# CompVis/stable-diffusion

Measured on AMD Instinct MI355X. Metric: 512x512 images/sec, SD-v1-4 50-step PLMS CFG=7.5, higher is better.
Workload: dtype f16

## Files before the change

### include/sdmi.h

```cpp
#ifndef SDMI_H_
#define SDMI_H_

#include <stdint.h>

#ifdef __cplusplus
extern "C" {
#endif

#define SDMI_ABI_VERSION 17

typedef struct sdmi_unet sdmi_unet;

typedef struct sdmi_unet_cfg {
  int32_t in_channels;
  int32_t out_channels;
  int32_t model_channels;
  int32_t num_res_blocks;
  int32_t n_levels;
  int32_t channel_mult[8];
  int32_t n_attention_resolutions;
  int32_t attention_resolutions[8];
  int32_t num_heads;
  int32_t transformer_depth;
  int32_t context_dim;
// ... 2 lines not shown
const char* sdmi_last_error(void);
int sdmi_abi_version(void);
int sdmi_has_experiments(void);

int sdmi_unet_create(const sdmi_unet_cfg* cfg, sdmi_unet** out);
#define SDMI_PRECISION_MIXED 0
#define SDMI_PRECISION_FULL 1
int sdmi_unet_create_with_precision(const sdmi_unet_cfg* cfg, int precision, sdmi_unet** out);
int sdmi_unet_precision(const sdmi_unet* h);
typedef struct sdmi_unet_ext {
  int32_t attention_block;
  int32_t resblock_updown;
} sdmi_unet_ext;
int sdmi_unet_create_ext(const sdmi_unet_cfg* cfg, const sdmi_unet_ext* ext, int precision, sdmi_unet** out);
#define SDMI_UNET_SCALE_SHIFT_NORM 1u
#define SDMI_UNET_NUM_HEAD_CHANNELS_SHIFT 16
#define SDMI_UNET_NUM_HEAD_CHANNELS_MASK 0x0fff0000u
#define SDMI_UNET_NUM_HEAD_CHANNELS(n) (((unsigned)(n) << SDMI_UNET_NUM_HEAD_CHANNELS_SHIFT) & SDMI_UNET_NUM_HEAD_CHANNELS_MASK)
int sdmi_unet_create_flags(const sdmi_unet_cfg* cfg, const sdmi_unet_ext* ext, unsigned flags, int precision, sdmi_unet** out);
int sdmi_unet_destroy(sdmi_unet* h);
int sdmi_unet_num_weights(const sdmi_unet* h);
int sdmi_unet_weight_info(const sdmi_unet* h, int idx, char* key_buf, int key_buf_len, int64_t* shape4, int* ndim);
int sdmi_unet_set_weight(sdmi_unet* h, const char* key, const float* ptr, const int64_t* shape, int ndim, void* stream);
int sdmi_unet_finalize(sdmi_unet* h);

int64_t sdmi_unet_packed_bytes(sdmi_unet* h);
int sdmi_unet_export_packed(sdmi_unet* h, void* host_buf, int64_t bytes, void* stream);
int sdmi_unet_import_packed(sdmi_unet* h, const void* host_buf, int64_t bytes, void* stream);

int64_t sdmi_unet_workspace_bytes(sdmi_unet* h, int B, int H, int W, int Lctx);

int sdmi_unet_cache_context(sdmi_unet* h, const float* ctx, int B, int Lctx, void* workspace, int64_t workspace_bytes,
                            void* stream);
int sdmi_unet_reserve_context(sdmi_unet* h, int B, int Lctx);

int sdmi_unet_cache_timesteps(sdmi_unet* h, const int64_t* t_host, int n, void* stream);
int sdmi_unet_hint_timestep(sdmi_unet* h, int64_t t);
int sdmi_unet_tape_stats(sdmi_unet* h, int64_t* replayed, int64_t* recorded);

int sdmi_unet_forward(sdmi_unet* h, const float* x, const int64_t* t_i64, const float* t_f32, const float* ctx,
                      float* eps_out, int B, int H, int W, int Lctx, void* workspace, int64_t workspace_bytes,
                      void* stream);

int sdmi_sampler_step(const float* eps_model, int cfg, float scale, const float* x, int mode, const float* old0,
                      const float* old1, const float* old2, float a_t, float a_prev, float sigma, float sqrt_1m_at,
                      const float* noise, float* e_t_out, float* x_prev, float* pred_x0, int64_t n, void* stream);


int sdmi_dpm_solver_step(const float* eps_model, int cfg, float scale, const float* x, const float* m_prev, float alpha_s,
                         float sigma_s, float cx, float a, float inv_r0, int order, float* m_out, float* x_next, int64_t n,
                         void* stream);

typedef struct sdmi_vae sdmi_vae;
typedef struct sdmi_vae_cfg {
  int32_t ch;
  int32_t out_ch;
  int32_t n_levels;
  int32_t ch_mult[8];
  int32_t num_res_blocks;
  int32_t in_channels;
  int32_t z_channels;
  int32_t embed_dim;
} sdmi_vae_cfg;
int sdmi_vae_create(const sdmi_vae_cfg* cfg, int parts, sdmi_vae** out);
typedef struct sdmi_vae_ext {
  int32_t double_z;
  int32_t mid_attn;
  int32_t n_embed;
} sdmi_vae_ext;
int sdmi_vae_create_ext(const sdmi_vae_cfg* cfg, const sdmi_vae_ext* ext, int parts, sdmi_vae** out);
int sdmi_vae_create_precision(const sdmi_vae_cfg* cfg, const sdmi_vae_ext* ext, int parts, int precision, sdmi_vae** out);
int sdmi_vae_precision(const sdmi_vae* h);
int sdmi_vae_decode_vq(sdmi_vae* h, const float* z, float z_scale, int quantize, float* img, int B, int H, int W, void* workspace,
                       int64_t workspace_bytes, void* stream);
int sdmi_vae_destroy(sdmi_vae* h);
int sdmi_vae_num_weights(const sdmi_vae* h);
int sdmi_vae_weight_info(const sdmi_vae* h, int idx, char* key_buf, int key_buf_len, int64_t* shape4, int* ndim);
int sdmi_vae_set_weight(sdmi_vae* h, const char* key, const float* ptr, const int64_t* shape, int ndim, void* stream);
int sdmi_vae_finalize(sdmi_vae* h);
int64_t sdmi_vae_decode_workspace_bytes(sdmi_vae* h, int B, int H, int W);
int sdmi_vae_decode(sdmi_vae* h, const float* z, float z_scale, float* img, int B, int H, int W, void* workspace,
                    int64_t workspace_bytes, void* stream);
int64_t sdmi_vae_encode_workspace_bytes(sdmi_vae* h, int B, int H, int W);
int sdmi_vae_encode(sdmi_vae* h, const float* img, float* moments, int B, int H, int W, void* workspace,
                    int64_t workspace_bytes, void* stream);


typedef struct sdmi_clip sdmi_clip;
typedef struct sdmi_clip_cfg {
  int32_t vocab_size;
  int32_t hidden_size;
  int32_t intermediate_size;
  int32_t num_layers;
  int32_t num_heads;
  int32_t max_positions;
} sdmi_clip_cfg;
int sdmi_clip_create(const sdmi_clip_cfg* cfg, sdmi_clip** out);
int sdmi_clip_destroy(sdmi_clip* h);
int sdmi_clip_num_weights(const sdmi_clip* h);
int sdmi_clip_weight_info(const sdmi_clip* h, int idx, char* key_buf, int key_buf_len, int64_t* shape4, int* ndim);
int sdmi_clip_set_weight(sdmi_clip* h, const char* key, const float* ptr, const int64_t* shape, int ndim, void* stream);
int sdmi_clip_finalize(sdmi_clip* h);
int64_t sdmi_clip_workspace_bytes(sdmi_clip* h, int B, int L);
int sdmi_clip_forward(sdmi_clip* h, const int64_t* ids, float* out, int B, int L, void* workspace, int64_t workspace_bytes,
                      void* stream);

typedef struct sdmi_bert sdmi_bert;
typedef struct sdmi_bert_cfg {
  int32_t vocab_size;
  int32_t dim;
  int32_t depth;
  int32_t heads;
  int32_t dim_head;
  int32_t ff_inner;
  int32_t max_seq_len;
} sdmi_bert_cfg;
int sdmi_bert_create(const sdmi_bert_cfg* cfg, sdmi_bert** out);
int sdmi_bert_destroy(sdmi_bert* h);
int sdmi_bert_num_weights(const sdmi_bert* h);
int sdmi_bert_weight_info(const sdmi_bert* h, int idx, char* key_buf, int key_buf_len, int64_t* shape4, int* ndim);
int sdmi_bert_set_weight(sdmi_bert* h, const char* key, const float* ptr, const int64_t* shape, int ndim, void* stream);
int sdmi_bert_finalize(sdmi_bert* h);
int64_t sdmi_bert_workspace_bytes(sdmi_bert* h, int B, int L);
int sdmi_bert_forward(sdmi_bert* h, const int64_t* ids, float* out, int B, int L, void* workspace, int64_t workspace_bytes,
                      void* stream);

typedef struct sdmi_igemm_desc {
  const void* a0; const void* a1; const void* a2;
  int32_t c0, c1, c2, lda0, lda1, lda2;
  int32_t B, Hin, Win, Hout, Wout, ksize, stride, up;
  const void* w;
  int32_t N;
  int32_t mode;
  const float* bias; const float* rowvec; int32_t ld_rowvec;
  const float* residual; int32_t ldr;
  float* out_f32; void* out_f16; int32_t ldo;
  void* seg_dst[3]; int32_t seg_kind[3];
  int32_t heads, dh, ntok, ntok_pad, segC;
  int32_t splitk;
  float* splitk_ws; int64_t splitk_ws_floats;
  int32_t tile;
  int32_t dma;
  int32_t asym_pad;
  int32_t gn_n; void* gn_acc[2]; int32_t gn_cpg[2]; int32_t gn_cbase[2];
  int32_t* splitk_cnt; int32_t splitk_cnt_ints;
  int32_t split16;
  const float* f16_scale; float* lnp_out;
  const float* lnf_part; int32_t lnf_npart; float lnf_eps; const float* lnf_cs; const float* lnf_d;
  const float* pgn_gamma; const float* pgn_beta; float pgn_eps; int32_t pgn_silu;
  void* pgn_out; int32_t pgn_keep_f32; int32_t* pgn_applied;
  void* out_lo;
} sdmi_igemm_desc;
int sdmi_k_igemm(const sdmi_igemm_desc* d, void* stream);
int sdmi_k_ff_tail(const sdmi_igemm_desc* proj_out, const void* ln_f16, const float* lnp, float ln_eps, const float* csd,
                   const void* wgg_f16, const void* wff2_f16, const float* bff2, const float* t, void* stream);
int sdmi_k_st_tail(const sdmi_igemm_desc* proj_out, const void* a_f16, const void* wo_f16, const float* bo, float* t, const float* ln_gamma,
                   float ln_eps, const float* csd, const void* wgg_f16, const void* wff2_f16, const float* bff2, void* stream);
int sdmi_k_gn_conv3(const sdmi_igemm_desc* conv, const float* x0, const float* x1, int c0, int c1, float* gn_ws, int64_t gn_ws_floats,
                    const float* gn_gamma, const float* gn_beta, float gn_eps, void* stream);
int sdmi_k_st_head(const float* x, float* gn_ws, int64_t gn_ws_floats, const float* gn_gamma, const float* gn_beta, float gn_eps,
                   const void* w_in3, const float* b_in, float* t, const float* ln_gamma, float ln_eps, const void* wqkv_f16,
                   const float* lnf_cs, const float* lnf_d, void* q, void* k, void* vt, int B, int ntok, int ntok_pad, int heads, int dh,
                   int C, void* stream);
int sdmi_k_st_mid(const void* a_f16, const void* wo_f16, const float* bo, float* t, const float* ln_gamma, float ln_eps, const void* wq_f16,
                  const float* lnf_cs, const float* lnf_d, void* q, int B, int ntok, int heads, int dh, int C, void* stream);
int sdmi_k_st_mid_ctx(const void* a_f16, const void* wo_f16, const float* bo, float* t, const float* ln_gamma, float ln_eps, const void* wq_f16,
                      const float* lnf_cs, const float* lnf_d, const void* ctx_k, const void* ctx_vt, int nkv, int nkv_pad, float scale, void* ao_out,
                      int B, int ntok, int heads, int dh, int C, void* stream);
int sdmi_k_ln_fold_prep(const void* w_f16, int N, int K, int ldw, const float* gamma, const float* beta, const float* bias,
                        float* cs, float* d, void* stream);
int sdmi_k_attention(const void* q, const void* k, const void* vt, void* out, int BH, int heads, int nq, int nkv,
                     int nkv_pad, int d, float scale, void* stream);
int sdmi_k_attention_split16(const void* q, const void* q_lo, const void* k, const void* k_lo, const void* vt, const void* vt_lo, void* out,
                             void* out_lo, int BH, int heads, int nq, int nkv, int nkv_pad, int d, float scale, void* stream);
int sdmi_k_attention_causal(const void* q, const void* k, const void* vt, void* out, int BH, int heads, int n, int n_pad,
                            int d, float scale, void* stream);
int sdmi_k_groupnorm(const float* x0, const float* x1, int c0, int c1, int B, int HW, const float* gamma,
                     const float* beta, float eps, int silu, void* out_f16, float* out_f32, void* raw_f16, void* out_lo,
                     void* raw_lo, float* partial_ws, int64_t partial_floats, void* stream);
int64_t sdmi_k_groupnorm_ws_floats(int B, int HW);
int sdmi_k_groupnorm_film(const float* x0, const float* x1, int c0, int c1, int B, int HW, const float* gamma, const float* beta, float eps,
                          int silu, const float* film, int film_ld, void* out_f16, float* out_f32, void* raw_f16, void* out_lo, void* raw_lo,
                          float* partial_ws, int64_t partial_floats, void* stream);
int sdmi_k_layernorm(const float* x, const float* gamma, const float* beta, void* out_f16, int M, int C, float eps,
                     void* stream);
int sdmi_k_cast_f16(const float* x, void* out_f16, void* out_lo, int64_t n, void* stream);
int sdmi_k_split_heads(const float* src, int ld, int col0, void* dst, void* dst_lo, int kind, int B, int ntok, int ntok_pad, int heads, int dh,
                       void* stream);
int sdmi_k_geglu_split(const float* src, int M, int F, void* out, void* out_lo, void* stream);
int sdmi_k_layernorm_split(const float* x, const float* gamma, const float* beta, void* out, void* out_lo, int M, int C, float eps, void* stream);
int sdmi_k_timestep_embedding(const int64_t* t_i64, const float* t_f32, float* out, int B, int dim, void* stream);
int sdmi_k_small_linear(const float* in, int ld_in, const float* w, const float* bias, float* out, int ld_out, int B,
                        int N, int K, int silu_in, void* stream);
int sdmi_k_conv_in(const float* x_nchw, const float* w_oihw, const float* bias, float* out_nhwc, int B, int Cin, int H,
                   int W, int Cout, void* stream);
int sdmi_k_conv_out(const float* h_nhwc, const float* w_ohwi, const float* bias, float* out_nchw, int B, int H, int W,
                    int Cin, int Cout, void* stream);
int sdmi_k_pack_conv_weight(const float* w_oihw, void* dst_f16, int O, int I, int KH, int KW, void* stream);
int sdmi_k_pack_conv_weight_src(const float* w_oihw, void* dst_f16, int O, int I, int KH, int KW, int c0, int c1, int c2, void* stream);
int sdmi_k_pack_conv_out(const float* w_oihw, float* dst_ohwi, int O, int I, void* stream);
int sdmi_k_pack_split3(const float* w, void* dst_f16, int N, int K, void* stream);
int sdmi_k_pack_conv_split3(const float* w_oihw, void* dst_f16, int O, int I, int KH, int KW, void* stream);
int sdmi_k_pointwise_nchw(const float* x, const float* w, const float* bias, float* out, int B, int Cin, int Cout, int HW,
                          float in_scale, void* stream);
int sdmi_k_softmax_rows(const float* S, void* P_f16, int rows, int cols, float scale, void* stream);
int sdmi_k_vq_quantize(const float* z, float z_scale, const float* codebook, float* norms_ws, int n_embed, int D, float* zq, int32_t* idx,
                       int B, int HW, void* stream);
int sdmi_k_resample2(const float* x, float* out_f32, void* out_f16, void* out_lo, int B, int H, int W, int C, int dir, void* stream);
int sdmi_k_patch_unfold(const float* x, const float* c, float* out, int B, int Cx, int Cc, int H, int W, int kh, int kw, int sy, int sx,
                        int l0, int nl, void* stream);
int sdmi_k_patch_fold(const float* o, const float* w, float* out, int B, int C, int H, int W, int kh, int kw, int sy, int sx, int uf, int df,
                      int norm_only, void* stream);
int sdmi_k_gelu_erf(const float* x, void* out_f16, int64_t n, void* stream);
int sdmi_k_pack_geglu(const float* w, const float* bias, void* wdst_f16, float* bdst, int N, int K, void* stream);
int sdmi_image_to_uint8(const float* img_nchw, void* out_nhwc_u8, int B, int C, int H, int W, void* stream);
int sdmi_range_check(int enable);
int sdmi_range_report(char* json_buf, int json_buf_len);
int sdmi_tune_begin(void);
int sdmi_tune_round(int r);
int sdmi_tune_end(const char* path, int* n_keys);
int sdmi_tune_dump(char* buf, int buflen);
int sdmi_profile_begin(void);
int sdmi_profile_end(char* json_buf, int json_buf_len);
int sdmi_k_prefetch_lines(const void* ptr, int64_t bytes, void* stream);
const void* sdmi_zero_page(void);

#ifdef __cplusplus
}
#endif
#endif
```

### stable-diffusion_amd/_lib.py

```python
import ctypes as C
import os

_HERE = os.path.dirname(os.path.abspath(__file__))
LIB_PATH = os.environ.get('SDMI_LIB_PATH') or os.path.join(_HERE, 'libsdmi.so')

c_f32p = C.c_void_p
c_ptr = C.c_void_p


class UNetCfg(C.Structure):
    _fields_ = [('in_channels', C.c_int32), ('out_channels', C.c_int32), ('model_channels', C.c_int32),
                ('num_res_blocks', C.c_int32), ('n_levels', C.c_int32), ('channel_mult', C.c_int32 * 8),
                ('n_attention_resolutions', C.c_int32), ('attention_resolutions', C.c_int32 * 8),
                ('num_heads', C.c_int32), ('transformer_depth', C.c_int32), ('context_dim', C.c_int32)]


class VaeCfg(C.Structure):
    _fields_ = [('ch', C.c_int32), ('out_ch', C.c_int32), ('n_levels', C.c_int32), ('ch_mult', C.c_int32 * 8),
                ('num_res_blocks', C.c_int32), ('in_channels', C.c_int32), ('z_channels', C.c_int32),
                ('embed_dim', C.c_int32)]


class UNetExt(C.Structure):
    _fields_ = [('attention_block', C.c_int32), ('resblock_updown', C.c_int32)]


class VaeExt(C.Structure):
    _fields_ = [('double_z', C.c_int32), ('mid_attn', C.c_int32), ('n_embed', C.c_int32)]


class ClipCfg(C.Structure):
    _fields_ = [('vocab_size', C.c_int32), ('hidden_size', C.c_int32), ('intermediate_size', C.c_int32),
                ('num_layers', C.c_int32), ('num_heads', C.c_int32), ('max_positions', C.c_int32)]


class BertCfg(C.Structure):
    _fields_ = [('vocab_size', C.c_int32), ('dim', C.c_int32), ('depth', C.c_int32), ('heads', C.c_int32),
                ('dim_head', C.c_int32), ('ff_inner', C.c_int32), ('max_seq_len', C.c_int32)]


class IGemmDesc(C.Structure):
    _fields_ = [('a0', c_ptr), ('a1', c_ptr), ('a2', c_ptr),
                ('c0', C.c_int32), ('c1', C.c_int32), ('c2', C.c_int32),
                ('lda0', C.c_int32), ('lda1', C.c_int32), ('lda2', C.c_int32),
                ('B', C.c_int32), ('Hin', C.c_int32), ('Win', C.c_int32), ('Hout', C.c_int32), ('Wout', C.c_int32),
                ('ksize', C.c_int32), ('stride', C.c_int32), ('up', C.c_int32),
                ('w', c_ptr), ('N', C.c_int32), ('mode', C.c_int32),
                ('bias', c_ptr), ('rowvec', c_ptr), ('ld_rowvec', C.c_int32),
                ('residual', c_ptr), ('ldr', C.c_int32),
                ('out_f32', c_ptr), ('out_f16', c_ptr), ('ldo', C.c_int32),
                ('seg_dst', c_ptr * 3), ('seg_kind', C.c_int32 * 3),
                ('heads', C.c_int32), ('dh', C.c_int32), ('ntok', C.c_int32), ('ntok_pad', C.c_int32),
                ('segC', C.c_int32), ('splitk', C.c_int32), ('splitk_ws', c_ptr), ('splitk_ws_floats', C.c_int64),
                ('tile', C.c_int32), ('dma', C.c_int32), ('asym_pad', C.c_int32),
                ('gn_n', C.c_int32), ('gn_acc', c_ptr * 2), ('gn_cpg', C.c_int32 * 2), ('gn_cbase', C.c_int32 * 2),
                ('splitk_cnt', c_ptr), ('splitk_cnt_ints', C.c_int32), ('split16', C.c_int32),
                ('f16_scale', c_ptr), ('lnp_out', c_ptr), ('lnf_part', c_ptr), ('lnf_npart', C.c_int32),
                ('lnf_eps', C.c_float), ('lnf_cs', c_ptr), ('lnf_d', c_ptr),
                ('pgn_gamma', c_ptr), ('pgn_beta', c_ptr), ('pgn_eps', C.c_float), ('pgn_silu', C.c_int32),
                ('pgn_out', c_ptr), ('pgn_keep_f32', C.c_int32), ('pgn_applied', C.POINTER(C.c_int32)),
                ('out_lo', c_ptr)]


_SIGS = {
    'sdmi_last_error': (C.c_char_p, []),
    'sdmi_abi_version': (C.c_int, []),
    'sdmi_unet_create': (C.c_int, [C.POINTER(UNetCfg), C.POINTER(c_ptr)]),
    'sdmi_unet_create_with_precision': (C.c_int, [C.POINTER(UNetCfg), C.c_int, C.POINTER(c_ptr)]),
    'sdmi_unet_precision': (C.c_int, [c_ptr]),
    'sdmi_unet_create_ext': (C.c_int, [C.POINTER(UNetCfg), C.POINTER(UNetExt), C.c_int, C.POINTER(c_ptr)]),
    'sdmi_unet_create_flags': (C.c_int, [C.POINTER(UNetCfg), C.POINTER(UNetExt), C.c_uint, C.c_int, C.POINTER(c_ptr)]),
    'sdmi_unet_destroy': (C.c_int, [c_ptr]),
    'sdmi_unet_num_weights': (C.c_int, [c_ptr]),
    'sdmi_unet_weight_info': (C.c_int, [c_ptr, C.c_int, C.c_char_p, C.c_int, C.POINTER(C.c_int64), C.POINTER(C.c_int)]),
    'sdmi_unet_set_weight': (C.c_int, [c_ptr, C.c_char_p, c_ptr, C.POINTER(C.c_int64), C.c_int, c_ptr]),
    'sdmi_unet_finalize': (C.c_int, [c_ptr]),
    'sdmi_unet_packed_bytes': (C.c_int64, [c_ptr]),
    'sdmi_unet_export_packed': (C.c_int, [c_ptr, c_ptr, C.c_int64, c_ptr]),
    'sdmi_unet_import_packed': (C.c_int, [c_ptr, c_ptr, C.c_int64, c_ptr]),
    'sdmi_unet_workspace_bytes': (C.c_int64, [c_ptr, C.c_int, C.c_int, C.c_int, C.c_int]),
    'sdmi_unet_cache_context': (C.c_int, [c_ptr, c_ptr, C.c_int, C.c_int, c_ptr, C.c_int64, c_ptr]),
    'sdmi_unet_reserve_context': (C.c_int, [c_ptr, C.c_int, C.c_int]),
    'sdmi_unet_cache_timesteps': (C.c_int, [c_ptr, C.POINTER(C.c_int64), C.c_int, c_ptr]),
    'sdmi_unet_hint_timestep': (C.c_int, [c_ptr, C.c_int64]),
    'sdmi_unet_tape_stats': (C.c_int, [c_ptr, C.POINTER(C.c_int64), C.POINTER(C.c_int64)]),
    'sdmi_unet_forward': (C.c_int, [c_ptr, c_ptr, c_ptr, c_ptr, c_ptr, c_ptr, C.c_int, C.c_int, C.c_int, C.c_int,
                                    c_ptr, C.c_int64, c_ptr]),
    'sdmi_sampler_step': (C.c_int, [c_ptr, C.c_int, C.c_float, c_ptr, C.c_int, c_ptr, c_ptr, c_ptr, C.c_float,
                                    C.c_float, C.c_float, C.c_float, c_ptr, c_ptr, c_ptr, c_ptr, C.c_int64, c_ptr]),
    'sdmi_dpm_solver_step': (C.c_int, [c_ptr, C.c_int, C.c_float, c_ptr, c_ptr, C.c_float, C.c_float, C.c_float, C.c_float,
                                       C.c_float, C.c_int, c_ptr, c_ptr, C.c_int64, c_ptr]),
    'sdmi_vae_create': (C.c_int, [C.POINTER(VaeCfg), C.c_int, C.POINTER(c_ptr)]),
    'sdmi_vae_destroy': (C.c_int, [c_ptr]),
    'sdmi_vae_create_ext': (C.c_int, [C.POINTER(VaeCfg), C.POINTER(VaeExt), C.c_int, C.POINTER(c_ptr)]),
    'sdmi_vae_create_precision': (C.c_int, [C.POINTER(VaeCfg), C.POINTER(VaeExt), C.c_int, C.c_int, C.POINTER(c_ptr)]),
    'sdmi_vae_precision': (C.c_int, [c_ptr]),
    'sdmi_vae_decode_vq': (C.c_int, [c_ptr, c_ptr, C.c_float, C.c_int, c_ptr, C.c_int, C.c_int, C.c_int, c_ptr, C.c_int64, c_ptr]),
    'sdmi_k_vq_quantize': (C.c_int, [c_ptr, C.c_float, c_ptr, c_ptr, C.c_int, C.c_int, c_ptr, c_ptr, C.c_int, C.c_int, c_ptr]),
    'sdmi_k_patch_unfold': (C.c_int, [c_ptr, c_ptr, c_ptr] + [C.c_int] * 11 + [c_ptr]),
    'sdmi_k_patch_fold': (C.c_int, [c_ptr, c_ptr, c_ptr] + [C.c_int] * 11 + [c_ptr]),
    'sdmi_k_resample2': (C.c_int, [c_ptr, c_ptr, c_ptr, c_ptr, C.c_int, C.c_int, C.c_int, C.c_int, C.c_int, c_ptr]),
    'sdmi_vae_num_weights': (C.c_int, [c_ptr]),
    'sdmi_vae_weight_info': (C.c_int, [c_ptr, C.c_int, C.c_char_p, C.c_int, C.POINTER(C.c_int64), C.POINTER(C.c_int)]),
    'sdmi_vae_set_weight': (C.c_int, [c_ptr, C.c_char_p, c_ptr, C.POINTER(C.c_int64), C.c_int, c_ptr]),
    'sdmi_vae_finalize': (C.c_int, [c_ptr]),
    'sdmi_vae_decode_workspace_bytes': (C.c_int64, [c_ptr, C.c_int, C.c_int, C.c_int]),
    'sdmi_vae_decode': (C.c_int, [c_ptr, c_ptr, C.c_float, c_ptr, C.c_int, C.c_int, C.c_int, c_ptr, C.c_int64, c_ptr]),
    'sdmi_vae_encode_workspace_bytes': (C.c_int64, [c_ptr, C.c_int, C.c_int, C.c_int]),
    'sdmi_vae_encode': (C.c_int, [c_ptr, c_ptr, c_ptr, C.c_int, C.c_int, C.c_int, c_ptr, C.c_int64, c_ptr]),
    'sdmi_clip_create': (C.c_int, [C.POINTER(ClipCfg), C.POINTER(c_ptr)]),
    'sdmi_clip_destroy': (C.c_int, [c_ptr]),
    'sdmi_clip_num_weights': (C.c_int, [c_ptr]),
    'sdmi_clip_weight_info': (C.c_int, [c_ptr, C.c_int, C.c_char_p, C.c_int, C.POINTER(C.c_int64), C.POINTER(C.c_int)]),
    'sdmi_clip_set_weight': (C.c_int, [c_ptr, C.c_char_p, c_ptr, C.POINTER(C.c_int64), C.c_int, c_ptr]),
    'sdmi_clip_finalize': (C.c_int, [c_ptr]),
    'sdmi_clip_workspace_bytes': (C.c_int64, [c_ptr, C.c_int, C.c_int]),
    'sdmi_clip_forward': (C.c_int, [c_ptr, c_ptr, c_ptr, C.c_int, C.c_int, c_ptr, C.c_int64, c_ptr]),
    'sdmi_bert_create': (C.c_int, [C.POINTER(BertCfg), C.POINTER(c_ptr)]),
    'sdmi_bert_destroy': (C.c_int, [c_ptr]),
    'sdmi_bert_num_weights': (C.c_int, [c_ptr]),
    'sdmi_bert_weight_info': (C.c_int, [c_ptr, C.c_int, C.c_char_p, C.c_int, C.POINTER(C.c_int64), C.POINTER(C.c_int)]),
    'sdmi_bert_set_weight': (C.c_int, [c_ptr, C.c_char_p, c_ptr, C.POINTER(C.c_int64), C.c_int, c_ptr]),
    'sdmi_bert_finalize': (C.c_int, [c_ptr]),
    'sdmi_bert_workspace_bytes': (C.c_int64, [c_ptr, C.c_int, C.c_int]),
    'sdmi_bert_forward': (C.c_int, [c_ptr, c_ptr, c_ptr, C.c_int, C.c_int, c_ptr, C.c_int64, c_ptr]),
    'sdmi_has_experiments': (C.c_int, []),
    'sdmi_k_igemm': (C.c_int, [C.POINTER(IGemmDesc), c_ptr]),
    'sdmi_k_ff_tail': (C.c_int, [C.POINTER(IGemmDesc), c_ptr, c_ptr, C.c_float, c_ptr, c_ptr, c_ptr, c_ptr, c_ptr, c_ptr]),
    'sdmi_k_gn_conv3': (C.c_int, [C.POINTER(IGemmDesc), c_ptr, c_ptr, C.c_int, C.c_int, c_ptr, C.c_int64, c_ptr, c_ptr, C.c_float, c_ptr]),
    'sdmi_k_st_mid_ctx': (C.c_int, [c_ptr, c_ptr, c_ptr, c_ptr, c_ptr, C.c_float, c_ptr, c_ptr, c_ptr, c_ptr, c_ptr, C.c_int, C.c_int, C.c_float, c_ptr,
                                    C.c_int, C.c_int, C.c_int, C.c_int, C.c_int, c_ptr]),
    'sdmi_k_st_tail': (C.c_int, [C.POINTER(IGemmDesc), c_ptr, c_ptr, c_ptr, c_ptr, c_ptr, C.c_float, c_ptr, c_ptr, c_ptr, c_ptr, c_ptr]),
    'sdmi_k_st_mid': (C.c_int, [c_ptr, c_ptr, c_ptr, c_ptr, c_ptr, C.c_float, c_ptr, c_ptr, c_ptr, c_ptr, C.c_int, C.c_int, C.c_int, C.c_int,
                                C.c_int, c_ptr]),
    'sdmi_k_st_head': (C.c_int, [c_ptr, c_ptr, C.c_int64, c_ptr, c_ptr, C.c_float, c_ptr, c_ptr, c_ptr, c_ptr, C.c_float, c_ptr, c_ptr, c_ptr,
                                 c_ptr, c_ptr, c_ptr, C.c_int, C.c_int, C.c_int, C.c_int, C.c_int, C.c_int, c_ptr]),
    'sdmi_k_attention_split16': (C.c_int, [c_ptr, c_ptr, c_ptr, c_ptr, c_ptr, c_ptr, c_ptr, c_ptr, C.c_int, C.c_int, C.c_int, C.c_int,
                                           C.c_int, C.c_int, C.c_float, c_ptr]),
    'sdmi_k_attention_causal': (C.c_int, [c_ptr, c_ptr, c_ptr, c_ptr, C.c_int, C.c_int, C.c_int, C.c_int, C.c_int, C.c_float,
                                          c_ptr]),
    'sdmi_k_pointwise_nchw': (C.c_int, [c_ptr, c_ptr, c_ptr, c_ptr, C.c_int, C.c_int, C.c_int, C.c_int, C.c_float, c_ptr]),
    'sdmi_k_softmax_rows': (C.c_int, [c_ptr, c_ptr, C.c_int, C.c_int, C.c_float, c_ptr]),
    'sdmi_k_gelu_erf': (C.c_int, [c_ptr, c_ptr, C.c_int64, c_ptr]),
    'sdmi_k_attention': (C.c_int, [c_ptr, c_ptr, c_ptr, c_ptr, C.c_int, C.c_int, C.c_int, C.c_int, C.c_int, C.c_int,
                                   C.c_float, c_ptr]),
    'sdmi_k_groupnorm': (C.c_int, [c_ptr, c_ptr, C.c_int, C.c_int, C.c_int, C.c_int, c_ptr, c_ptr, C.c_float, C.c_int,
                                   c_ptr, c_ptr, c_ptr, c_ptr, c_ptr, c_ptr, C.c_int64, c_ptr]),
    'sdmi_k_groupnorm_ws_floats': (C.c_int64, [C.c_int, C.c_int]),
    'sdmi_k_groupnorm_film': (C.c_int, [c_ptr, c_ptr, C.c_int, C.c_int, C.c_int, C.c_int, c_ptr, c_ptr, C.c_float, C.c_int, c_ptr, C.c_int,
                                        c_ptr, c_ptr, c_ptr, c_ptr, c_ptr, c_ptr, C.c_int64, c_ptr]),
    'sdmi_k_layernorm': (C.c_int, [c_ptr, c_ptr, c_ptr, c_ptr, C.c_int, C.c_int, C.c_float, c_ptr]),
    'sdmi_k_cast_f16': (C.c_int, [c_ptr, c_ptr, c_ptr, C.c_int64, c_ptr]),
    'sdmi_k_split_heads': (C.c_int, [c_ptr, C.c_int, C.c_int, c_ptr, c_ptr, C.c_int, C.c_int, C.c_int, C.c_int, C.c_int, C.c_int,
                                     c_ptr]),
    'sdmi_k_geglu_split': (C.c_int, [c_ptr, C.c_int, C.c_int, c_ptr, c_ptr, c_ptr]),
    'sdmi_k_layernorm_split': (C.c_int, [c_ptr, c_ptr, c_ptr, c_ptr, c_ptr, C.c_int, C.c_int, C.c_float, c_ptr]),
    'sdmi_k_timestep_embedding': (C.c_int, [c_ptr, c_ptr, c_ptr, C.c_int, C.c_int, c_ptr]),
    'sdmi_k_small_linear': (C.c_int, [c_ptr, C.c_int, c_ptr, c_ptr, c_ptr, C.c_int, C.c_int, C.c_int, C.c_int,
                                      C.c_int, c_ptr]),
    'sdmi_k_conv_in': (C.c_int, [c_ptr, c_ptr, c_ptr, c_ptr, C.c_int, C.c_int, C.c_int, C.c_int, C.c_int, c_ptr]),
    'sdmi_k_conv_out': (C.c_int, [c_ptr, c_ptr, c_ptr, c_ptr, C.c_int, C.c_int, C.c_int, C.c_int, C.c_int, c_ptr]),
    'sdmi_k_pack_conv_weight': (C.c_int, [c_ptr, c_ptr, C.c_int, C.c_int, C.c_int, C.c_int, c_ptr]),
    'sdmi_k_pack_conv_weight_src': (C.c_int, [c_ptr, c_ptr, C.c_int, C.c_int, C.c_int, C.c_int, C.c_int, C.c_int, C.c_int, c_ptr]),
    'sdmi_k_pack_conv_out': (C.c_int, [c_ptr, c_ptr, C.c_int, C.c_int, c_ptr]),
    'sdmi_k_pack_split3': (C.c_int, [c_ptr, c_ptr, C.c_int, C.c_int, c_ptr]),
    'sdmi_k_pack_conv_split3': (C.c_int, [c_ptr, c_ptr, C.c_int, C.c_int, C.c_int, C.c_int, c_ptr]),
    'sdmi_k_pack_geglu': (C.c_int, [c_ptr, c_ptr, c_ptr, c_ptr, C.c_int, C.c_int, c_ptr]),
    'sdmi_k_ln_fold_prep': (C.c_int, [c_ptr, C.c_int, C.c_int, C.c_int, c_ptr, c_ptr, c_ptr, c_ptr, c_ptr, c_ptr]),
    'sdmi_image_to_uint8': (C.c_int, [c_ptr, c_ptr, C.c_int, C.c_int, C.c_int, C.c_int, c_ptr]),
    'sdmi_range_check': (C.c_int, [C.c_int]),
    'sdmi_range_report': (C.c_int, [C.c_char_p, C.c_int]),
    'sdmi_tune_begin': (C.c_int, []),
    'sdmi_tune_round': (C.c_int, [C.c_int]),
    'sdmi_tune_end': (C.c_int, [C.c_char_p, C.POINTER(C.c_int)]),
    'sdmi_tune_dump': (C.c_int, [C.c_char_p, C.c_int]),
    'sdmi_profile_begin': (C.c_int, []),
    'sdmi_profile_end': (C.c_int, [C.c_char_p, C.c_int]),
    'sdmi_k_prefetch_lines': (C.c_int, [c_ptr, C.c_int64, c_ptr]),
    'sdmi_zero_page': (c_ptr, []),
}

_lib = None


class SdmiError(RuntimeError):
    pass


def load():
    global _lib
    if _lib is None:
        if not os.path.exists(LIB_PATH):
            raise SdmiError(f'{LIB_PATH} not found: build it with `python stable-diffusion_amd/build.py` '
                            '(the MI355X path has no fallback implementation)')
        lib = C.CDLL(LIB_PATH)
        for name, (res, args) in _SIGS.items():
            fn = getattr(lib, name)
            fn.restype = res
            fn.argtypes = args
        if lib.sdmi_abi_version() != 17:
            raise SdmiError('libsdmi ABI version mismatch')
        _lib = lib
    return _lib


def exported_symbols():
    return sorted(_SIGS)


def check(rc):
    if rc != 0:
        raise SdmiError(load().sdmi_last_error().decode('utf-8', 'replace'))


def ptr(t):
    return None if t is None else t.data_ptr()


def stream_ptr():
    import torch
    return torch.cuda.current_stream().cuda_stream
```

### stable-diffusion_amd/csrc/api.cpp

```cpp
#include <string.h>

#include <new>

#include "prof.h"
#include "split16.h"
#include "unet.h"
#include "vae.h"
#include "clip.h"

namespace sdmi {
static thread_local std::string g_err;
void set_error(const std::string& msg) { g_err = msg; }
int fail(const std::string& msg) { g_err = msg; return -1; }
}

struct sdmi_unet { sdmi::UNet impl; };
struct sdmi_vae { sdmi::Vae impl; };
struct sdmi_clip { sdmi::ClipText impl; };
struct sdmi_bert { sdmi::BertText impl; };

using namespace sdmi;

static void* g_zero_page[16] = {nullptr};
static int zero_page(const f16** out) {
// ... 188 lines not shown
                       int64_t workspace_bytes, void* stream) {
  SDMI_CHECK(h && z && img, "null argument");
  return h->impl.decode(z, z_scale, img, B, H, W, workspace, workspace_bytes, (hipStream_t)stream, false, nullptr, quantize != 0);
}
int64_t sdmi_vae_encode_workspace_bytes(sdmi_vae* h, int B, int H, int W) {
  if (!h) { fail("null handle"); return 0; }
  int64_t need = 0;
  if (h->impl.encode(nullptr, nullptr, B, H, W, nullptr, 0, nullptr, true, &need)) return 0;
  return need;
}
int sdmi_vae_encode(sdmi_vae* h, const float* img, float* moments, int B, int H, int W, void* workspace,
                    int64_t workspace_bytes, void* stream) {
  SDMI_CHECK(h && img && moments, "null argument");
  return h->impl.encode(img, moments, B, H, W, workspace, workspace_bytes, (hipStream_t)stream, false, nullptr);
}
int sdmi_k_pointwise_nchw(const float* x, const float* w, const float* bias, float* out, int B, int Cin, int Cout, int HW,
                          float in_scale, void* stream) {
  return launch_pointwise_nchw(x, w, bias, out, B, Cin, Cout, HW, in_scale, (hipStream_t)stream);
}
int sdmi_k_softmax_rows(const float* S, void* P_f16, int rows, int cols, float scale, void* stream) {
  return launch_softmax_rows(S, (f16*)P_f16, rows, cols, cols, cols, scale, (hipStream_t)stream);
}


int sdmi_clip_create(const sdmi_clip_cfg* cfg, sdmi_clip** out) {
  SDMI_CHECK(cfg && out, "null argument");
  sdmi_clip* h = new (std::nothrow) sdmi_clip();
  SDMI_CHECK(h != nullptr, "out of host memory");
  if (h->impl.build(*cfg)) { delete h; return -1; }
  *out = h;
  return 0;
}
int sdmi_clip_destroy(sdmi_clip* h) { delete h; return 0; }
int sdmi_clip_num_weights(const sdmi_clip* h) { return h ? (int)h->impl.slots().size() : fail("null handle"); }
static int text_weight_info(const TextEncBase& t, int idx, char* key_buf, int key_buf_len, int64_t* shape4, int* ndim) {
  SDMI_CHECK(key_buf && shape4 && ndim, "null argument");
  SDMI_CHECK(idx >= 0 && idx < (int)t.slots().size(), "weight index out of range");
  const CWeightSlot& s = t.slots()[idx];
  SDMI_CHECK((int)s.key.size() + 1 <= key_buf_len, "key buffer too small");
  memcpy(key_buf, s.key.c_str(), s.key.size() + 1);
  *ndim = (int)s.shape.size();
  for (int i = 0; i < 4; ++i) shape4[i] = i < *ndim ? s.shape[i] : 1;
  return 0;
}
int sdmi_clip_weight_info(const sdmi_clip* h, int idx, char* key_buf, int key_buf_len, int64_t* shape4, int* ndim) {
  SDMI_CHECK(h && key_buf && shape4 && ndim, "null argument");
  return text_weight_info(h->impl, idx, key_buf, key_buf_len, shape4, ndim);
}
int sdmi_clip_set_weight(sdmi_clip* h, const char* key, const float* ptr, const int64_t* shape, int ndim, void* stream) {
  SDMI_CHECK(h && key && ptr && shape, "null argument");
  return h->impl.set_weight(key, ptr, shape, ndim, (hipStream_t)stream);
}
int sdmi_clip_finalize(sdmi_clip* h) { SDMI_CHECK(h, "null handle"); return h->impl.finalize(); }
int64_t sdmi_clip_workspace_bytes(sdmi_clip* h, int B, int L) {
  if (!h) { fail("null handle"); return 0; }
  int64_t need = 0;
  if (h->impl.forward(nullptr, nullptr, B, L, nullptr, 0, nullptr, true, &need)) return 0;
  return need;
}
int sdmi_clip_forward(sdmi_clip* h, const int64_t* ids, float* out, int B, int L, void* workspace, int64_t workspace_bytes,
                      void* stream) {
  SDMI_CHECK(h && ids && out, "null argument");
  return h->impl.forward(ids, out, B, L, workspace, workspace_bytes, (hipStream_t)stream, false, nullptr);
}

int sdmi_bert_create(const sdmi_bert_cfg* cfg, sdmi_bert** out) {
  SDMI_CHECK(cfg && out, "null argument");
  sdmi_bert* h = new (std::nothrow) sdmi_bert();
  SDMI_CHECK(h != nullptr, "out of host memory");
  if (h->impl.build(*cfg)) { delete h; return -1; }
  *out = h;
  return 0;
}
int sdmi_bert_destroy(sdmi_bert* h) { delete h; return 0; }
int sdmi_bert_num_weights(const sdmi_bert* h) { return h ? (int)h->impl.slots().size() : fail("null handle"); }
int sdmi_bert_weight_info(const sdmi_bert* h, int idx, char* key_buf, int key_buf_len, int64_t* shape4, int* ndim) {
  SDMI_CHECK(h && key_buf && shape4 && ndim, "null argument");
  return text_weight_info(h->impl, idx, key_buf, key_buf_len, shape4, ndim);
}
int sdmi_bert_set_weight(sdmi_bert* h, const char* key, const float* ptr, const int64_t* shape, int ndim, void* stream) {
  SDMI_CHECK(h && key && ptr && shape, "null argument");
  return h->impl.set_weight(key, ptr, shape, ndim, (hipStream_t)stream);
}
int sdmi_bert_finalize(sdmi_bert* h) { SDMI_CHECK(h, "null handle"); return h->impl.finalize(); }
int64_t sdmi_bert_workspace_bytes(sdmi_bert* h, int B, int L) {
  if (!h) { fail("null handle"); return 0; }
  int64_t need = 0;
  if (h->impl.forward(nullptr, nullptr, B, L, nullptr, 0, nullptr, true, &need)) return 0;
  return need;
}
int sdmi_bert_forward(sdmi_bert* h, const int64_t* ids, float* out, int B, int L, void* workspace, int64_t workspace_bytes,
                      void* stream) {
  SDMI_CHECK(h && ids && out, "null argument");
  return h->impl.forward(ids, out, B, L, workspace, workspace_bytes, (hipStream_t)stream, false, nullptr);
}
int sdmi_k_vq_quantize(const float* z, float z_scale, const float* codebook, float* norms_ws, int n_embed, int D, float* zq, int32_t* idx,
                       int B, int HW, void* stream) {
  if (launch_vq_norms(codebook, norms_ws, n_embed, D, (hipStream_t)stream)) return -1;
  return launch_vq_quantize(z, z_scale, codebook, norms_ws, n_embed, D, zq, (int*)idx, B, HW, (hipStream_t)stream);
}
int sdmi_k_resample2(const float* x, float* out_f32, void* out_f16, void* out_lo, int B, int H, int W, int C, int dir, void* stream) {
  return launch_resample2(x, out_f32, (f16*)out_f16, (f16*)out_lo, B, H, W, C, dir, (hipStream_t)stream);
}
int sdmi_k_patch_unfold(const float* x, const float* c, float* out, int B, int Cx, int Cc, int H, int W, int kh, int kw, int sy, int sx,
                        int l0, int nl, void* stream) {
  return launch_patch_unfold(x, c, out, B, Cx, Cc, H, W, kh, kw, sy, sx, l0, nl, (hipStream_t)stream);
}
int sdmi_k_patch_fold(const float* o, const float* w, float* out, int B, int C, int H, int W, int kh, int kw, int sy, int sx, int uf, int df,
                      int norm_only, void* stream) {
  return launch_patch_fold(o, w, out, B, C, H, W, kh, kw, sy, sx, uf, df, norm_only, (hipStream_t)stream);
}
int sdmi_k_gelu_erf(const float* x, void* out_f16, int64_t n, void* stream) {
  return launch_gelu_erf(x, (f16*)out_f16, n, (hipStream_t)stream);
}
int sdmi_k_attention_causal(const void* q, const void* k, const void* vt, void* out, int BH, int heads, int n, int n_pad,
                            int d, float scale, void* stream) {
  AttnParams a = AttnParams();
  a.q = (const f16*)q; a.k = (const f16*)k; a.vt = (const f16*)vt; a.out = (f16*)out;
  a.BH = BH; a.heads = heads; a.nq = n; a.nkv = n; a.nkv_pad = n_pad; a.d = d; a.scale = scale; a.causal = 1;
  return launch_attention(a, (hipStream_t)stream);
}

static int igemm_params_of(const sdmi_igemm_desc* d, IGemmParams& p) {
  p.a0 = (const f16*)d->a0; p.a1 = (const f16*)d->a1; p.a2 = (const f16*)d->a2;
  p.c0 = d->c0; p.c1 = d->c1; p.c2 = d->c2; p.lda0 = d->lda0; p.lda1 = d->lda1; p.lda2 = d->lda2;
  p.B = d->B; p.Hin = d->Hin; p.Win = d->Win; p.Hout = d->Hout; p.Wout = d->Wout;
  p.ksize = d->ksize; p.stride = d->stride; p.up = d->up; p.pad = d->asym_pad ? 0 : 1;
  p.w = (const f16*)d->w; p.M = d->B * d->Hout * d->Wout; p.N = d->N; p.K = d->ksize * d->ksize * (d->c0 + d->c1 + d->c2);
  p.mode = d->mode; p.bias = d->bias; p.rowvec = d->rowvec; p.ld_rowvec = d->ld_rowvec;
  p.residual = d->residual; p.ldr = d->ldr; p.out_f32 = d->out_f32; p.out_f16 = (f16*)d->out_f16; p.ldo = d->ldo;
  for (int i = 0; i < 3; ++i) { p.seg_dst[i] = (f16*)d->seg_dst[i]; p.seg_kind[i] = d->seg_kind[i]; }
  p.heads = d->heads; p.dh = d->dh; p.ntok = d->ntok; p.ntok_pad = d->ntok_pad; p.segC = d->segC;
  p.splitk = d->splitk; p.splitk_ws = d->splitk_ws; p.splitk_ws_floats = d->splitk_ws_floats;
  p.splitk_cnt = d->splitk_cnt; p.splitk_cnt_ints = d->splitk_cnt_ints;
  p.gn_n = d->gn_n;
  for (int i = 0; i < 2; ++i) { p.gn_acc[i] = (long long*)d->gn_acc[i]; p.gn_cpg[i] = d->gn_cpg[i]; p.gn_cbase[i] = d->gn_cbase[i]; }
  if (d->split16) {
    p.split16 = 1; p.c1 = 0; p.K = d->c0; p.ldw = 3 * d->c0;
  }
  p.f16_scale = d->f16_scale; p.lnp_out = d->lnp_out;
  p.lnf_part = d->lnf_part; p.lnf_npart = d->lnf_npart; p.lnf_eps = d->lnf_eps; p.lnf_cs = d->lnf_cs; p.lnf_d = d->lnf_d;
  p.pgn_gamma = d->pgn_gamma; p.pgn_beta = d->pgn_beta; p.pgn_eps = d->pgn_eps; p.pgn_silu = d->pgn_silu;
  p.pgn_out = (f16*)d->pgn_out; p.pgn_keep_f32 = d->pgn_keep_f32; p.pgn_applied = d->pgn_applied;
  p.out_lo = (f16*)d->out_lo;
  return zero_page(&p.zero_page);
}
int sdmi_k_igemm(const sdmi_igemm_desc* d, void* stream) {
  SDMI_CHECK(d, "null descriptor");
  IGemmParams p = IGemmParams();
  if (igemm_params_of(d, p)) return -1;
  IGemmTune t; t.tile = d->tile; t.dma = d->dma;
  return launch_igemm(p, t, (hipStream_t)stream);
}
int sdmi_k_ff_tail(const sdmi_igemm_desc* proj_out, const void* ln_f16, const float* lnp, float ln_eps, const float* csd,
                   const void* wgg_f16, const void* wff2_f16, const float* bff2, const float* t, void* stream) {
  SDMI_CHECK(proj_out, "null descriptor");
  FfTailParams q = FfTailParams();
  if (igemm_params_of(proj_out, q.epi)) return -1;
  SDMI_CHECK(proj_out->split16 && proj_out->ksize == 1, "ff_tail: the proj_out descriptor is a split-fp16 1x1 (w = sdmi_k_pack_split3)");
  q.ln = (const f16*)ln_f16; q.lnp = lnp; q.ln_eps = ln_eps; q.csd = csd; q.wgg = (const f16*)wgg_f16; q.wff2 = (const f16*)wff2_f16;
  q.bff2 = bff2; q.t = t; q.wpo = (const f16*)proj_out->w;
  return launch_ff_tail(q, (hipStream_t)stream);
}
int sdmi_k_st_tail(const sdmi_igemm_desc* proj_out, const void* a_f16, const void* wo_f16, const float* bo, float* t, const float* ln_gamma,
                   float ln_eps, const float* csd, const void* wgg_f16, const void* wff2_f16, const float* bff2, void* stream) {
  SDMI_CHECK(proj_out && a_f16, "null argument");
  FfTailParams q = FfTailParams();
  if (igemm_params_of(proj_out, q.epi)) return -1;
  SDMI_CHECK(proj_out->split16 && proj_out->ksize == 1, "st_tail: the proj_out descriptor is a split-fp16 1x1 (w = sdmi_k_pack_split3)");
  q.a16 = (const f16*)a_f16; q.wo = (const f16*)wo_f16; q.bo = bo; q.ln_gamma = ln_gamma; q.ln_eps = ln_eps; q.csd = csd;
  q.wgg = (const f16*)wgg_f16; q.wff2 = (const f16*)wff2_f16; q.bff2 = bff2; q.t = t; q.wpo = (const f16*)proj_out->w;
  return launch_ff_tail(q, (hipStream_t)stream);
}
int sdmi_k_gn_conv3(const sdmi_igemm_desc* conv, const float* x0, const float* x1, int c0, int c1, float* gn_ws, int64_t gn_ws_floats,
                    const float* gn_gamma, const float* gn_beta, float gn_eps, void* stream) {
  SDMI_CHECK(conv && x0 && gn_ws && gn_gamma && gn_beta, "gn_conv3: null argument");
  GnConvParams q = GnConvParams();
  if (igemm_params_of(conv, q.epi)) return -1;
  const int B = q.epi.B;
  SDMI_CHECK(gn_ws_floats >= gn_acc_words(B) * 2, "groupnorm workspace too small");
  SDMI_HIP_OK(hipMemsetAsync(gn_ws, 0, gn_acc_words(B) * sizeof(long long), (hipStream_t)stream));
  GroupNormParams g = GroupNormParams();
  g.x0 = x0; g.c0 = c0; g.x1 = x1; g.c1 = c1; g.B = B; g.HW = q.epi.Hout * q.epi.Wout; g.gamma = gn_gamma; g.beta = gn_beta; g.eps = gn_eps;
  g.stats_only = 1; g.acc = (long long*)gn_ws;
  if (launch_groupnorm(g, (hipStream_t)stream)) return -1;
  q.x0 = x0; q.x1 = x1; q.c0 = c0; q.c1 = c1; q.gn_acc = (const long long*)gn_ws; q.gn_gamma = gn_gamma; q.gn_beta = gn_beta; q.gn_eps = gn_eps;
  q.w = (const f16*)conv->w;
  return launch_gn_conv3(q, (hipStream_t)stream);
}
int sdmi_k_st_head(const float* x, float* gn_ws, int64_t gn_ws_floats, const float* gn_gamma, const float* gn_beta, float gn_eps,
                   const void* w_in3, const float* b_in, float* t, const float* ln_gamma, float ln_eps, const void* wqkv_f16,
                   const float* lnf_cs, const float* lnf_d, void* q, void* k, void* vt, int B, int ntok, int ntok_pad, int heads, int dh,
                   int C, void* stream) {
  SDMI_CHECK(x && gn_ws && gn_gamma && gn_beta, "st_head: null argument");
  SDMI_CHECK(gn_ws_floats >= gn_acc_words(B) * 2, "groupnorm workspace too small");
  SDMI_HIP_OK(hipMemsetAsync(gn_ws, 0, gn_acc_words(B) * sizeof(long long), (hipStream_t)stream));
  GroupNormParams g = GroupNormParams();
  g.x0 = x; g.c0 = C; g.B = B; g.HW = ntok; g.gamma = gn_gamma; g.beta = gn_beta; g.eps = gn_eps; g.stats_only = 1; g.acc = (long long*)gn_ws;
  if (launch_groupnorm(g, (hipStream_t)stream)) return -1;
  StHeadParams p = StHeadParams();
  p.x = x; p.gn_acc = (const long long*)gn_ws; p.gn_gamma = gn_gamma; p.gn_beta = gn_beta; p.gn_eps = gn_eps;
  p.w_in = (const f16*)w_in3; p.b_in = b_in; p.t = t; p.ln_gamma = ln_gamma; p.ln_eps = ln_eps; p.wqkv = (const f16*)wqkv_f16;
  p.lnf_cs = lnf_cs; p.lnf_d = lnf_d; p.q = (f16*)q; p.k = (f16*)k; p.vt = (f16*)vt;
  p.M = B * ntok; p.B = B; p.ntok = ntok; p.ntok_pad = ntok_pad; p.heads = heads; p.dh = dh; p.C = C;
  return launch_st_head(p, (hipStream_t)stream);
}
int sdmi_k_st_mid(const void* a_f16, const void* wo_f16, const float* bo, float* t, const float* ln_gamma, float ln_eps, const void* wq_f16,
                  const float* lnf_cs, const float* lnf_d, void* q, int B, int ntok, int heads, int dh, int C, void* stream) {
  StHeadParams p = StHeadParams();
  p.a16 = (const f16*)a_f16; p.w_in = (const f16*)wo_f16; p.b_in = bo; p.t = t; p.ln_gamma = ln_gamma; p.ln_eps = ln_eps;
  p.wqkv = (const f16*)wq_f16; p.lnf_cs = lnf_cs; p.lnf_d = lnf_d; p.q = (f16*)q;
  p.M = B * ntok; p.B = B; p.ntok = ntok; p.ntok_pad = ntok; p.heads = heads; p.dh = dh; p.C = C;
  return launch_st_mid(p, (hipStream_t)stream);
}
int sdmi_k_st_mid_ctx(const void* a_f16, const void* wo_f16, const float* bo, float* t, const float* ln_gamma, float ln_eps, const void* wq_f16,
                      const float* lnf_cs, const float* lnf_d, const void* ctx_k, const void* ctx_vt, int nkv, int nkv_pad, float scale, void* ao_out,
                      int B, int ntok, int heads, int dh, int C, void* stream) {
  StHeadParams p = StHeadParams();
  p.a16 = (const f16*)a_f16; p.w_in = (const f16*)wo_f16; p.b_in = bo; p.t = t; p.ln_gamma = ln_gamma; p.ln_eps = ln_eps;
  p.wqkv = (const f16*)wq_f16; p.lnf_cs = lnf_cs; p.lnf_d = lnf_d;
  p.ctx_k = (const f16*)ctx_k; p.ctx_vt = (const f16*)ctx_vt; p.ctx_nkv = nkv; p.ctx_nkv_pad = nkv_pad; p.ctx_scale = scale; p.ao_out = (f16*)ao_out;
  SDMI_CHECK(ctx_k && ctx_vt && ao_out, "st_mid_ctx: null argument");
  p.M = B * ntok; p.B = B; p.ntok = ntok; p.ntok_pad = ntok; p.heads = heads; p.dh = dh; p.C = C;
  return launch_st_mid(p, (hipStream_t)stream);
}
int sdmi_k_ln_fold_prep(const void* w_f16, int N, int K, int ldw, const float* gamma, const float* beta, const float* bias,
                        float* cs, float* d, void* stream) {
  return launch_ln_fold_prep((const f16*)w_f16, N, K, ldw, gamma, beta, bias, cs, d, (hipStream_t)stream);
}
int sdmi_k_attention(const void* q, const void* k, const void* vt, void* out, int BH, int heads, int nq, int nkv,
                     int nkv_pad, int d, float scale, void* stream) {
  AttnParams a = AttnParams();
  a.q = (const f16*)q; a.k = (const f16*)k; a.vt = (const f16*)vt; a.out = (f16*)out;
  a.BH = BH; a.heads = heads; a.nq = nq; a.nkv = nkv; a.nkv_pad = nkv_pad; a.d = d; a.scale = scale;
  if (const char* e = getenv("SDMI_ATTN_NW")) a.nw = atoi(e);
  return launch_attention(a, (hipStream_t)stream);
}
int sdmi_k_attention_split16(const void* q, const void* q_lo, const void* k, const void* k_lo, const void* vt, const void* vt_lo, void* out,
                             void* out_lo, int BH, int heads, int nq, int nkv, int nkv_pad, int d, float scale, void* stream) {
  AttnSplitParams a = AttnSplitParams();
  a.q = (const f16*)q; a.q_lo = (const f16*)q_lo; a.k = (const f16*)k; a.k_lo = (const f16*)k_lo; a.vt = (const f16*)vt;
  a.vt_lo = (const f16*)vt_lo; a.out = (f16*)out; a.out_lo = (f16*)out_lo;
  a.BH = BH; a.heads = heads; a.nq = nq; a.nkv = nkv; a.nkv_pad = nkv_pad; a.d = d; a.scale = scale;
  return launch_attention_split16(a, (hipStream_t)stream);
}
int64_t sdmi_k_groupnorm_ws_floats(int B, int HW) { (void)HW; return gn_acc_words(B) * 2; }
int sdmi_k_groupnorm(const float* x0, const float* x1, int c0, int c1, int B, int HW, const float* gamma,
                     const float* beta, float eps, int silu, void* out_f16, float* out_f32, void* raw_f16, void* out_lo,
                     void* raw_lo, float* partial_ws, int64_t partial_floats, void* stream) {
  SDMI_CHECK(partial_floats >= gn_acc_words(B) * 2, "groupnorm workspace too small");
  SDMI_HIP_OK(hipMemsetAsync(partial_ws, 0, gn_acc_words(B) * sizeof(long long), (hipStream_t)stream));
  GroupNormParams g = GroupNormParams();
  g.x0 = x0; g.x1 = x1; g.c0 = c0; g.c1 = c1; g.B = B; g.HW = HW; g.gamma = gamma; g.beta = beta; g.eps = eps;
  g.silu = silu; g.out_f16 = (f16*)out_f16; g.out_f32 = out_f32; g.raw_f16 = (f16*)raw_f16; g.out_lo = (f16*)out_lo; g.raw_lo = (f16*)raw_lo;
  g.acc = (long long*)partial_ws;
  return launch_groupnorm(g, (hipStream_t)stream);
}
int sdmi_k_groupnorm_film(const float* x0, const float* x1, int c0, int c1, int B, int HW, const float* gamma, const float* beta, float eps,
                          int silu, const float* film, int film_ld, void* out_f16, float* out_f32, void* raw_f16, void* out_lo, void* raw_lo,
                          float* partial_ws, int64_t partial_floats, void* stream) {
  SDMI_CHECK(partial_floats >= gn_acc_words(B) * 2, "groupnorm workspace too small");
  SDMI_HIP_OK(hipMemsetAsync(partial_ws, 0, gn_acc_words(B) * sizeof(long long), (hipStream_t)stream));
  GroupNormParams g = GroupNormParams();
  g.x0 = x0; g.x1 = x1; g.c0 = c0; g.c1 = c1; g.B = B; g.HW = HW; g.gamma = gamma; g.beta = beta; g.eps = eps;
  g.silu = silu; g.out_f16 = (f16*)out_f16; g.out_f32 = out_f32; g.raw_f16 = (f16*)raw_f16; g.out_lo = (f16*)out_lo; g.raw_lo = (f16*)raw_lo;
  g.film = film; g.film_ld = film_ld;
  g.acc = (long long*)partial_ws;
  return launch_groupnorm(g, (hipStream_t)stream);
}
int sdmi_k_layernorm(const float* x, const float* gamma, const float* beta, void* out_f16, int M, int C, float eps,
                     void* stream) {
  return launch_layernorm(x, gamma, beta, (f16*)out_f16, M, C, eps, (hipStream_t)stream);
}
int sdmi_k_cast_f16(const float* x, void* out_f16, void* out_lo, int64_t n, void* stream) {
  return launch_cast_f16(x, (f16*)out_f16, (f16*)out_lo, n, (hipStream_t)stream);
}
int sdmi_k_split_heads(const float* src, int ld, int col0, void* dst, void* dst_lo, int kind, int B, int ntok, int ntok_pad, int heads, int dh,
                       void* stream) {
  return launch_split_heads(src, ld, col0, (f16*)dst, (f16*)dst_lo, kind, B, ntok, ntok_pad, heads, dh, (hipStream_t)stream);
}
int sdmi_k_geglu_split(const float* src, int M, int F, void* out, void* out_lo, void* stream) {
  return launch_geglu_split(src, M, F, (f16*)out, (f16*)out_lo, (hipStream_t)stream);
}
int sdmi_k_layernorm_split(const float* x, const float* gamma, const float* beta, void* out, void* out_lo, int M, int C, float eps, void* stream) {
  return launch_layernorm_split(x, gamma, beta, (f16*)out, (f16*)out_lo, M, C, eps, (hipStream_t)stream);
}
int sdmi_k_timestep_embedding(const int64_t* t_i64, const float* t_f32, float* out, int B, int dim, void* stream) {
  return launch_timestep_embedding(t_i64, t_f32, out, B, dim, (hipStream_t)stream);
}
int sdmi_k_small_linear(const float* in, int ld_in, const float* w, const float* bias, float* out, int ld_out, int B,
                        int N, int K, int silu_in, void* stream) {
  return launch_small_linear(in, ld_in, w, bias, out, ld_out, B, N, K, silu_in, (hipStream_t)stream);
}
int sdmi_k_conv_in(const float* x, const float* w, const float* bias, float* out, int B, int Cin, int H, int W, int Cout,
                   void* stream) {
  return launch_conv_in(x, w, bias, out, B, Cin, H, W, Cout, (hipStream_t)stream);
}
int sdmi_k_conv_out(const float* h, const float* w, const float* bias, float* out, int B, int H, int W, int Cin, int Cout,
                    void* stream) {
  return launch_conv_out(h, w, bias, out, B, H, W, Cin, Cout, (hipStream_t)stream);
}
int sdmi_k_pack_conv_weight(const float* w, void* dst, int O, int I, int KH, int KW, void* stream) {
  return launch_pack_conv_weight(w, (f16*)dst, O, I, KH, KW, (hipStream_t)stream);
}
int sdmi_k_pack_conv_weight_src(const float* w, void* dst, int O, int I, int KH, int KW, int c0, int c1, int c2, void* stream) {
  return launch_pack_conv_weight_src(w, (f16*)dst, O, I, KH, KW, c0, c1, c2, (hipStream_t)stream);
// ... 57 lines not shown
```

### stable-diffusion_amd/csrc/common.h

```cpp
#pragma once
#include <hip/hip_runtime.h>
#include <stdint.h>
#include <algorithm>
#include <string>

#include "tape.h"

typedef _Float16 f16;
typedef _Float16 f16x2 __attribute__((ext_vector_type(2)));
typedef _Float16 f16x4 __attribute__((ext_vector_type(4)));
typedef _Float16 f16x8 __attribute__((ext_vector_type(8)));
typedef float f32x4 __attribute__((ext_vector_type(4)));
typedef float f32x16 __attribute__((ext_vector_type(16)));

#ifdef __HIPCC__
__device__ __forceinline__ float gn_apply_elem(float v, float mean, float rstd, float gamma, float beta, int silu) {
  float t = __builtin_fmaf((v - mean) * rstd, gamma, beta);
  if (silu) t = t * __builtin_amdgcn_rcpf(1.0f + __expf(-t));
  return t;
}
__device__ __forceinline__ float gn_apply_film_elem(float v, float mean, float rstd, float gamma, float beta, float scale, float shift,
                                                    int silu) {
  float t = __builtin_fmaf((v - mean) * rstd, gamma, beta);
  t = __builtin_fmaf(t, 1.0f + scale, shift);
  if (silu) t = t * __builtin_amdgcn_rcpf(1.0f + __expf(-t));
  return t;
}
__device__ __forceinline__ void gn_acc_add(unsigned long long* dst, float v) {
  const double d = (double)v;
  const double hi = rint(d);
  atomicAdd(dst, (unsigned long long)(long long)hi);
  atomicAdd(dst + 1, (unsigned long long)__double2ll_rn((d - hi) * 1099511627776.0));
}
__device__ __forceinline__ double gn_acc_value(long long hi, long long lo) {
  return (double)hi + (double)lo * (1.0 / 1099511627776.0);
}
__device__ __forceinline__ void gn_fixed_split(float v, long long* hi, long long* lo) {
  const double d = (double)v;
  const double h = rint(d);
  *hi = (long long)h;
  *lo = __double2ll_rn((d - h) * 1099511627776.0);
}
__device__ __forceinline__ void gn_mean_rstd(long long s, long long sl, long long ss, long long ssl, double n, float eps,
                                             float* mean, float* rstd) {
  const double m = gn_acc_value(s, sl) / n;
  double var = gn_acc_value(ss, ssl) / n - m * m;
  if (var < 0.0) var = 0.0;
  *mean = (float)m;
  *rstd = (float)(1.0 / sqrt(var + (double)eps));
}
#endif

namespace sdmi {

void set_error(const std::string& msg);
int fail(const std::string& msg);

#define SDMI_HIP_OK(expr)                                                                    \
  do {                                                                                       \
    hipError_t _e = (expr);                                                                  \
    if (_e != hipSuccess)                                                                    \
      return ::sdmi::fail(std::string(#expr) + ": " + hipGetErrorString(_e));                \
  } while (0)

#define SDMI_CHECK(cond, msg)                                                                \
  do {                                                                                       \
    if (!(cond)) return ::sdmi::fail(std::string("check failed: ") + #cond + " -- " + (msg)); \
  } while (0)

static inline int cdiv(int a, int b) { return (a + b - 1) / b; }
static inline int64_t round_up(int64_t a, int64_t b) { return (a + b - 1) / b * b; }

enum EpiMode { EPI_PLAIN = 0, EPI_GEGLU = 1, EPI_HEADS = 2 };

#ifdef SDMI_NT_STORES
#define SDMI_ST(T, ptr, val) __builtin_nontemporal_store((T)(val), (T*)(ptr))
#else
#define SDMI_ST(T, ptr, val) (*(T*)(ptr) = (T)(val))
#endif
#ifndef SDMI_W_AUX
#define SDMI_W_AUX 0
#endif
#ifndef SDMI_WT_STORES
#define SDMI_WT_STORES 1
#endif
#if defined(__HIPCC__) && SDMI_WT_STORES >= 1
typedef unsigned sdmi_u32x4 __attribute__((ext_vector_type(4)));
typedef unsigned sdmi_u32x2 __attribute__((ext_vector_type(2)));
__device__ __forceinline__ void sdmi_st_wt16(const void* base, size_t byte_off, f32x4 v) {
  if (__builtin_expect(byte_off < (size_t)0x80000000u - 16, 1)) {
    const __amdgpu_buffer_rsrc_t r = __builtin_amdgcn_make_buffer_rsrc((void*)base, 0, (int)0x80000000, 0x00020000);
    __builtin_amdgcn_raw_buffer_store_b128(__builtin_bit_cast(sdmi_u32x4, v), r, (int)byte_off, 0, 16);
  } else {
    *(f32x4*)((char*)base + byte_off) = v;
  }
}
__device__ __forceinline__ void sdmi_st_wt8(const void* base, size_t byte_off, f16x4 v) {
  if (__builtin_expect(byte_off < (size_t)0x80000000u - 16, 1)) {
    const __amdgpu_buffer_rsrc_t r = __builtin_amdgcn_make_buffer_rsrc((void*)base, 0, (int)0x80000000, 0x00020000);
    __builtin_amdgcn_raw_buffer_store_b64(__builtin_bit_cast(sdmi_u32x2, v), r, (int)byte_off, 0, 16);
  } else {
    *(f16x4*)((char*)base + byte_off) = v;
  }
}
#define SDMI_ST_F32X4(base, off, val) sdmi_st_wt16((base), (size_t)(off) * 4, (val))
#if SDMI_WT_STORES >= 2
#define SDMI_ST_F16X4(base, off, val) sdmi_st_wt8((base), (size_t)(off) * 2, (val))
#else
#define SDMI_ST_F16X4(base, off, val) SDMI_ST(f16x4, (base) + (off), (val))
#endif
#else
#define SDMI_ST_F32X4(base, off, val) SDMI_ST(f32x4, (base) + (off), (val))
#define SDMI_ST_F16X4(base, off, val) SDMI_ST(f16x4, (base) + (off), (val))
#endif

struct IGemmParams {
  const f16* a0 = nullptr; const f16* a1 = nullptr; const f16* a2 = nullptr;
  int c0 = 0, c1 = 0, c2 = 0;
  int lda0 = 0, lda1 = 0, lda2 = 0;
  int B = 1, Hin = 1, Win = 1;
  int Hout = 1, Wout = 1;
  int ksize = 1, stride = 1, up = 0;
  int pad = 1;
  const f16* w = nullptr;
  int M = 0, N = 0, K = 0;
  int k_alg = 0;
  int split16 = 0;
  int ldw = 0;
  int mode = EPI_PLAIN;
  const float* bias = nullptr;
  const float* rowvec = nullptr; int ld_rowvec = 0;
  const float* residual = nullptr; int ldr = 0;
  float* out_f32 = nullptr; f16* out_f16 = nullptr; int ldo = 0;
  f16* out_lo = nullptr;
  const float* ln_gamma = nullptr; const float* ln_beta = nullptr; f16* ln_out = nullptr; float ln_eps = 1e-5f;
  const float* f16_scale = nullptr;
  float* lnp_out = nullptr;
  const float* lnf_part = nullptr; int lnf_npart = 0; float lnf_eps = 1e-5f;
  const float* lnf_cs = nullptr; const float* lnf_d = nullptr;
  f16* seg_dst[3] = {nullptr, nullptr, nullptr};
  int seg_kind[3] = {0, 0, 0};
  int heads = 0, dh = 0, ntok = 0, ntok_pad = 0, segC = 0;
  int splitk = 1;
  float* splitk_ws = nullptr; int64_t splitk_ws_floats = 0;
  int* splitk_cnt = nullptr; int splitk_cnt_ints = 0;
  int nkt = 0;
#ifdef SDMI_IGEMM_TIMING
  long long* dbg_times = nullptr;
  int dbg_abl = 0;
#endif
  int splitk_fused = 0;
  int slab_tiled = 0, slab_bm = 0, slab_bn = 0, slab_wm = 0, slab_wn = 0;
  int slab_sh_qpt = 0, slab_sh_nt = 0, slab_sh_tn = 0, slab_sh_wn = 0;
  int epi_vec = 0;
  int tile_n_fastest = 0;
  const f16* zero_page = nullptr;
  int gn_n = 0;
  long long* gn_acc[2] = {nullptr, nullptr};
  int gn_cpg[2] = {0, 0}, gn_cbase[2] = {0, 0};
  unsigned long long gn_magic[2] = {0, 0};
  const float* pgn_gamma = nullptr; const float* pgn_beta = nullptr; float pgn_eps = 1e-5f; int pgn_silu = 1;
  f16* pgn_out = nullptr;
  int pgn_keep_f32 = 0;
  int* pgn_applied = nullptr;
  unsigned long long magic_hw = 0, magic_w = 0, magic_w2 = 0;
  int log2w = 0;
  const float* xf0 = nullptr; const float* xf1 = nullptr;
  const long long* gn_in_acc = nullptr;
  const float* gn_in_gamma = nullptr; const float* gn_in_beta = nullptr; float gn_in_eps = 1e-5f; int gn_in_silu = 1;
  f16* raw_hi = nullptr; f16* raw_lo = nullptr;
  f16* gn_scratch = nullptr;
  unsigned long long magic_cpg_in = 0;
  int halo_thi = 0, halo_ipt = 1, log2_tpi = 30;
  unsigned long long magic_hpi = 0;
};

constexpr int SDMI_NUM_TILES = 22;
struct IGemmTune {
  int tile = -1;
  int dma = -1;
};

int launch_igemm(const IGemmParams& p, const IGemmTune& tune, hipStream_t stream);
bool range_check_enabled();
uint64_t tune_generation();
bool tune_collecting();
int range_check_set(int enable);
int range_scan(const char* what, const f16* p, int64_t n, hipStream_t stream);
int range_report(std::string* json);

int tune_begin();
int tune_round(int r);
int tune_end(const char* path, int* n_keys);
int tune_dump(std::string* out);
int launch_splitk_reduce(const IGemmParams& p, int nsplit, hipStream_t stream);

struct FfTailParams {
  const f16* ln = nullptr;
  const float* lnp = nullptr;
  float ln_eps = 1e-5f;
  const float* csd = nullptr;
  const f16* wgg = nullptr;
  const f16* wff2 = nullptr;
  const float* bff2 = nullptr;
  const float* t = nullptr;
  const f16* wpo = nullptr;
  const f16* a16 = nullptr;
  const f16* wo = nullptr;
  const float* bo = nullptr;
  const float* ln_gamma = nullptr;
#ifdef SDMI_RC_TIMING
  long long* dbg = nullptr;
#endif
  IGemmParams epi;
};
bool ff_tail_supported(int C, int M, int rows_per_sample);
int launch_ff_tail(const FfTailParams& p, hipStream_t stream);

struct StHeadParams {
  const f16* a16 = nullptr;
  const float* x = nullptr;
  const long long* gn_acc = nullptr;
  const float* gn_gamma = nullptr; const float* gn_beta = nullptr; float gn_eps = 1e-6f;
  const f16* w_in = nullptr;
  const float* b_in = nullptr;
  float* t = nullptr;
  const float* ln_gamma = nullptr;
  float ln_eps = 1e-5f;
  const f16* wqkv = nullptr;
  const float* lnf_cs = nullptr; const float* lnf_d = nullptr;
  f16* q = nullptr; f16* k = nullptr;
  f16* vt = nullptr;
  int M = 0, B = 0, ntok = 0, ntok_pad = 0, heads = 0, dh = 0, C = 0;
  const f16* ctx_k = nullptr; const f16* ctx_vt = nullptr; int ctx_nkv = 0, ctx_nkv_pad = 0; float ctx_scale = 0.f; f16* ao_out = nullptr;
#ifdef SDMI_RC_TIMING
  long long* dbg = nullptr;
#endif
};
bool st_head_supported(int C, int M, int ntok, int ntok_pad, int heads, int dh);
int launch_st_head(const StHeadParams& p, hipStream_t stream);
int launch_st_mid(const StHeadParams& p, hipStream_t stream);

struct GnConvParams {
  const float* x0 = nullptr; const float* x1 = nullptr; int c0 = 0, c1 = 0;
  const long long* gn_acc = nullptr;
  const float* gn_gamma = nullptr; const float* gn_beta = nullptr; float gn_eps = 1e-5f;
  const f16* w = nullptr;
#ifdef SDMI_RC_TIMING
  long long* dbg = nullptr;
#endif
  IGemmParams epi;
};
bool gn_conv3_supported(int B, int H, int W, int c0, int c1, int Cout);
int launch_gn_conv3(const GnConvParams& p, hipStream_t stream);

struct AttnParams {
  const f16* q = nullptr;
  const f16* k = nullptr;
  const f16* vt = nullptr;
  f16* out = nullptr;
  int BH = 0, heads = 0, nq = 0, nkv = 0, nkv_pad = 0, d = 0;
  float scale = 1.f;
  int nw = 0;
  int causal = 0;
  int prio = 0;
  int pingpong = 0;
};
int launch_attention(const AttnParams& p, hipStream_t stream);
int launch_attention_wide(const AttnParams& p, hipStream_t stream);

struct GroupNormParams {
  const float* x0 = nullptr; const float* x1 = nullptr; int c0 = 0, c1 = 0;
  int B = 0, HW = 0;
  const float* gamma = nullptr; const float* beta = nullptr; float eps = 1e-5f;
  int silu = 0;
  int stats_only = 0;
  int skip_stats = 0;
  f16* out_f16 = nullptr;
  float* out_f32 = nullptr;
  f16* raw_f16 = nullptr;
  f16* out_lo = nullptr;
  f16* raw_lo = nullptr;
  const float* film = nullptr; int film_ld = 0;
  long long* acc = nullptr;
};
constexpr int GN_SLOTS = 8;
constexpr int GN_MAX_CALLS = 96;
constexpr int GN_WORDS = 4;
constexpr int GN_STRIDE = 16;
static inline int64_t gn_acc_words(int B) { return (int64_t)B * 32 * GN_SLOTS * GN_STRIDE; }
int launch_groupnorm(const GroupNormParams& p, hipStream_t stream);

int launch_layernorm(const float* x, const float* gamma, const float* beta, f16* out, int M, int C, float eps,
                     hipStream_t stream, float* out_f32 = nullptr);
int launch_cast_f16(const float* x, f16* out, f16* out_lo, int64_t n, hipStream_t stream);

int launch_timestep_embedding(const int64_t* t_i64, const float* t_f32, float* out, int B, int dim, hipStream_t s);
int launch_small_linear(const float* in, int ld_in, const float* w, const float* bias, float* out, int ld_out,
                        int B, int N, int K, int silu_in, hipStream_t s);
int launch_ctx1_broadcast(const f16* vt, int ld_v, f16* ao, int B, int ntok, int C, hipStream_t s);
int launch_conv_in(const float* x_nchw, const float* w, const float* bias, float* out_nhwc, int B, int Cin, int H,
                   int W, int Cout, hipStream_t s, int gn_n = 0, long long* const* gn_acc = nullptr, const int* gn_cpg = nullptr,
                   const int* gn_cbase = nullptr);
int launch_conv_out(const float* h_nhwc, const float* w_khwc, const float* bias, float* out_nchw, int B, int H, int W,
                    int Cin, int Cout, hipStream_t s);

struct DpmStepParams {
  const float* eps_model = nullptr;
  int cfg = 0; float scale = 1.f;
  const float* x = nullptr;
  const float* m_prev = nullptr;
  float alpha_s = 1.f, sigma_s = 0.f;
  float cx = 1.f, a = 0.f, inv_r0 = 0.f;
  int order = 1;
  float* m_out = nullptr;
  float* x_next = nullptr;
  int64_t n = 0;
};
int launch_dpm_step(const DpmStepParams& p, hipStream_t s);

int launch_embed_tokens(const int64_t* ids, const float* tok_emb, const float* pos_emb, float* out, int M, int L, int C,
                        int vocab, hipStream_t s);
int launch_quick_gelu(const float* x, f16* out, int64_t n, hipStream_t s);
int launch_gelu_erf(const float* x, f16* out, int64_t n, hipStream_t s);

int launch_pointwise_nchw(const float* x_nchw, const float* w, const float* bias, float* out_nchw, int B, int Cin, int Cout,
                          int HW, float in_scale, hipStream_t s);
int launch_softmax_rows(const float* S, f16* P, int rows, int cols, int lds, int ldp, float scale, hipStream_t s);

int launch_resample2(const float* x, float* o32, f16* hi, f16* lo, int B, int H, int W, int C, int dir, hipStream_t s);
int launch_vq_norms(const float* e, float* se, int n_embed, int D, hipStream_t s);
int launch_vq_quantize(const float* z, float z_scale, const float* e, const float* se, int n_embed, int D, float* zq, int* idx, int B,
                       int HW, hipStream_t s);

int launch_patch_unfold(const float* x, const float* c, float* out, int B, int Cx, int Cc, int H, int W, int kh, int kw, int sy, int sx,
                        int l0, int nl, hipStream_t s);
// ... 32 lines not shown
```

### stable-diffusion_amd/csrc/conv3halo.hip

```cpp
#include "igemm_dev.h"

namespace sdmi {
namespace {

template <int BM, int BN, int WARPS_M, int WARPS_N, int NS>
__global__ void __launch_bounds__(WARPS_M* WARPS_N * 64) conv3halo_kernel(const IGemmParams p, const int tiles_m,
                                                                           const int tiles_n, const int chunks_per_split) {
#if defined(__HIP_DEVICE_COMPILE__)
  constexpr int NT = WARPS_M * WARPS_N * 64;
  constexpr int RPP = NT / 8;
  constexpr int PB = BN / RPP;
  constexpr int WTM = BM / WARPS_M, WTN = BN / WARPS_N;
  constexpr int TM = WTM / 32, TN = WTN / 32;
  constexpr int HPMAX = (BM / 64 + 2) * 66;
  constexpr int AHP = (HPMAX + RPP - 1) / RPP;
  constexpr int HALO_BYTES = AHP * RPP * 128;
  constexpr int BSTAGE = BN * 128;
  constexpr int LDS_BYTES = 2 * HALO_BYTES + NS * BSTAGE;
  constexpr int LASTA = 10 - NS;
  constexpr int PA = (AHP + LASTA) / (LASTA + 1);
  constexpr int KS = BK / 16;
  constexpr int G = (TM * TN >= 4) ? 1 : 2;
  constexpr int U = KS / G;
  constexpr int MPU = G * TM * TN;
  static_assert(PB >= 1 && TM >= 1 && TN >= 1 && RPP % 16 == 0 && NS >= 2 && NS <= 9, "tile/wave shape");
  static_assert(LDS_BYTES <= 160 * 1024, "LDS budget");

  __shared__ __attribute__((aligned(16))) unsigned char smem[LDS_BYTES];

  const int nblk = gridDim.x;
  const int bid = blockIdx.x;
  const int q8 = nblk >> 3, r8 = nblk & 7, xcd = bid & 7;
  const int wgid = (xcd < r8 ? xcd * (q8 + 1) : r8 * (q8 + 1) + (xcd - r8) * q8) + (bid >> 3);
  const int tiles_mn = tiles_m * tiles_n;
  const int split = wgid / tiles_mn;
  const int tmn = wgid - split * tiles_mn;
  int tile_m, tile_n;
  if (p.tile_n_fastest) { tile_m = tmn / tiles_n; tile_n = tmn - tile_m * tiles_n; }
  else { tile_n = tmn / tiles_m; tile_m = tmn - tile_n * tiles_m; }
  const int m0 = tile_m * BM, n0 = tile_n * BN;
  const int nch = (p.c0 + p.c1 + p.c2) / BK;
  const int c_begin = split * chunks_per_split;
  const int c_end = min(nch, c_begin + chunks_per_split);
  if (c_begin >= c_end) return;

  const int tid = threadIdx.x;
  SDMI_STAMP(dbg_t0);
  const int lane = tid & 63;
  const int wave = tid >> 6;
  const int cpos = tid & 7, lrow = tid >> 3;
  const int gch = cpos ^ ((lrow >> 1) & 7);
  const int wave_u = __builtin_amdgcn_readfirstlane(wave);
  const int wm = wave / WARPS_N, wn = wave - wm * WARPS_N;
  const int l31 = lane & 31, lg = lane >> 5;
  const int rsw = (l31 >> 1) & 7;

  const int W = p.Wout, H = p.Hout, HW = H * W, W2 = W + 2, ld = p.lda0;
  const int bimg = m0 / HW;
  const int THI = p.halo_thi;
  const int HPI = (THI + 2) * W2;
  const int y0 = p.halo_ipt > 1 ? 0 : (m0 - bimg * HW) >> p.log2w;
  const int HP = p.halo_ipt * HPI;
  constexpr int OOB = (int)0x80000000;

  int hvoff[AHP];
#pragma unroll
  for (int q = 0; q < AHP; ++q) {
    const int hp = q * RPP + lrow;
    const int ip = fast_div(hp, p.magic_hpi), hr = hp - ip * HPI;
    const int hy = fast_div(hr, p.magic_w2), hx = hr - hy * W2;
    const int y = y0 + hy - 1, x = hx - 1;
    const bool valid = hp < HP && y >= 0 && y < H && x >= 0 && x < W;
    hvoff[q] = valid ? ((((bimg + ip) * H + y) * W + x) * ld + gch * 8) * 2 : OOB;
  }
  int b_off[PB];
#pragma unroll
  for (int i = 0; i < PB; ++i) {
    const int n = min(n0 + i * RPP + lrow, p.N - 1);
    b_off[i] = (n * p.K + gch * 8) * 2;
  }
  int hr0[TM];
#pragma unroll
  for (int i = 0; i < TM; ++i) {
    const int ml = wm * WTM + i * 32 + l31;
    const int ip = ml >> p.log2_tpi, mr = ml & ((1 << p.log2_tpi) - 1);
    hr0[i] = ip * HPI + (mr >> p.log2w) * W2 + (mr & (W - 1));
  }
  const int b_lds = 2 * HALO_BYTES + (wn * WTN + l31) * 128;

  const char* const srcA0 = (const char*)p.a0; const char* const srcA1 = (const char*)p.a1;
  const char* const srcA2 = (const char*)p.a2;
  const __amdgpu_buffer_rsrc_t rsrc_w = __builtin_amdgcn_make_buffer_rsrc((void*)p.w, 0, OOB, 0x00020000);
  const int pc0 = p.c0, pc01 = p.c0 + p.c1;
  struct ChunkSrc { __amdgpu_buffer_rsrc_t rsrc; int soff; };
  auto chunk_src = [&](int c) {
    const int cin0 = c * BK;
    const char* src; int coff;
    if (cin0 < pc0) { src = srcA0; coff = cin0; }
    else if (cin0 < pc01) { src = srcA1; coff = cin0 - pc0; }
    else { src = srcA2; coff = cin0 - pc01; }
    ChunkSrc r; r.rsrc = __builtin_amdgcn_make_buffer_rsrc((void*)src, 0, OOB, 0x00020000); r.soff = coff * 2;
    return r;
  };
  auto issue_halo = [&](const ChunkSrc& cs, int hbuf, int q) {
    auto dst = (__attribute__((address_space(3))) void*)(smem + hbuf * HALO_BYTES + (q * RPP + wave_u * 8) * 128);
    __builtin_amdgcn_raw_ptr_buffer_load_lds(cs.rsrc, dst, 16, hvoff[q], cs.soff, 0, 0);
  };
  auto issue_b = [&](int kt, int stage, int q) {
    auto dst = (__attribute__((address_space(3))) void*)(smem + 2 * HALO_BYTES + stage * BSTAGE + (q * RPP + wave_u * 8) * 128);
    __builtin_amdgcn_raw_ptr_buffer_load_lds(rsrc_w, dst, 16, b_off[q], kt * (BK * 2), 0, SDMI_W_AUX);
  };

  f32x16 acc[TM][TN];
#pragma unroll
  for (int i = 0; i < TM; ++i)
#pragma unroll
    for (int j = 0; j < TN; ++j)
#pragma unroll
      for (int r = 0; r < 16; ++r) acc[i][j][r] = 0.f;

  auto a_base = [&](int i, int ky, int kx, int hbuf) -> int {
    const int rowt = hr0[i] + ky * W2 + kx;
    return hbuf * HALO_BYTES + ((rowt << 7) | ((lg ^ ((rowt >> 1) & 7)) << 4));
  };
  auto read_frags = [&](const int (&ab)[TM], int bstage, int ks, f16x8 (&a)[TM], f16x8 (&b)[TN]) {
#pragma unroll
    for (int i = 0; i < TM; ++i) a[i] = *(const f16x8*)(smem + (ab[i] ^ (ks << 5)));
    const unsigned char* st = smem + bstage * BSTAGE + b_lds + (((ks * 2 + lg) ^ rsw) << 4);
#pragma unroll
    for (int j = 0; j < TN; ++j) b[j] = *(const f16x8*)(st + j * 32 * 128);
  };
  auto mfma_step = [&](const f16x8 (&a)[TM], const f16x8 (&b)[TN]) {
#pragma unroll
    for (int i = 0; i < TM; ++i)
#pragma unroll
      for (int j = 0; j < TN; ++j) acc[i][j] = __builtin_amdgcn_mfma_f32_32x32x16_f16(a[i], b[j], acc[i][j], 0, 0, 0);
  };

  auto a_lo = [](int t) { return t <= LASTA ? (t * PA < AHP ? t * PA : AHP) : AHP; };
  auto a_hi = [](int t) { return t <= LASTA ? ((t + 1) * PA < AHP ? (t + 1) * PA : AHP) : AHP; };
  auto in_flight_ok = [&](int t) {
    int n = 0;
    for (int d = 0; d < NS - 2; ++d) { const int tt = (t - d + 18) % 9; n += a_hi(tt) - a_lo(tt) + PB; }
    return n;
  };

  const int kt_first = c_begin * 9, kt_last = c_end * 9 - 1;
  {
    const ChunkSrc cs = chunk_src(c_begin);
#pragma unroll
    for (int q = 0; q < AHP; ++q) issue_halo(cs, 0, q);
#pragma unroll
    for (int s2 = 0; s2 < NS - 1; ++s2) {
      const int vt = 9 - (NS - 1) + s2;
#pragma unroll
      for (int e = a_lo(vt); e < a_hi(vt); ++e) issue_halo(cs, 0, 0);
#pragma unroll
      for (int q = 0; q < PB; ++q) issue_b(min(kt_first + s2, kt_last), s2, q);
    }
  }
  wait_vmcnt_n(in_flight_ok(8));
  asm volatile("s_waitcnt lgkmcnt(0)\n\ts_barrier" ::: "memory");
  SDMI_STAMP(dbg_t1);
  f16x8 fa[2][G][TM], fb[2][G][TN];
  int ab[TM];
#pragma unroll
  for (int i = 0; i < TM; ++i) ab[i] = a_base(i, 0, 0, 0);
#pragma unroll
  for (int g = 0; g < G; ++g) read_frags(ab, 0, g, fa[0][g], fb[0][g]);

  int cur = 0, nxt = NS - 1, hb = 0;
  for (int c = c_begin; c < c_end; ++c) {
    const ChunkSrc csn = chunk_src(min(c + 1, c_end - 1));
#pragma unroll
    for (int tap = 0; tap < 9; ++tap) {
      const int kt = c * 9 + tap;
      const int tap1 = tap == 8 ? 0 : tap + 1;
      const int hb1 = tap == 8 ? (hb ^ 1) : hb;
      const int cur1 = (cur + 1 == NS) ? 0 : cur + 1;
      int ab1[TM];
#pragma unroll
      for (int i = 0; i < TM; ++i) ab1[i] = a_base(i, tap1 / 3, tap1 % 3, hb1);
      const int alo = a_lo(tap);
      const int na = a_hi(tap) - alo;
      const int npieces = na + PB;
      const int ppu = (npieces + U - 2) / (U - 1);
      const int bt = min(kt + NS - 1, kt_last);
#pragma unroll
      for (int u = 0; u < U; ++u) {
        if (u + 1 < U) {
#pragma unroll
          for (int g = 0; g < G; ++g) read_frags(ab, cur, (u + 1) * G + g, fa[(u + 1) & 1][g], fb[(u + 1) & 1][g]);
#pragma unroll
          for (int e = u * ppu; e < (u + 1) * ppu && e < npieces; ++e) {
            if (e < na) issue_halo(csn, hb ^ 1, alo + e);
            else issue_b(bt, nxt, e - na);
          }
        } else {
          wait_vmcnt_n(in_flight_ok(tap));
          asm volatile("s_waitcnt lgkmcnt(0)\n\ts_barrier" ::: "memory");
#pragma unroll
          for (int g = 0; g < G; ++g) read_frags(ab1, cur1, g, fa[0][g], fb[0][g]);
        }
#pragma unroll
        for (int g = 0; g < G; ++g) mfma_step(fa[u & 1][g], fb[u & 1][g]);
        __builtin_amdgcn_sched_group_barrier(0x100, G * (TM + TN), 0);
#pragma unroll
        for (int e = 0; e < MPU; ++e) {
          __builtin_amdgcn_sched_group_barrier(0x008, 1, 0);
          if (u + 1 < U && e < ppu && u * ppu + e < npieces) __builtin_amdgcn_sched_group_barrier(0x010, 1, 0);
        }
      }
#pragma unroll
      for (int i = 0; i < TM; ++i) ab[i] = ab1[i];
      cur = cur1;
      nxt = (nxt + 1 == NS) ? 0 : nxt + 1;
      hb = hb1;
    }
  }
  wait_vmcnt<0>();
  SDMI_STAMP(dbg_t2);
  igemm_epilogue<BM, BN, WARPS_M, WARPS_N, LDS_BYTES>(p, acc, m0, n0, split, tile_m, tile_n, smem);
#ifdef SDMI_IGEMM_TIMING
  if (p.dbg_times && tid == 0) {
    long long* d = p.dbg_times + 6 * (size_t)blockIdx.x;
    d[0] = dbg_t0; d[1] = dbg_t1; d[2] = dbg_t2; d[4] = (long long)__builtin_readcyclecounter();
  }
#endif
#endif
}

}

bool halo_supported(const IGemmParams& p, int bm) {
  const int W = p.Wout, HW = p.Hout * p.Wout;
  if (p.c0 % BK || p.c1 % BK || p.c2 % BK) return false;
  if (!(p.ksize == 3 && p.stride == 1 && p.pad == 1 && !p.up && p.Hin == p.Hout && p.Win == p.Wout && W >= 8 && W <= 64 &&
        (W & (W - 1)) == 0 && bm % W == 0))
    return false;
  const int cap = (((bm / 64 + 2) * 66 + bm / 4 - 1) / (bm / 4)) * (bm / 4);
  if (bm <= HW) return HW % bm == 0 && (bm / W + 2) * (W + 2) <= cap;
  return bm % HW == 0 && p.M % bm == 0 && (bm / HW) * (p.Hout + 2) * (W + 2) <= cap;
}

template <int BM, int BN, int WARPS_M, int WARPS_N, int NS>
int launch_halo_cfg(const IGemmParams& p, int splitk, hipStream_t stream) {
  SDMI_CHECK(halo_supported(p, BM), "halo-staged conv tile requested for an unsupported shape");
  const int tiles_m = cdiv(p.M, BM), tiles_n = cdiv(p.N, BN);
  const int nch = (p.c0 + p.c1 + p.c2) / BK;
  const int chunks_per_split = cdiv(nch, splitk);
  const int nsplit = cdiv(nch, chunks_per_split);
  IGemmParams q = p;
  q.splitk = nsplit;
  q.tile_n_fastest = tile_order_n_fastest(p);
  q.splitk_fused = 0;
  slab_layout(q, BM, BN, WARPS_M, WARPS_N, nsplit);
  q.epi_vec = epi_vec_ok(p);
  SDMI_CHECK(splitk_ws_need(p, BM, BN, nsplit) <= p.splitk_ws_floats, "split-K workspace too small");
  SDMI_CHECK((int64_t)p.M < (int64_t)65536 * p.Hout * p.Wout, "fast_div_hw: at most 65535 samples per launch");
  q.magic_hw = div_magic_hw(p.Hout * p.Wout);
  q.magic_w = div_magic(p.Wout);
  q.magic_w2 = div_magic(p.Wout + 2);
  q.log2w = 0;
  while ((1 << q.log2w) < p.Wout) ++q.log2w;
  {
    const int HW = p.Hout * p.Wout;
    q.halo_ipt = BM <= HW ? 1 : BM / HW;
    q.halo_thi = BM <= HW ? BM / p.Wout : p.Hout;
    q.magic_hpi = div_magic((q.halo_thi + 2) * (p.Wout + 2));
    const int tpi = q.halo_thi * p.Wout;
    q.log2_tpi = 0;
    while ((1 << q.log2_tpi) < tpi) ++q.log2_tpi;
    if (q.halo_ipt == 1) q.log2_tpi = 30;
  }
  for (int t = 0; t < p.gn_n; ++t) q.gn_magic[t] = div_magic(p.gn_cpg[t]);
  dim3 grid(tiles_m * tiles_n * nsplit), block(WARPS_M * WARPS_N * 64);
  static const int by_shape = env_int("SDMI_PROF_SHAPES", 0);
  std::string pname = std::string("conv3halo_") + std::to_string(BM) + "x" + std::to_string(BN) + "w" +
                      std::to_string(WARPS_M * WARPS_N) + "s" + std::to_string(NS);
  if (by_shape && prof_enabled())
    pname += "_M" + std::to_string(p.M) + "_N" + std::to_string(p.N) + "_K" + std::to_string(p.K) + "_s" + std::to_string(nsplit);
  const double src_pix = (double)p.B * p.Hin * p.Win;
  ProfScope ps(pname.c_str(), 2.0 * p.M * (double)p.N * p.K,
               src_pix * (p.c0 + p.c1) * 2.0 + (double)p.N * p.K * 2.0 + (double)p.M * p.N * ((p.out_f32 ? 4.0 : 0.0) + (p.out_f16 ? 2.0 : 0.0)) +
                   (p.residual ? (double)p.M * p.N * 4.0 : 0.0),
               stream);
  SDMI_LAUNCH((conv3halo_kernel<BM, BN, WARPS_M, WARPS_N, NS>), grid, block, 0, stream, q, tiles_m, tiles_n, chunks_per_split);
  SDMI_HIP_OK(hipGetLastError());
  ps.end();
  if (nsplit > 1) return launch_splitk_reduce(q, nsplit, stream);
  if (q.ln_out) return launch_layernorm(q.out_f32, q.ln_gamma, q.ln_beta, q.ln_out, q.M, q.N, q.ln_eps, stream);
  return 0;
}

int launch_halo_tile(int tile, const IGemmParams& p, int splitk, hipStream_t stream) {
  switch (tile) {
    case 14: return launch_halo_cfg<256, 64, 4, 2, 5>(p, splitk, stream);
    case 15: return launch_halo_cfg<256, 128, 4, 2, 3>(p, splitk, stream);
    case 16: return launch_halo_cfg<128, 64, 2, 2, 8>(p, splitk, stream);
    case 17: return launch_halo_cfg<128, 128, 2, 2, 5>(p, splitk, stream);
    default: return fail("not a halo-staged conv tile id");
  }
}

}
```

### stable-diffusion_amd/csrc/igemm.hip

```cpp
#include <dlfcn.h>

#include <map>
#include <mutex>
#include <tuple>
#include <vector>

#include "igemm_dev.h"

namespace sdmi {
namespace {

__global__ void __launch_bounds__(256) splitk_reduce_kernel(IGemmParams p, int nsplit, int rows_per_block) {
  __shared__ unsigned long long s_gn[2][32][GN_WORDS];
  const int tx = threadIdx.x & 7, ty = threadIdx.x >> 3;
  const int n = (blockIdx.x * 8 + tx) * 4;
  const int row0 = blockIdx.y * rows_per_block;
  const int HW = p.Hout * p.Wout;
  const bool gn = p.gn_n > 0;
  const bool ncol = n < p.N;
  if (gn) {
    for (int i = threadIdx.x; i < 2 * 32 * GN_WORDS; i += 256) (&s_gn[0][0][0])[i] = 0ull;
    __syncthreads();
  }
  const size_t slab_sz = (size_t)p.M * p.N;
// ... 309 lines not shown
    const bool coop = env_int("SDMI_REDUCE_GN_XCD", SDMI_REDUCE_GN_XCD_DEFAULT) && p.pgn_out && p.pgn_gamma && p.pgn_beta && p.mode == EPI_PLAIN && p.gn_n == 1 &&
                      p.gn_cbase[0] == 0 && p.gn_cpg[0] == p.N / 32 && p.N % 128 == 0 && p.N / 32 >= 16 && p.M == p.B * p.Hout * p.Wout &&
                      (p.Hout * p.Wout) % 32 == 0 && !p.out_f16 && !p.out_lo && !p.ln_out && p.splitk_cnt && p.splitk_cnt_ints >= COOP_BAR_INTS &&
                      quads % 1024 == 0 && quads / 1024 <= 256 && (!p.pgn_keep_f32 || (p.out_f32 && p.ldo % 4 == 0));
    ProfScope pst(coop ? "splitk_reduce_gn" : "splitk_reduce", 0.0, coop ? mn * (4.0 * nsplit + 2.0 + (p.pgn_keep_f32 ? 4.0 : 0.0)) : mn * 4.0 * (nsplit + 1), stream);
    const int rb_env = env_int("SDMI_REDUCE_BLOCK", 256);
    const int rb = (rb_env == 128 || (rb_env == 0 && quads / 256 < 512)) ? 128 : 256;
    if (coop) {
      SDMI_LAUNCH(splitk_reduce_tiled_kernel<true>, dim3((unsigned)(quads / 1024)), dim3(1024), 0, stream, p, nsplit);
      SDMI_HIP_OK(hipGetLastError());
      pst.end();
      if (p.pgn_applied) *p.pgn_applied = 1;
      if (range_check_enabled() && range_scan("GroupNorm fp16 output (split-K reduction)", p.pgn_out, (int64_t)p.M * p.N, stream)) return -1;
      return 0;
    }
    SDMI_LAUNCH(splitk_reduce_tiled_kernel<false>, dim3((unsigned)(quads / rb)), dim3(rb), 0, stream, p, nsplit);
    SDMI_HIP_OK(hipGetLastError());
    pst.end();
    if (p.ln_out) return launch_layernorm(p.out_f32, p.ln_gamma, p.ln_beta, p.ln_out, p.M, p.N, p.ln_eps, stream);
    return 0;
  }
  if (p.mode == EPI_HEADS) {
    const int64_t total_h = (int64_t)p.M * (p.N / 4);
    ProfScope psh("splitk_reduce", 0.0, (double)p.M * p.N * (4.0 * nsplit + 2.0), stream);
    SDMI_LAUNCH(splitk_reduce_heads_kernel, dim3((unsigned)((total_h + 255) / 256)), dim3(256), 0, stream, p, nsplit);
    SDMI_HIP_OK(hipGetLastError());
    return 0;
  }
  const int hw = p.Hout * p.Wout;
  if (p.gn_n > 0) SDMI_CHECK(hw % 32 == 0, "GroupNorm statistics need Hout*Wout % 32 == 0");
  const int rpb = reduce_rows_per_block(p);
  ProfScope ps2("splitk_reduce", 0.0, (double)p.M * p.N * 4.0 * (nsplit + 1), stream);
  SDMI_LAUNCH(splitk_reduce_kernel, dim3((unsigned)cdiv(p.N / 4, 8), (unsigned)cdiv(p.M, rpb)), dim3(256), 0, stream, p, nsplit,
                     rpb);
  SDMI_HIP_OK(hipGetLastError());
  ps2.end();
  if (p.ln_out) return launch_layernorm(p.out_f32, p.ln_gamma, p.ln_beta, p.ln_out, p.M, p.N, p.ln_eps, stream);
  return 0;
}

struct TileCfg { int bm, bn, wm, wn, ns; };
static const TileCfg kTiles[SDMI_NUM_TILES] = {
    {128, 128, 2, 2, 2},
    {128, 64, 2, 2, 2},
    {64, 64, 2, 2, 2},
    {256, 128, 4, 2, 2},
    {128, 64, 2, 2, 3},
    {64, 64, 2, 2, 3},
    {256, 128, 4, 2, 3},
    {128, 128, 2, 2, 3},
    {64, 128, 2, 2, 3},
    {128, 128, 4, 2, 3},
    {64, 64, 2, 2, 4},
    {128, 256, 2, 4, 2},
    {64, 256, 1, 4, 3},
    {256, 64, 4, 1, 3},
    {256, 64, 4, 2, 5},
    {256, 128, 4, 2, 3},
    {128, 64, 2, 2, 8},
    {128, 128, 2, 2, 5},
    {64, 64, 2, 2, 8},
    {64, 128, 2, 2, 6},
    {128, 64, 2, 2, 6},
    {128, 128, 4, 2, 4},
};
static inline bool tile_is_halo(int t) { return t >= 14 && t <= 17; }
static inline bool tile_tn_even(int t) { return (kTiles[t].bn / kTiles[t].wn / 32) % 2 == 0; }

static int launch_tile(int tile, const IGemmParams& p, bool dma, int splitk, hipStream_t stream) {
  if (p.split16) return launch_split16_tile(tile, p, splitk, stream);
  if (igemm_has_half(p)) {
    switch (tile) {
      case 0: case 1: case 2: case 3: case 4: case 5: return launch_generic_tile_h0(tile, p, dma, splitk, stream);
      case 6: case 7: case 8: case 9: case 10: return launch_generic_tile_h1(tile, p, dma, splitk, stream);
      case 11: case 12: case 13: case 18: case 19: case 20: case 21: return launch_generic_tile_h2(tile, p, dma, splitk, stream);
      default: break;
    }
  }
  switch (tile) {
    case 0: case 1: case 2: case 3: case 4: case 5: return launch_generic_tile_g0(tile, p, dma, splitk, stream);
    case 6: case 7: case 8: case 9: case 10: return launch_generic_tile_g1(tile, p, dma, splitk, stream);
    case 11: case 12: case 13: case 18: case 19: case 20: case 21: return launch_generic_tile_g2(tile, p, dma, splitk, stream);
    case 14: case 15: case 16: case 17: return launch_halo_tile(tile, p, splitk, stream);
    default: return fail("unknown igemm tile id");
  }
}

struct TuneKey {
  int M, N, K, ksize, stride, up, mode, splitk_req;
  bool operator<(const TuneKey& o) const {
    return std::tie(M, N, K, ksize, stride, up, mode, splitk_req) <
           std::tie(o.M, o.N, o.K, o.ksize, o.stride, o.up, o.mode, o.splitk_req);
  }
};
struct TuneChoice { int tile, splitk; double us; };
struct TuneRec { TuneKey key; int cand; hipEvent_t e0, e1; };

class Tuner {
 public:
  std::mutex mu;
  std::map<TuneKey, TuneChoice> table;
  bool loaded = false, collecting = false;
  int round = 0;
  std::vector<TuneRec> recs;
  std::map<TuneKey, std::vector<std::pair<TuneChoice, std::vector<float>>>> stats;
  std::vector<hipEvent_t> pool;

  static std::string default_path() {
    if (const char* e = getenv("SDMI_TUNE_FILE")) return e;
    Dl_info info;
    if (dladdr((const void*)&Tuner::default_path, &info) && info.dli_fname) {
      std::string so = info.dli_fname;
      const size_t k = so.find_last_of('/');
      return (k == std::string::npos ? std::string(".") : so.substr(0, k)) + "/tune_gfx950.txt";
    }
    return "tune_gfx950.txt";
  }
  void load_file(const std::string& path) {
    FILE* f = fopen(path.c_str(), "r");
    if (!f) return;
    char line[256];
    while (fgets(line, sizeof line, f)) {
      if (line[0] == '#') continue;
      TuneKey k; TuneChoice c; c.us = 0;
      if (sscanf(line, "%d %d %d %d %d %d %d %d %d %d %lf", &k.M, &k.N, &k.K, &k.ksize, &k.stride, &k.up, &k.mode,
                 &k.splitk_req, &c.tile, &c.splitk, &c.us) >= 10 && c.tile >= 0 && c.tile < SDMI_NUM_TILES && c.splitk >= 1 &&
          c.splitk <= 16)
        table[k] = c;
    }
    fclose(f);
  }
  void ensure_loaded() {
    if (loaded) return;
    loaded = true;
    if (env_int("SDMI_TUNE_DISABLE", 0)) return;
    load_file(default_path());
  }
  hipEvent_t ev() {
    if (!pool.empty()) { hipEvent_t e = pool.back(); pool.pop_back(); return e; }
    hipEvent_t e = nullptr;
    (void)hipEventCreate(&e);
    return e;
  }
};
static Tuner g_tuner;

static std::vector<TuneChoice> tune_candidates(const IGemmParams& p, bool can_split) {
  std::vector<TuneChoice> out;
  const int nkt = igemm_nkt(p);
  static const int splits[] = {1, 2, 3, 4, 5, 6, 8, 10, 12, 16};
  for (int t = 0; t < SDMI_NUM_TILES; ++t) {
    const TileCfg& c = kTiles[t];
    if (tile_is_halo(t) && !halo_supported(p, c.bm)) continue;
    if (p.split16 && !split16_tile_supported(t)) continue;
    if (!p.split16 && ((c.ns == 2 && t != 11 && !tile_is_halo(t)) || t == 12 || t == 13)) continue;
    if (p.mode == EPI_GEGLU && !tile_tn_even(t)) continue;
    if (p.lnp_out && (p.M % c.bm || p.N % c.bn || (p.Hout * p.Wout) % c.bm)) continue;
    const long blocks = (long)cdiv(p.M, c.bm) * cdiv(p.N, c.bn);
    if ((long)c.bm > 2L * p.M && c.bm > 64) continue;
    if ((long)c.bn > 2L * p.N && c.bn > 64) continue;
    for (int sk : splits) {
      if ((sk == 5 || sk == 10) && !tile_is_halo(t)) continue;
      if (sk > 1) {
        if (p.splitk != 0 || !can_split) break;
        if (nkt / sk < 4) break;
        if (tile_is_halo(t) && (nkt / 9) % sk != 0) continue;
        if (blocks * (sk / 2 + 1) > 1536) break;
        if (splitk_ws_need(p, c.bm, c.bn, sk) > p.splitk_ws_floats) break;
      }
      if (blocks * sk < 48 && sk < 16 && nkt / (sk * 2) >= 4 && can_split && p.splitk == 0) continue;
      out.push_back({t, p.splitk > 1 ? p.splitk : sk, 0.0});
      if (p.splitk != 0) break;
    }
  }
  if (out.empty()) out.push_back({5, p.splitk > 0 ? p.splitk : 1, 0.0});
  return out;
}

int tune_begin() {
  std::lock_guard<std::mutex> lk(g_tuner.mu);
  g_tuner.ensure_loaded();
  g_tuner.collecting = true; g_tuner.round = 0;
  g_tuner.recs.clear(); g_tuner.stats.clear();
  return 0;
}
int tune_round(int r) {
  std::lock_guard<std::mutex> lk(g_tuner.mu);
  g_tuner.round = r;
  return 0;
}
static int tune_drain() {
  for (auto& r : g_tuner.recs) {
    float ms = 0.f;
    SDMI_HIP_OK(hipEventSynchronize(r.e1));
    SDMI_HIP_OK(hipEventElapsedTime(&ms, r.e0, r.e1));
    auto& v = g_tuner.stats[r.key];
    if ((int)v.size() > r.cand) v[r.cand].second.push_back(ms * 1e3f);
    g_tuner.pool.push_back(r.e0); g_tuner.pool.push_back(r.e1);
  }
  g_tuner.recs.clear();
  return 0;
}
bool tune_collecting() { return g_tuner.collecting; }
static uint64_t g_tune_generation = 0;
uint64_t tune_generation() { return g_tune_generation; }
int tune_end(const char* path, int* n_keys) {
  std::lock_guard<std::mutex> lk(g_tuner.mu);
  if (!g_tuner.collecting) return fail("sdmi_tune_end without sdmi_tune_begin");
  if (tune_drain()) return -1;
  g_tuner.collecting = false;
  auto score = [](std::vector<float> v) -> double {
    if (v.empty()) return 1e30;
    std::sort(v.begin(), v.end());
    return v.size() % 2 ? v[v.size() / 2] : 0.5 * (v[v.size() / 2 - 1] + v[v.size() / 2]);
  };
  for (auto& kv : g_tuner.stats) {
    double best = 1e30; const TuneChoice* bc = nullptr;
    for (auto& c : kv.second) {
      const double sc = score(c.second);
      if (sc < best) { best = sc; bc = &c.first; }
    }
    if (bc) g_tuner.table[kv.first] = {bc->tile, bc->splitk, best};
  }
  if (n_keys) *n_keys = (int)g_tuner.stats.size();
  ++g_tune_generation;
  const std::string out = (path && *path) ? std::string(path) : Tuner::default_path();
  FILE* f = fopen(out.c_str(), "w");
  if (!f) return fail("cannot write the tuning table to " + out);
  fprintf(f, "# libsdmi igemm tuning table (gfx950), measured in situ by tools/tune.py -- M N K ksize stride up mode splitk_req tile splitk us\n");
  for (auto& kv : g_tuner.table) {
    const TuneKey& k = kv.first;
    fprintf(f, "%d %d %d %d %d %d %d %d %d %d %.2f\n", k.M, k.N, k.K, k.ksize, k.stride, k.up, k.mode, k.splitk_req, kv.second.tile,
            kv.second.splitk, kv.second.us);
  }
  fclose(f);
  return 0;
}
int tune_dump(std::string* out) {
  std::lock_guard<std::mutex> lk(g_tuner.mu);
  char buf[256];
  for (auto& kv : g_tuner.stats) {
    const TuneKey& k = kv.first;
    for (auto& c : kv.second) {
      if (c.second.empty()) continue;
      std::vector<float> v = c.second;
      std::sort(v.begin(), v.end());
      snprintf(buf, sizeof buf, "%d %d %d %d %d %d %d %d | %d %d %.2f %.2f %d\n", k.M, k.N, k.K, k.ksize, k.stride, k.up, k.mode,
               k.splitk_req, c.first.tile, c.first.splitk, (double)v[v.size() / 2], (double)v[0], (int)v.size());
      *out += buf;
    }
  }
  return 0;
}

int launch_igemm(const IGemmParams& p, const IGemmTune& tune, hipStream_t stream) {
  SDMI_CHECK(p.M > 0 && p.N > 0 && p.K > 0, "empty GEMM");
  SDMI_CHECK(p.ksize == 1 || p.ksize == 3, "ksize must be 1 or 3");
  const int Cin = p.c0 + p.c1 + p.c2;
  SDMI_CHECK(p.K == p.ksize * p.ksize * Cin, "K != ksize^2 * (c0 + c1 + c2)");
  SDMI_CHECK(p.c0 % BKH == 0 && p.c1 % BKH == 0 && p.c2 % BKH == 0 && p.c0 > 0, "channel counts of every A source must be multiples of 32");
  SDMI_CHECK((p.c2 == 0 || p.c1 > 0), "third A source without a second");
  SDMI_CHECK(p.lda0 % 8 == 0 && (p.a1 == nullptr || p.lda1 % 8 == 0), "A row pitch must be a multiple of 8 halves");
  SDMI_CHECK(p.zero_page != nullptr, "zero page missing");
  SDMI_CHECK(p.M == p.B * p.Hout * p.Wout, "M != B * Hout * Wout");
  SDMI_CHECK(p.c1 == 0 || p.a1 != nullptr, "second A source missing");
  SDMI_CHECK(p.c2 == 0 || (p.a2 != nullptr && p.lda2 % 8 == 0), "third A source missing");
  SDMI_CHECK((p.c1 == 0 || p.lda1 == p.lda0) && (p.c2 == 0 || p.lda2 == p.lda0), "all A sources must share one row pitch");
  SDMI_CHECK(!p.up || (p.ksize == 3 && p.stride == 1), "upsample folding needs a 3x3 stride-1 conv");
  if (p.mode == EPI_GEGLU) SDMI_CHECK(p.N % 64 == 0 && p.out_f16 != nullptr, "GEGLU needs N % 64 == 0 and an fp16 output");
  if (p.ln_out)
    SDMI_CHECK(p.mode == EPI_PLAIN && p.out_f32 && p.ldo == p.N && p.N % 4 == 0 && p.N <= 2560 && p.ln_gamma && p.ln_beta,
               "LayerNorm post-op needs plain mode, an fp32 output with ldo == N <= 2560, gamma and beta");
  if (p.out_lo) SDMI_CHECK(p.mode == EPI_PLAIN && p.ldo % 4 == 0, "out_lo needs plain mode");
  if (p.lnp_out || p.f16_scale)
    SDMI_CHECK(p.mode == EPI_PLAIN && p.out_f32 && p.out_f16 && !p.out_lo && !p.ln_out && p.N % 64 == 0 && p.M % 64 == 0 &&
                   (p.Hout * p.Wout) % 64 == 0 && p.splitk == 1 && epi_vec_ok(p),
               "LayerNorm row statistics: plain mode, fp32 + fp16 outputs, no split-K, M / N / rows per sample multiples of 64, 16-byte aligned rows");
  if (p.lnf_part)
    SDMI_CHECK(p.ksize == 1 && p.c1 == 0 && p.c2 == 0 && !p.split16 && p.lnf_npart * 32 == p.K && p.lnf_cs && p.lnf_d && !p.bias &&
                   p.splitk == 1 && p.lnf_npart <= 40,
               "LayerNorm-folding GEMM: dense, one source, K = 32 * lnf_npart <= 1280, column sums + offsets, no bias, no split-K");
  if (p.gn_n) {
    SDMI_CHECK(p.mode == EPI_PLAIN && p.gn_n <= 2 && (p.Hout * p.Wout) % 32 == 0, "GroupNorm statistics need plain mode and Hout*Wout % 32 == 0");
    SDMI_CHECK(p.N % 4 == 0, "GroupNorm statistics: N % 4 == 0");
    for (int t = 0; t < p.gn_n; ++t)
      SDMI_CHECK(p.gn_acc[t] && p.gn_cpg[t] >= 2 && (p.gn_cbase[t] + p.N + p.gn_cpg[t] - 1) / p.gn_cpg[t] <= 32, "bad GroupNorm statistics target");
  }
  if (p.mode == EPI_HEADS) SDMI_CHECK(p.segC > 0 && p.dh > 0 && p.N % p.segC == 0 && p.N / p.segC <= 3, "bad head scatter");

  SDMI_CHECK((int64_t)p.B * p.Hin * p.Win * p.lda0 * 2 + (int64_t)(p.Win + 1) * p.lda0 * 2 < ((int64_t)1 << 31) - 65536 &&
                 (int64_t)p.N * p.K * 2 < ((int64_t)1 << 31) - 65536,
             "tensor too large for 31-bit byte offsets (buffer addressing)");
  static const int env_dma = env_int("SDMI_IGEMM_DMA", 1);
  static const int env_tile = env_int("SDMI_IGEMM_TILE", -1);
  const bool dma = (tune.dma >= 0 ? tune.dma : env_dma) != 0;
  int tile = tune.tile >= 0 ? tune.tile : env_tile;
  SDMI_CHECK(tile < SDMI_NUM_TILES, "unknown igemm tile id");
  int splitk = p.splitk;
  const int nkt = igemm_nkt(p);
  static const int env_split = env_int("SDMI_SPLITK", -1);
  const bool can_split_plain = p.mode == EPI_PLAIN && p.splitk_ws && p.N % 4 == 0 && p.ldo % 4 == 0 &&
                               (p.residual == nullptr || p.ldr % 4 == 0);
  const bool can_split_heads = p.mode == EPI_HEADS && p.splitk_ws && p.dh % 4 == 0 && p.segC % 4 == 0;
  const bool can_split = can_split_plain || can_split_heads;
  if (env_split >= 0 && splitk == 0) splitk = env_split;

  hipEvent_t ev0 = nullptr, ev1 = nullptr;
  TuneKey tkey{p.M, p.N, nkt * BK, p.split16 ? 11 : p.ksize, p.stride, p.up, p.mode, splitk};
  int tcand = -1;
  if (tile < 0) {
    std::lock_guard<std::mutex> lk(g_tuner.mu);
    g_tuner.ensure_loaded();
    static const int only_ksize = env_int("SDMI_TUNE_ONLY_KSIZE", -1);
    if (g_tuner.collecting && (only_ksize < 0 || tkey.ksize == only_ksize)) {
      IGemmParams q = p; q.splitk = splitk;
      const std::vector<TuneChoice> cands = tune_candidates(q, can_split);
      auto& st = g_tuner.stats[tkey];
      if (st.empty()) for (auto& c : cands) st.push_back({c, {}});
      tcand = g_tuner.round % (int)cands.size();
      tile = cands[tcand].tile; splitk = cands[tcand].splitk;
      ev0 = g_tuner.ev(); ev1 = g_tuner.ev();
    } else {
      auto it = g_tuner.table.find(tkey);
      if (it != g_tuner.table.end()) {
        const int tt = it->second.tile, sk = it->second.splitk;
        const bool halo = tile_is_halo(tt);
        const bool ws_ok = sk == 1 || (can_split && splitk_ws_need(p, kTiles[tt].bm, kTiles[tt].bn, sk) <= p.splitk_ws_floats);
        const bool split_ok = splitk != 0 ? (sk == splitk && ws_ok)
                                          : (sk == 1 || (ws_ok && nkt / sk >= 4 && (halo || (sk != 5 && sk != 10)) &&
                                                         (!halo || (nkt / 9) % sk == 0)));
        if (split_ok && (p.mode != EPI_GEGLU || tile_tn_even(tt)) && (!halo || halo_supported(p, kTiles[tt].bm)) &&
            (!p.split16 || split16_tile_supported(tt))) {
          tile = tt; splitk = sk;
        }
      }
    }
  }
  if (p.mode == EPI_GEGLU && tile >= 0 && !tile_tn_even(tile)) tile = 0;
  if (p.split16) {
    if (tile >= 0) SDMI_CHECK(split16_tile_supported(tile), "split-fp16 GEMM: tile id without an instantiation");
    else tile = 5;
  }
  if (tile < 0) {
    const double gflop = 2.0 * p.M * (double)p.N * p.K * 1e-9;
    if (p.mode == EPI_GEGLU) tile = 0;
    else if (p.mode == EPI_HEADS) tile = 2;
    else tile = gflop >= 25.0 ? 3 : 5;
  }
  if (p.lnp_out) {
    const int hw = p.Hout * p.Wout;
    if (p.M % kTiles[tile].bm || p.N % kTiles[tile].bn || hw % kTiles[tile].bm || (p.split16 && !split16_tile_supported(tile))) tile = 5;
  }
  if (splitk <= 0) {
    splitk = 1;
    if (can_split) {
      const long blocks = (long)cdiv(p.M, kTiles[tile].bm) * cdiv(p.N, kTiles[tile].bn);
      const long want = (kTiles[tile].wm * kTiles[tile].wn == 8) ? 160 : 512;
      while (blocks * splitk < want && nkt / (splitk * 2) >= 8 && splitk < 16 &&
             splitk_ws_need(p, kTiles[tile].bm, kTiles[tile].bn, splitk * 2) <= p.splitk_ws_floats)
        splitk *= 2;
    }
  }
  if (splitk > 1) {
    SDMI_CHECK(can_split, "split-K needs plain or head-scatter mode, a slab workspace and N / ldo / ldr multiples of 4");
    SDMI_CHECK(splitk_ws_need(p, kTiles[tile].bm, kTiles[tile].bn, splitk) <= p.splitk_ws_floats, "split-K workspace too small");
  }
  if (ev0) SDMI_HIP_OK(hipEventRecord(ev0, stream));
#ifdef SDMI_IGEMM_TIMING
  static const char* dbg_path = getenv("SDMI_IGEMM_TIMING");
  static const int dbg_abl = env_int("SDMI_EPI_ABL", 0);
  static long long* dbg_buf = nullptr;
  constexpr int DBG_WG = 16384;
  IGemmParams pd = p;
  pd.dbg_abl = dbg_abl;
  if (dbg_path) {
    if (!dbg_buf) SDMI_HIP_OK(hipMalloc((void**)&dbg_buf, 6 * DBG_WG * sizeof(long long)));
    SDMI_HIP_OK(hipMemsetAsync(dbg_buf, 0, 6 * DBG_WG * sizeof(long long), stream));
    pd.dbg_times = dbg_buf;
  }
  const int rc = launch_tile(tile, pd, dma, splitk, stream);
  if (dbg_path && pd.dbg_times && rc == 0) {
    SDMI_HIP_OK(hipStreamSynchronize(stream));
    std::vector<long long> h(6 * DBG_WG);
    SDMI_HIP_OK(hipMemcpy(h.data(), dbg_buf, h.size() * sizeof(long long), hipMemcpyDeviceToHost));
    std::vector<long long> pro, loop, epi, sto, start;
    long long tmin = 0, tmax = 0;
    for (int b = 0; b < DBG_WG; ++b) {
      const long long* d = &h[6 * b];
      if (d[4] == 0) continue;
      pro.push_back(d[1] - d[0]); loop.push_back(d[2] - d[1]); epi.push_back(d[4] - d[2]);
      sto.push_back(d[3] ? d[3] - d[2] : d[4] - d[2]);
      if (start.empty() || d[0] < tmin) tmin = d[0];
      if (d[4] > tmax) tmax = d[4];
      start.push_back(d[0]);
    }
    if (!pro.empty()) {
      auto med = [](std::vector<long long>& v) { std::sort(v.begin(), v.end()); return v[v.size() / 2]; };
      auto mx = [](std::vector<long long>& v) { return *std::max_element(v.begin(), v.end()); };
      long long late = 0;
      for (long long t : start) late = std::max(late, t - tmin);
      if (FILE* f = fopen(dbg_path, "a")) {
        const int nkt_split = (p.K / BK + std::max(splitk, 1) - 1) / std::max(splitk, 1);
        fprintf(f, "M%d N%d K%d k%d mode%d tile%d split%d res%d gn%d blocks%zu k-tiles/block %d | shader cycles: span %lld last-start %lld | median prologue %lld loop %lld epilogue %lld (stores %lld) | max loop %lld max epi %lld | loop cycles per k-tile %.1f\n",
                p.M, p.N, p.K, p.ksize, p.mode, tile, splitk, p.residual ? 1 : 0, p.gn_n, pro.size(), nkt_split, tmax - tmin, late, med(pro), med(loop),
                med(epi), med(sto), mx(loop), mx(epi), (double)med(loop) / nkt_split);
        fclose(f);
      }
    }
  }
#else
  const int rc = launch_tile(tile, p, dma, splitk, stream);
#endif
  if (rc == 0 && range_check_enabled()) {
    const char* what = p.mode == EPI_GEGLU ? "igemm GEGLU output" : (p.mode == EPI_HEADS ? "igemm q/k/v^T" : "igemm fp16 output");
    if (p.mode == EPI_HEADS) {
      for (int sg = 0; sg < p.N / p.segC; ++sg)
        if (range_scan(what, p.seg_dst[sg], p.seg_kind[sg] == 0 ? (int64_t)p.M * p.segC : (int64_t)p.B * p.segC * p.ntok_pad, stream)) return -1;
    } else if (p.out_f16) {
      if (range_scan(what, p.out_f16, (int64_t)(p.M - 1) * p.ldo + (p.mode == EPI_GEGLU ? p.N / 2 : p.N), stream)) return -1;
    }
    if (p.ln_out && range_scan("LayerNorm output", p.ln_out, (int64_t)p.M * p.N, stream)) return -1;
  }
  if (ev0) {
    SDMI_HIP_OK(hipEventRecord(ev1, stream));
    std::lock_guard<std::mutex> lk(g_tuner.mu);
    g_tuner.recs.push_back({tkey, tcand, ev0, ev1});
  }
  return rc;
}

}
```

### stable-diffusion_amd/csrc/unet.cpp

```cpp
#include "unet.h"

extern "C" char** environ;
#include "prof.h"
#include "split16.h"

#include <math.h>
#include <stdio.h>
#include <string.h>

#include <algorithm>

namespace sdmi {

static bool in_list(const int* v, int n, int x) {
  for (int i = 0; i < n; ++i)
    if (v[i] == x) return true;
  return false;
}

void UNet::expect(const std::string& key, std::vector<int64_t> shape, WKind kind, void** dst, int row0, int ld,
                  void** dst2) {
  WeightSlot s;
  s.key = key; s.shape = std::move(shape); s.kind = kind; s.dst = dst; s.row0 = row0; s.ld = ld; s.dst2 = dst2;
  slot_index_[key] = (int)slots_.size();
// ... 286 lines not shown
  return 0;
}

size_t UNet::slot_bytes(const WeightSlot& s) const {
  size_t numel = 1;
  for (int64_t d : s.shape) numel *= (size_t)d;
  switch (s.kind) {
    case W_F32: case W_CONV_OUT: case W_GEGLU_B: case W_QKV_LEGACY_B: return numel * sizeof(float);
    case W_QKV_LEGACY: return numel * sizeof(f16) * (s.ld ? 3 : 1);
    case W_F32_ROWS: return (size_t)emb_total_ * s.ld * sizeof(float);
    case W_CONV: case W_GEGLU_W: return numel * sizeof(f16);
    case W_SPLIT3: case W_CONV_SPLIT3: return 3 * numel * sizeof(f16);
    case W_SPLIT3_ROWS: case W_ROWS16: {
      size_t total_rows = (size_t)s.shape[0];
      if (s.key.find(".attn1.to_") != std::string::npos && s.key.find("to_out") == std::string::npos) total_rows *= 3;
      if (s.key.find(".attn2.to_k") != std::string::npos || s.key.find(".attn2.to_v") != std::string::npos) total_rows *= 2;
      return total_rows * s.ld * sizeof(f16) * (s.kind == W_SPLIT3_ROWS ? 3 : 1);
    }
  }
  return 0;
}

int UNet::set_weight(const char* key, const float* ptr, const int64_t* shape, int ndim, hipStream_t stream) {
  auto it = slot_index_.find(key);
  if (it == slot_index_.end()) return fail(std::string("unexpected weight key: ") + key);
  WeightSlot& s = slots_[it->second];
  SDMI_CHECK((int)s.shape.size() == ndim, std::string("rank mismatch for ") + key);
  int64_t numel = 1;
  for (int i = 0; i < ndim; ++i) {
    SDMI_CHECK(shape[i] == s.shape[i], std::string("shape mismatch for ") + key);
    numel *= shape[i];
  }
  DevStage st;
  if (st.acquire(ptr, numel, stream)) return -1;
  const float* dptr = st.dptr;
  int rc = 0;
  switch (s.kind) {
    case W_F32:
      rc = dev_alloc(s.dst, slot_bytes(s));
      if (!rc) SDMI_HIP_OK(hipMemcpyAsync(*s.dst, dptr, numel * sizeof(float), hipMemcpyDeviceToDevice, stream));
      break;
    case W_F32_ROWS: {
      rc = dev_alloc(s.dst, slot_bytes(s));
      if (!rc)
        SDMI_HIP_OK(hipMemcpyAsync((float*)*s.dst + (size_t)s.row0 * s.ld, dptr, numel * sizeof(float),
                                   hipMemcpyDeviceToDevice, stream));
      break;
    }
    case W_CONV:
      rc = dev_alloc(s.dst, slot_bytes(s));
      if (!rc) rc = launch_pack_conv_weight(dptr, (f16*)*s.dst, (int)shape[0], (int)shape[1], (int)shape[2], (int)shape[3], stream);
      break;
    case W_SPLIT3:
      rc = dev_alloc(s.dst, slot_bytes(s));
      if (!rc) rc = launch_pack_split3(dptr, (f16*)*s.dst, (int)shape[0], (int)shape[1], stream);
      break;
    case W_CONV_SPLIT3:
      rc = dev_alloc(s.dst, slot_bytes(s));
      if (!rc) rc = launch_pack_conv_split3(dptr, (f16*)*s.dst, (int)shape[0], (int)shape[1], (int)shape[2], (int)shape[3], stream);
      break;
    case W_SPLIT3_ROWS:
      rc = dev_alloc(s.dst, slot_bytes(s));
      if (!rc) rc = launch_pack_split3(dptr, (f16*)*s.dst + (size_t)s.row0 * 3 * s.ld, (int)shape[0], (int)shape[1], stream);
      break;
    case W_CONV_OUT:
      rc = dev_alloc(s.dst, slot_bytes(s));
      if (!rc) rc = launch_pack_conv_out(dptr, (float*)*s.dst, (int)shape[0], (int)shape[1], stream);
      break;
    case W_ROWS16: {
      const int rows = (int)shape[0];
      rc = dev_alloc(s.dst, slot_bytes(s));
      if (!rc) rc = launch_pack_rows(dptr, (f16*)*s.dst, rows, (int)shape[1], s.row0, s.ld, stream);
      break;
    }
    case W_QKV_LEGACY:
    case W_QKV_LEGACY_B: {
      const int R = (int)shape[0], K = s.kind == W_QKV_LEGACY ? (int)shape[1] : 1, heads = s.row0, C = R / 3, d = C / heads;
      float* perm = nullptr;
      rc = dev_alloc(s.dst, slot_bytes(s));
      if (!rc && s.kind == W_QKV_LEGACY) SDMI_HIP_OK(hipMalloc((void**)&perm, (size_t)R * K * sizeof(float)));
      float* dst = s.kind == W_QKV_LEGACY ? perm : (float*)*s.dst;
      for (int h = 0; !rc && h < heads; ++h)
        for (int j = 0; j < 3; ++j)
          SDMI_HIP_OK(hipMemcpyAsync(dst + ((size_t)j * C + (size_t)h * d) * K, dptr + ((size_t)h * 3 * d + (size_t)j * d) * K,
                                     (size_t)d * K * sizeof(float), hipMemcpyDeviceToDevice, stream));
      if (!rc && s.kind == W_QKV_LEGACY)
        rc = s.ld ? launch_pack_split3(perm, (f16*)*s.dst, R, K, stream) : launch_pack_rows(perm, (f16*)*s.dst, R, K, 0, K, stream);
      if (perm) {
        SDMI_HIP_OK(hipStreamSynchronize(stream));
        (void)hipFree(perm);
      }
      break;
    }
    case W_GEGLU_W: {
      rc = dev_alloc(s.dst, slot_bytes(s));
      if (!rc) rc = launch_pack_geglu(dptr, nullptr, (f16*)*s.dst, nullptr, (int)shape[0], (int)shape[1], stream);
      break;
    }
    case W_GEGLU_B: {
      rc = dev_alloc(s.dst, slot_bytes(s));
      if (!rc) {
        f16* tmp = nullptr;
        SDMI_HIP_OK(hipMalloc((void**)&tmp, numel * sizeof(f16)));
        rc = launch_pack_geglu(dptr, dptr, tmp, (float*)*s.dst, (int)shape[0], 1, stream);
        SDMI_HIP_OK(hipStreamSynchronize(stream));
        (void)hipFree(tmp);
      }
      break;
    }
  }
  if (st.release(stream)) return -1;
  if (rc) return rc;
  s.set = true;
  ++weights_gen_;
  finalized_ = false;
  ctx_valid_ = false;
  drop_timestep_table();
  return 0;
}

int UNet::finalize() {
  for (auto& s : slots_)
    if (!s.set) return fail("weight not set: " + s.key);
  if (!zero_) {
    SDMI_HIP_OK(hipMalloc((void**)&zero_, 4096));
    owned_.push_back(zero_);
    SDMI_HIP_OK(hipMemset(zero_, 0, 4096));
  }
  if (reserve_ctx_cache(8, 77)) return -1;
  {
    SDMI_HIP_OK(hipDeviceSynchronize());
    auto each = [&](Layer& L) -> int {
      if (L.kind != L_ATTN || full()) return 0;
      const int C = L.cin;
      for (auto& T : L.tb) {
        const int n_[3] = {3 * C, C, 8 * C};
        const f16* w_[3] = {T.wqkv, T.wq2, T.wgg};
        const float* b_[3] = {nullptr, nullptr, T.bgg};
        for (int i = 0; i < 3; ++i) {
          if (dev_alloc((void**)&T.lnf[2 * i], (size_t)n_[i] * sizeof(float)) || dev_alloc((void**)&T.lnf[2 * i + 1], (size_t)n_[i] * sizeof(float)))
            return -1;
          if (launch_ln_fold_prep(w_[i], n_[i], C, C, T.ln[2 * i], T.ln[2 * i + 1], b_[i], T.lnf[2 * i], T.lnf[2 * i + 1], nullptr)) return -1;
        }
        if (ff_tail_supported(C, 32, 32)) {
          if (dev_alloc((void**)&T.lnf_csd, (size_t)16 * C * sizeof(float))) return -1;
          for (int h = 0; h < 4; ++h) {
            SDMI_HIP_OK(hipMemcpyAsync(T.lnf_csd + (size_t)h * 4 * C, T.lnf[4] + (size_t)h * 2 * C, (size_t)2 * C * sizeof(float), hipMemcpyDeviceToDevice, nullptr));
            SDMI_HIP_OK(hipMemcpyAsync(T.lnf_csd + (size_t)h * 4 * C + 2 * C, T.lnf[5] + (size_t)h * 2 * C, (size_t)2 * C * sizeof(float), hipMemcpyDeviceToDevice, nullptr));
          }
        }
      }
      return 0;
    };
    for (auto& blk : input_blocks_) for (auto& L : blk) if (each(L)) return -1;
    for (auto& L : middle_) if (each(L)) return -1;
    for (auto& blk : output_blocks_) for (auto& L : blk) if (each(L)) return -1;
    SDMI_HIP_OK(hipDeviceSynchronize());
  }
  ++weights_gen_;
  finalized_ = true;
  return 0;
}

namespace {
struct PackedHeader {
  char magic[8];
  int32_t abi, precise_1x1, n_buffers, reserved;
  sdmi_unet_cfg cfg;
  int64_t total_bytes;
};
constexpr int64_t PK_ALIGN = 256;
constexpr int PK_NHC_SHIFT = 16;
constexpr int32_t PK_NHC_MASK = 0xfff << PK_NHC_SHIFT;
constexpr int32_t PK_FULL = 4;
}

int UNet::packed_layout(std::vector<std::pair<void**, size_t>>* bufs, int64_t* total) const {
  std::vector<void**> seen;
  int64_t off = (int64_t)round_up((int64_t)sizeof(PackedHeader), PK_ALIGN);
  for (const auto& s : slots_) {
    if (std::find(seen.begin(), seen.end(), s.dst) != seen.end()) continue;
    seen.push_back(s.dst);
    const size_t b = slot_bytes(s);
    if (bufs) bufs->push_back({s.dst, b});
    off += (int64_t)round_up((int64_t)b, PK_ALIGN);
  }
  *total = off;
  return 0;
}

int UNet::export_packed(void* host_buf, int64_t bytes, hipStream_t stream) {
  SDMI_CHECK(finalized_, "export needs a finalized handle");
  std::vector<std::pair<void**, size_t>> bufs;
  int64_t total = 0;
  packed_layout(&bufs, &total);
  SDMI_CHECK(host_buf && bytes >= total, "packed buffer too small: need " + std::to_string(total) + " bytes");
  PackedHeader h{};
  memcpy(h.magic, "SDMIPK01", 8);
  h.abi = SDMI_ABI_VERSION; h.precise_1x1 = precise_1x1_ ? 1 : 0; h.n_buffers = (int32_t)bufs.size(); h.cfg = cfg_;
  h.reserved = (precise_kv_ ? 1 : 0) | (precise_last_res_ ? 2 : 0) | (precise_1x1_max_ds_ << 8);
  h.reserved |= (ext_.attention_block << 4) | (ext_.resblock_updown << 5) | ((scale_shift_ ? 1 : 0) << 6);
  h.reserved |= num_head_channels_ << PK_NHC_SHIFT;
  if (full()) h.reserved |= PK_FULL;
  h.total_bytes = total;
  memcpy(host_buf, &h, sizeof(h));
  int64_t off = (int64_t)round_up((int64_t)sizeof(PackedHeader), PK_ALIGN);
  for (auto& b : bufs) {
    SDMI_HIP_OK(hipMemcpyAsync((char*)host_buf + off, *b.first, b.second, hipMemcpyDeviceToHost, stream));
    off += (int64_t)round_up((int64_t)b.second, PK_ALIGN);
  }
  SDMI_HIP_OK(hipStreamSynchronize(stream));
  return 0;
}

int UNet::import_packed(const void* host_buf, int64_t bytes, hipStream_t stream) {
  SDMI_CHECK(host_buf && bytes >= (int64_t)sizeof(PackedHeader), "packed blob truncated");
  PackedHeader h;
  memcpy(&h, host_buf, sizeof(h));
  SDMI_CHECK(memcmp(h.magic, "SDMIPK01", 8) == 0, "not a libsdmi packed-weight blob");
  SDMI_CHECK(h.abi == SDMI_ABI_VERSION, "packed blob was written by a different ABI version: repack it");
  SDMI_CHECK(memcmp(&h.cfg, &cfg_, sizeof(cfg_)) == 0, "packed blob was written for a different UNet configuration");
  SDMI_CHECK(((h.reserved & PK_FULL) != 0) == full(), std::string("packed blob was written by a ") +
             ((h.reserved & PK_FULL) ? "full" : "mixed") + "-precision UNet handle and cannot be imported into a " + (full() ? "full" : "mixed") +
             "-precision one: repack it with a handle of this precision");
  SDMI_CHECK((h.precise_1x1 != 0) == precise_1x1_, "packed blob was written with a different precision allocation (split-fp16 1x1 convs)");
  SDMI_CHECK((h.reserved & (7 << 4)) == ((ext_.attention_block << 4) | (ext_.resblock_updown << 5) | ((scale_shift_ ? 1 : 0) << 6)),
             "packed blob was written for a different UNet family (attention_block / resblock_updown / scale-shift norm)");
  SDMI_CHECK(((h.reserved & PK_NHC_MASK) >> PK_NHC_SHIFT) == num_head_channels_,
             "packed blob was written for num_head_channels " + std::to_string((h.reserved & PK_NHC_MASK) >> PK_NHC_SHIFT) + ", this handle has " +
             std::to_string(num_head_channels_) + ": repack it");
  SDMI_CHECK((h.reserved & ~PK_FULL & ~(7 << 4) & ~PK_NHC_MASK) == ((precise_kv_ ? 1 : 0) | (precise_last_res_ ? 2 : 0) | (precise_1x1_max_ds_ << 8)),
             "packed blob was written with a different precision allocation (context K / V, last ResBlock, 1x1 conv levels)");
  std::vector<std::pair<void**, size_t>> bufs;
  int64_t total = 0;
  packed_layout(&bufs, &total);
  SDMI_CHECK(h.n_buffers == (int32_t)bufs.size() && h.total_bytes == total && bytes >= total, "packed blob truncated or inconsistent");
  int64_t off = (int64_t)round_up((int64_t)sizeof(PackedHeader), PK_ALIGN);
  for (auto& b : bufs) {
    if (dev_alloc(b.first, b.second)) return -1;
    SDMI_HIP_OK(hipMemcpyAsync(*b.first, (const char*)host_buf + off, b.second, hipMemcpyHostToDevice, stream));
    off += (int64_t)round_up((int64_t)b.second, PK_ALIGN);
  }
  SDMI_HIP_OK(hipStreamSynchronize(stream));
  for (auto& s : slots_) s.set = true;
  ctx_valid_ = false;
  drop_timestep_table();
  return finalize();
}

struct Fwd : FwdBase {
  UNet* u; int Lctx;
  bool ln_fold_on = false;
  bool ff_tail_on = false;
  bool st_head_on = false;
  bool st_mid_on = false;
  bool st_tail_on = false;
  bool st_mid_ctx_on = false;
  bool ctx1_on = false;
  bool gn_conv_on = false;
  float* emb_all = nullptr;
  int emb_ld = 0;
  bool emb_caller = false;
  const f16* ctx16 = nullptr;
  const f16* ctx16_lo = nullptr;

  Act res_block(Layer& L, const Act& x0, const Act* x1) {
    const int H = x0.H, W = x0.W, M = B * H * W;
    const int Cin = x0.C + (x1 ? x1->C : 0), Cout = L.cout;
    if (Cin != L.cin) { ok(fail("res block channel mismatch at " + L.prefix)); }
    if (Cin == Cout && x1) ok(fail("identity skip with a concatenated input at " + L.prefix));
    const size_t mark = scratch.off;
    f16* raw = (Cin != Cout) ? S<f16>((size_t)M * Cin) : nullptr;
    const bool p1 = L.p1x1;
    const bool p3 = L.precise3;
    f16* raw_lo = (Cin != Cout && p1) ? S<f16>((size_t)M * Cin) : nullptr;
    auto split3 = [&](IGemmParams& q, const f16* hi, const f16* lo, int C) {
      q.a0 = hi; q.c0 = C; q.lda0 = C; q.a1 = lo; q.c1 = C; q.lda1 = C; q.a2 = hi; q.c2 = C; q.lda2 = C; q.K = 27 * C; q.k_alg = 9 * C;
    };
    float* h = S<float>((size_t)M * Cout);
    Act out = make_act(P<float>((size_t)M * Cout), Cout, H, W, true);
    Act hact = make_act(h, Cout, H, W, true);
    f16* a2 = nullptr;
    int& gn2_applied = u->gn2_applied_;
    gn2_applied = 0;
    const bool ss = u->scale_shift_;
    const float* const film = ss ? emb_all + L.emb_off : nullptr;
    const bool gc1 = gn_conv_on && !ss && !p3 && Cin == Cout && gn_conv3_supported(B, H, W, x0.C, x1 ? x1->C : 0, Cout);
    const bool gc2 = gn_conv_on && !ss && !p3 && gn_conv3_supported(B, H, W, Cout, 0, Cout);
    auto gn_conv = [&](const Act& a0, const Act* a1, const float* gamma, const float* beta, const f16* w, IGemmParams& e) {
      GnConvParams g = GnConvParams();
      g.gn_acc = groupnorm(a0, a1, gamma, beta, 1e-5f, 1, nullptr, nullptr, nullptr, nullptr, nullptr, true);
      g.x0 = a0.p; g.c0 = a0.C; g.x1 = a1 ? a1->p : nullptr; g.c1 = a1 ? a1->C : 0;
      g.gn_gamma = gamma; g.gn_beta = beta; g.gn_eps = 1e-5f; g.w = w; g.epi = e;
      if (!dry && !rc) ok(launch_gn_conv3(g, s));
    };
    if (gc1) {
      IGemmParams p = conv3(nullptr, Cin, H, W, H, W, 1, 0, L.w16[0], Cout);
      p.bias = L.f32[2]; p.rowvec = emb_all + L.emb_off; p.ld_rowvec = emb_ld;
      p.out_f32 = h; p.ldo = Cout;
      attach_gn_targets(p, hact);
      TapeCaller tc(Tape::R_EMB, emb_caller ? p.rowvec : nullptr);
      gn_conv(x0, x1, L.f32[0], L.f32[1], L.w16[0], p);
    } else {
      f16* a = S<f16>((size_t)M * Cin);
      f16* a_lo = p3 ? S<f16>((size_t)M * Cin) : nullptr;
      groupnorm(x0, x1, L.f32[0], L.f32[1], 1e-5f, 1, a, nullptr, raw, a_lo, raw_lo);
      IGemmParams p = conv3(a, Cin, H, W, H, W, 1, 0, L.w16[0], Cout);
      if (p3) split3(p, a, a_lo, Cin);
      p.bias = L.f32[2];
      if (!ss) { p.rowvec = emb_all + L.emb_off; p.ld_rowvec = emb_ld; }
      p.out_f32 = h; p.ldo = Cout;
      attach_gn_targets(p, hact);
      if (!gc2 && !p3 && !ss) {
        a2 = S<f16>((size_t)M * Cout);
        p.pgn_gamma = L.f32[3]; p.pgn_beta = L.f32[4]; p.pgn_eps = 1e-5f; p.pgn_silu = 1; p.pgn_out = a2; p.pgn_applied = &gn2_applied;
      }
      TapeCaller tc(Tape::R_EMB, emb_caller ? p.rowvec : nullptr);
      gemm(p);
    }
    const float* residual = x0.p;
    if (Cin != Cout) {
      IGemmParams p = dense1x1(raw, raw_lo, M, Cin, L.w16[2], Cout, H * W, p1);
      p.bias = L.f32[6]; p.out_f32 = out.p; p.ldo = Cout;
      gemm(p);
      residual = out.p;
    }
    if (gc2) {
      IGemmParams p = conv3(nullptr, Cout, H, W, H, W, 1, 0, L.w16[1], Cout);
      p.bias = L.f32[5]; p.residual = residual; p.ldr = Cout; p.out_f32 = out.p; p.ldo = Cout;
      attach_gn_targets(p, out);
      attach_f16_copy(p, out);
      gn_conv(hact, nullptr, L.f32[3], L.f32[4], L.w16[1], p);
    } else {
      f16* a2_lo = nullptr;
      if (p3) { a2 = S<f16>((size_t)M * Cout); a2_lo = S<f16>((size_t)M * Cout); }
      if (ss && !a2) a2 = S<f16>((size_t)M * Cout);
      {
        TapeCaller tc(Tape::R_EMB, emb_caller ? film : nullptr);
        groupnorm(hact, nullptr, L.f32[3], L.f32[4], 1e-5f, 1, a2, nullptr, nullptr, a2_lo, nullptr, false, gn2_applied != 0, film, emb_ld);
      }
      IGemmParams p = conv3(a2, Cout, H, W, H, W, 1, 0, L.w16[1], Cout);
      if (p3) split3(p, a2, a2_lo, Cout);
      p.bias = L.f32[5]; p.residual = residual; p.ldr = Cout; p.out_f32 = out.p; p.ldo = Cout;
      attach_gn_targets(p, out);
      attach_f16_copy(p, out);
      gemm(p);
    }
    scratch.off = mark;
    return out;
  }

  void context_kv(Layer& L, int d) {
    TBlock& T = L.tb[d];
    const int C = L.cin, Lp = (int)round_up(Lctx, 8);
    const int CD = u->cfg_.context_dim;
    IGemmParams p = dense(ctx16, B * Lctx, CD, T.wkv2, 2 * C, Lctx);
    if (ctx16_lo) {
      p.a1 = ctx16_lo; p.c1 = CD; p.lda1 = CD; p.a2 = ctx16; p.c2 = CD; p.lda2 = CD; p.K = 3 * CD; p.k_alg = CD;
    }
    if (u->full()) {
      const size_t mark = scratch.off;
      float* kv = S<float>((size_t)B * Lctx * 2 * C);
      p.out_f32 = kv; p.ldo = 2 * C;
      gemm(p);
      if (!dry && !rc) ok(launch_split_heads(kv, 2 * C, 0, T.ck, T.ck_lo, 0, B, Lctx, Lp, L.heads, L.dh, s));
      if (!dry && !rc) ok(launch_split_heads(kv, 2 * C, C, T.cvt, T.cvt_lo, 1, B, Lctx, Lp, L.heads, L.dh, s));
      scratch.off = mark;
      return;
    }
    p.mode = EPI_HEADS; p.seg_dst[0] = T.ck; p.seg_dst[1] = T.cvt; p.seg_kind[0] = 0; p.seg_kind[1] = 1;
    p.heads = L.heads; p.dh = L.dh; p.ntok = Lctx; p.ntok_pad = Lp; p.segC = C; p.splitk = 1;
    if (!dry && !rc && Lp != Lctx) {
      hipError_t e = memset_async(T.cvt, 0, (size_t)B * C * Lp * sizeof(f16), s);
      if (e != hipSuccess) ok(fail(std::string("hipMemsetAsync: ") + hipGetErrorString(e)));
    }
    gemm(p);
  }

  Act attn_block_full(Layer& L, const Act& x) {
    const int H = x.H, W = x.W, N = H * W, M = B * N, C = L.cin;
    const int Np = (int)round_up(N, 8), Lp = (int)round_up(Lctx, 8);
    const float scale = 1.0f / sqrtf((float)L.dh);
    const size_t mark = scratch.off;
    f16* a = S<f16>((size_t)M * C); f16* a_lo = S<f16>((size_t)M * C);
    float* t = S<float>((size_t)M * C);
    float* y = S<float>((size_t)M * 8 * C);
    f16* q = S<f16>((size_t)M * C); f16* q_lo = S<f16>((size_t)M * C);
    f16* k = S<f16>((size_t)M * C); f16* k_lo = S<f16>((size_t)M * C);
    f16* vt = S<f16>((size_t)B * C * Np); f16* vt_lo = S<f16>((size_t)B * C * Np);
    f16* gg = S<f16>((size_t)M * 4 * C); f16* gg_lo = S<f16>((size_t)M * 4 * C);
    auto linear = [&](const f16* hi, const f16* lo, int K, const f16* w, int n_out, const float* bias, float* out, bool residual) {
      IGemmParams p = dense1x1(hi, lo, M, K, w, n_out, N, true);
      p.bias = bias; p.out_f32 = out; p.ldo = n_out;
      if (residual) { p.residual = out; p.ldr = n_out; }
      gemm(p);
    };
    auto layernorm = [&](const float* gamma, const float* beta) {
      if (!dry && !rc) ok(launch_layernorm_split(t, gamma, beta, a, a_lo, M, C, 1e-5f, s));
    };
    auto heads = [&](const float* src, int ld, int col0, f16* dst, f16* dst_lo, int kind) {
      if (!dry && !rc) ok(launch_split_heads(src, ld, col0, dst, dst_lo, kind, B, N, Np, L.heads, L.dh, s));
    };
    auto attend = [&](const f16* kk, const f16* kk_lo, const f16* v, const f16* v_lo, int nkv, int nkv_pad) {
      AttnSplitParams p = AttnSplitParams();
      p.q = q; p.q_lo = q_lo; p.k = kk; p.k_lo = kk_lo; p.vt = v; p.vt_lo = v_lo; p.out = a; p.out_lo = a_lo;
      p.BH = B * L.heads; p.heads = L.heads; p.nq = N; p.nkv = nkv; p.nkv_pad = nkv_pad; p.d = L.dh; p.scale = scale;
      if (!dry && !rc) ok(launch_attention_split16(p, s));
    };
    groupnorm(x, nullptr, L.f32[0], L.f32[1], 1e-6f, 0, a, nullptr, nullptr, a_lo, nullptr);
    linear(a, a_lo, C, L.w16[0], C, L.f32[2], t, false);
    for (auto& T : L.tb) {
      layernorm(T.ln[0], T.ln[1]);
      linear(a, a_lo, C, T.wqkv, 3 * C, nullptr, y, false);
      heads(y, 3 * C, 0, q, q_lo, 0); heads(y, 3 * C, C, k, k_lo, 0); heads(y, 3 * C, 2 * C, vt, vt_lo, 1);
      attend(k, k_lo, vt, vt_lo, N, Np);
      linear(a, a_lo, C, T.wo1, C, T.bo1, t, true);
      layernorm(T.ln[2], T.ln[3]);
      if (ctx16) context_kv(L, (int)(&T - L.tb.data()));
      linear(a, a_lo, C, T.wq2, C, nullptr, y, false);
      heads(y, C, 0, q, q_lo, 0);
      attend(T.ck, T.ck_lo, T.cvt, T.cvt_lo, Lctx, Lp);
      linear(a, a_lo, C, T.wo2, C, T.bo2, t, true);
      layernorm(T.ln[4], T.ln[5]);
      linear(a, a_lo, C, T.wgg, 8 * C, T.bgg, y, false);
      if (!dry && !rc) ok(launch_geglu_split(y, M, 4 * C, gg, gg_lo, s));
      linear(gg, gg_lo, 4 * C, T.wff2, C, T.bff2, t, true);
    }
    if (!dry && !rc) ok(launch_cast_f16(t, a, a_lo, (int64_t)M * C, s));
    Act out = make_act(P<float>((size_t)M * C), C, H, W, true);
    {
      IGemmParams p = dense1x1(a, a_lo, M, C, L.w16[1], C, N, true);
      p.bias = L.f32[3]; p.residual = x.p; p.ldr = C; p.out_f32 = out.p; p.ldo = C;
      attach_gn_targets(p, out);
      gemm(p);
    }
    scratch.off = mark;
    return out;
  }

  Act attn_block(Layer& L, const Act& x) {
    if (u->full()) return attn_block_full(L, x);
    const int H = x.H, W = x.W, N = H * W, M = B * N, C = L.cin;
    const int Np = (int)round_up(N, 8), Lp = (int)round_up(Lctx, 8);
    const float scale = 1.0f / sqrtf((float)L.dh);
    const size_t mark = scratch.off;
    f16* xn = S<f16>((size_t)M * C);
    const bool p1 = L.p1x1;
    f16* xn_lo = p1 ? S<f16>((size_t)M * C) : nullptr;
    const bool fold_ln = ln_fold_on && C % 64 == 0 && C <= 1280 && N % 64 == 0 && M % 64 == 0 && M >= u->ln_fold_min_rows_;
    const bool chain_head = st_head_on && fold_ln && p1 && L.tb[0].lnf[0] != nullptr &&
                            st_head_supported(C, M, N, Np, L.heads, L.dh) && dense1x1(nullptr, nullptr, M, C, L.w16[0], C, N, p1).split16;
    long long* gn_stats = nullptr;
    if (chain_head) gn_stats = groupnorm(x, nullptr, L.f32[0], L.f32[1], 1e-6f, 0, nullptr, nullptr, nullptr, nullptr, nullptr, true);
    else groupnorm(x, nullptr, L.f32[0], L.f32[1], 1e-6f, 0, xn, nullptr, nullptr, xn_lo, nullptr);
    float* t = S<float>((size_t)M * C);
    f16* ln = S<f16>((size_t)M * C);
    f16* q = S<f16>((size_t)M * C);
    f16* k = S<f16>((size_t)M * C);
    f16* vt = S<f16>((size_t)B * C * Np);
    f16* ao = S<f16>((size_t)M * C);
    f16* gg = S<f16>((size_t)M * 4 * C);
    float* lnp = fold_ln ? S<float>((size_t)(C / 32) * M * 2) : nullptr;
    auto with_ln = [&](IGemmParams& p, const float* gamma, const float* beta) {
      if (fold_ln) { p.out_f16 = ln; p.f16_scale = gamma; p.lnp_out = lnp; p.splitk = 1; }
      else { p.ln_gamma = gamma; p.ln_beta = beta; p.ln_out = ln; p.ln_eps = 1e-5f; }
    };
    auto fold_in = [&](IGemmParams& p, const float* cs, const float* dn) {
      if (!fold_ln) return;
      p.lnf_part = lnp; p.lnf_npart = C / 32; p.lnf_eps = 1e-5f; p.lnf_cs = cs; p.lnf_d = dn; p.bias = nullptr;
    };
    if (chain_head) {
      TBlock& T = L.tb[0];
      StHeadParams h = StHeadParams();
      h.x = x.p; h.gn_acc = gn_stats; h.gn_gamma = L.f32[0]; h.gn_beta = L.f32[1]; h.gn_eps = 1e-6f;
      h.w_in = L.w16[0]; h.b_in = L.f32[2]; h.t = t; h.ln_gamma = T.ln[0]; h.ln_eps = 1e-5f;
      h.wqkv = T.wqkv; h.lnf_cs = T.lnf[0]; h.lnf_d = T.lnf[1]; h.q = q; h.k = k; h.vt = vt;
      h.M = M; h.B = B; h.ntok = N; h.ntok_pad = Np; h.heads = L.heads; h.dh = L.dh; h.C = C;
      if (!dry && !rc && Np != N) {
        hipError_t e = memset_async(vt, 0, (size_t)B * C * Np * sizeof(f16), s);
        if (e != hipSuccess) ok(fail(std::string("hipMemsetAsync: ") + hipGetErrorString(e)));
      }
      if (!dry && !rc) ok(launch_st_head(h, s));
    } else {
      IGemmParams p = dense1x1(xn, xn_lo, M, C, L.w16[0], C, N, p1);
      p.bias = L.f32[2]; p.out_f32 = t; p.ldo = C;
      with_ln(p, L.tb[0].ln[0], L.tb[0].ln[1]);
      gemm(p);
    }
    const int depth = (int)L.tb.size();
    const bool chain_ff = ff_tail_on && fold_ln && p1 && depth == 1 && L.tb[0].lnf_csd != nullptr && ff_tail_supported(C, M, N) &&
                          dense1x1(nullptr, nullptr, M, C, L.w16[1], C, N, p1).split16;
    const bool chain_tail = chain_ff && st_tail_on;
    for (int d = 0; d < depth; ++d) {
      TBlock& T = L.tb[d];
      if (!(chain_head && d == 0)) {
        IGemmParams p = dense(ln, M, C, T.wqkv, 3 * C, N);
// ... 256 lines not shown
  for (auto& blk : input_blocks_) for (auto& L : blk) if (each(L)) return -1;
  for (auto& L : middle_) if (each(L)) return -1;
  for (auto& blk : output_blocks_) for (auto& L : blk) if (each(L)) return -1;
  ctx_cap_ = need; ctx_B_ = 0; ctx_L_ = 0; ctx_valid_ = false;
  return 0;
}

int UNet::ensure_ctx_cache(int B, int Lctx, bool may_grow) {
  if (ctx_B_ == B && ctx_L_ == Lctx) return 0;
  const int64_t need = (int64_t)B * round_up(Lctx, 8);
  if (need > ctx_cap_) {
    if (may_grow) { if (reserve_ctx_cache(B, Lctx)) return -1; }
    else return fail("context of " + std::to_string(B) + " x " + std::to_string(Lctx) + " tokens exceeds the reserved K/V capacity (" +
                     std::to_string(ctx_cap_) + " padded rows): call sdmi_unet_reserve_context(h, B, Lctx) once, outside the sampling loop");
  }
  ctx_B_ = B; ctx_L_ = Lctx; ctx_valid_ = false;
  return 0;
}

int UNet::cache_timesteps(const int64_t* t_host, int n, hipStream_t stream) {
  SDMI_CHECK(finalized_, "sdmi_unet_finalize() has not succeeded yet");
  SDMI_CHECK(n >= 0 && n <= 4096 && (n == 0 || t_host != nullptr), "bad timestep list");
  drop_timestep_table();
  if (n == 0) return 0;
  const int mc = cfg_.model_channels;
  const size_t row = (size_t)emb_total_, tmp = (size_t)8 * (mc + 2 * (size_t)te_);
  const size_t need = (size_t)n * row + tmp;
  if (need > emb_tab_floats_) {
    if (emb_tab_) (void)hipFree(emb_tab_);
    emb_tab_ = nullptr; emb_tab_floats_ = 0;
    SDMI_HIP_OK(hipMalloc((void**)&emb_tab_, need * sizeof(float)));
    emb_tab_floats_ = need;
  }
  if ((size_t)n > emb_tab_tcap_) {
    if (emb_tab_tdev_) (void)hipFree(emb_tab_tdev_);
    emb_tab_tdev_ = nullptr; emb_tab_tcap_ = 0;
    SDMI_HIP_OK(hipMalloc((void**)&emb_tab_tdev_, (size_t)n * sizeof(int64_t)));
    emb_tab_tcap_ = (size_t)n;
  }
  std::vector<int64_t> host(t_host, t_host + n);
  emb_tab_src_.swap(host);
  SDMI_HIP_OK(hipMemcpyAsync(emb_tab_tdev_, emb_tab_src_.data(), (size_t)n * sizeof(int64_t), hipMemcpyHostToDevice, stream));
  float* temb = emb_tab_ + (size_t)n * row;
  float* e1 = temb + (size_t)8 * mc;
  float* emb = e1 + (size_t)8 * te_;
  for (int i0 = 0; i0 < n; i0 += 8) {
    const int nb = std::min(8, n - i0);
    int r = launch_timestep_embedding(emb_tab_tdev_ + i0, nullptr, temb, nb, mc, stream);
    if (!r) r = launch_small_linear(temb, mc, te_w0_, te_b0_, e1, te_, nb, te_, mc, 0, stream);
    if (!r) r = launch_small_linear(e1, te_, te_w2_, te_b2_, emb, te_, nb, te_, te_, 1, stream);
    if (!r) r = launch_small_linear(emb, te_, emb_w_, emb_b_, emb_tab_ + (size_t)i0 * row, emb_total_, nb, emb_total_, te_, 1, stream);
    if (r) return r;
  }
  emb_tab_t_ = emb_tab_src_;
  return 0;
}

int UNet::hint_timestep(int64_t t) {
  emb_hint_row_ = -1;
  for (size_t i = 0; i < emb_tab_t_.size(); ++i)
    if (emb_tab_t_[i] == t) { emb_hint_row_ = (int)i; break; }
  return 0;
}

int UNet::run(const float* x, const int64_t* t_i64, const float* t_f32, const float* ctx, float* eps_out, int B, int H,
              int W, int Lctx, void* workspace, int64_t ws_bytes, hipStream_t stream, bool dry, bool ctx_only,
              int64_t* bytes_needed) {
  SDMI_CHECK(dry || finalized_, "sdmi_unet_finalize() has not succeeded yet");
  SDMI_CHECK(B >= 1 && B <= 8, "batch (CFG rows) must be 1..8 per call");
  if (has_ctx()) SDMI_CHECK(H >= 1 && W >= 1 && Lctx >= 1, "bad shape");
  else SDMI_CHECK(H >= 1 && W >= 1 && Lctx == 0 && ctx == nullptr && !ctx_only,
                  "bad shape: this UNet has no cross-attention (AttentionBlocks): pass ctx = NULL and Lctx = 0");
  const int down = 1 << (cfg_.n_levels - 1);
  if (ext_.resblock_updown)
    SDMI_CHECK(H % down == 0 && W % down == 0, "latent H and W must be multiples of " + std::to_string(down) +
               " for resblock_updown (the down ResBlocks' avg_pool2d rounds down, the skip concat needs the sizes back)");
  SDMI_CHECK(H % down == 0 && W % down == 0, "H and W must be divisible by 2^(levels-1) (the UNet's skip concat requires it)");

  const int hint_row = emb_hint_row_;
  if (!dry && !ctx_only) emb_hint_row_ = -1;

  const char* e_rp = getenv("SDMI_REPLAY"); const char* e_rv = getenv("SDMI_REPLAY_VERIFY");
  const bool replay_on = !(e_rp && atoi(e_rp) == 0);
  const bool replay_verify = e_rv && atoi(e_rv) != 0;
  const bool hinted = t_i64 != nullptr && hint_row >= 0 && hint_row < (int)emb_tab_t_.size();
  auto in_ws = [&](const void* p, size_t bytes) {
    return p && (uintptr_t)p < (uintptr_t)workspace + (uint64_t)ws_bytes && (uintptr_t)workspace < (uintptr_t)p + bytes;
  };
  const size_t img = (size_t)B * H * W * sizeof(float);
  const bool tape_ok = replay_on && !dry && !ctx_only && !prof_enabled() && !tune_collecting() && !range_check_enabled() &&
                       workspace != nullptr && (t_i64 || t_f32) && !in_ws(x, img * cfg_.in_channels) && !in_ws(eps_out, img * cfg_.out_channels) &&
                       !in_ws(t_i64 ? (const void*)t_i64 : t_f32, (size_t)B * (t_i64 ? 8 : 4)) &&
                       !in_ws(ctx, (size_t)B * Lctx * cfg_.context_dim * sizeof(float));
  TapeKey tkey;
  uintptr_t caller[Tape::R_COUNT] = {0, 0, 0, 0, 0};
  Tape* rec = nullptr;
  std::unique_ptr<Tape> verify_against;
  if (tape_ok) {
    tkey.B = B; tkey.H = H; tkey.W = W; tkey.Lctx = Lctx; tkey.mode = hinted ? 0 : (t_i64 ? 1 : 2);
    tkey.ws = workspace; tkey.ws_bytes = ws_bytes; tkey.have_ctx = ctx != nullptr;
    tkey.env = sdmi_env_hash() ^ (tune_generation() * 0x9e3779b97f4a7c15ull); tkey.weights_gen = weights_gen_; tkey.ctx_gen = ctx_gen_;
    auto low4 = [](const void* p, int shift) { return (unsigned)((uintptr_t)p & 15) << shift; };
    tkey.align = low4(x, 0) | low4(eps_out, 4) | low4(ctx, 8) | low4(t_i64 ? (const void*)t_i64 : t_f32, 12);
    caller[Tape::R_X] = (uintptr_t)x; caller[Tape::R_OUT] = (uintptr_t)eps_out;
    caller[Tape::R_T] = hinted ? 0 : (t_i64 ? (uintptr_t)t_i64 : (uintptr_t)t_f32);
    caller[Tape::R_CTX] = (uintptr_t)ctx;
    caller[Tape::R_EMB] = hinted ? (uintptr_t)(emb_tab_ + (size_t)hint_row * emb_total_) : 0;
    for (size_t i = 0; i < tapes_.size(); ++i) {
      if (!(tapes_[i].first == tkey)) continue;
      std::unique_ptr<Tape> hit = std::move(tapes_[i].second);
      tapes_.erase(tapes_.begin() + (long)i);
      SDMI_CHECK(finalized_, "sdmi_unet_finalize() has not succeeded yet");
      if (ensure_ctx_cache(B, Lctx, false)) return -1;
      if (!ctx && has_ctx()) SDMI_CHECK(ctx_valid_, "ctx == NULL but no cached context for this (B, Lctx); call sdmi_unet_cache_context first");
      hit->retarget(caller);
      if (replay_verify) { verify_against = std::move(hit); break; }
      const int e = hit->replay(stream);
      const bool sets = hit->sets_ctx_valid;
      const int64_t need = hit->bytes_needed;
      tapes_.emplace_back(tkey, std::move(hit));
      if (e) return fail(std::string("launch tape replay: ") + hipGetErrorString((hipError_t)e));
      if (sets) ctx_valid_ = true;
      if (bytes_needed) *bytes_needed = need;
      ++tape_hits_;
      return 0;
    }
  }
  std::unique_ptr<Tape> fresh;
  if (tape_ok) {
    fresh.reset(new Tape());
    memcpy(fresh->caller, caller, sizeof(caller));
    rec = fresh.get();
  }

  Fwd f;
  f.u = this; f.s = stream; f.dry = dry; f.B = B; f.Lctx = Lctx; f.zero = zero_; f.precise_1x1 = precise_1x1_;
  {
    const char* e_fold = getenv("SDMI_LN_FOLD"); const char* e_vec = getenv("SDMI_EPI_VEC");
    f.ln_fold_on = (e_fold ? atoi(e_fold) != 0 : ln_fold_) && !(e_vec && atoi(e_vec) == 0);
    const char* e_ff = getenv("SDMI_FF_TAIL");
    f.ff_tail_on = e_ff ? atoi(e_ff) != 0 : ff_tail_;
    const char* e_sh = getenv("SDMI_ST_HEAD");
    f.st_head_on = e_sh ? atoi(e_sh) != 0 : st_head_;
    const char* e_sm = getenv("SDMI_ST_MID");
    f.st_mid_on = e_sm ? atoi(e_sm) != 0 : st_head_;
    const char* e_st = getenv("SDMI_ST_TAIL");
    f.st_tail_on = e_st ? atoi(e_st) != 0 : ff_tail_;
    const char* e_mc = getenv("SDMI_ST_MID_CTX");
    f.st_mid_ctx_on = e_mc ? atoi(e_mc) != 0 : st_head_;
    const char* e_c1 = getenv("SDMI_CTX1");
    f.ctx1_on = !(e_c1 && atoi(e_c1) == 0);
    const char* e_gc = getenv("SDMI_GN_CONV");
    f.gn_conv_on = e_gc ? atoi(e_gc) != 0 : false;
    if (full()) {
      f.ln_fold_on = f.ff_tail_on = f.st_head_on = f.st_mid_on = f.st_tail_on = f.st_mid_ctx_on = f.gn_conv_on = false;
    }
  }
  int64_t persist_bytes = 0, scratch_bytes = 0;
  for (int pass = (dry ? 0 : 0); pass < 2; ++pass) {
    const bool d = (pass == 0) ? true : false;
    if (pass == 1 && dry) break;
    f.dry = d; f.rc = 0;
    f.n_acts = 0;
    TapeRecGuard tape_guard(d ? nullptr : rec);
    f.plan = fuse_gn_stats_ ? &gn_plan_ : nullptr;
    if (d) gn_plan_.clear();
    f.persist = Arena(); f.scratch = Arena();
    f.persist.dry = f.scratch.dry = d;
    if (!d) {
      SDMI_CHECK(persist_bytes + scratch_bytes <= ws_bytes, "workspace too small: need " +
                 std::to_string(persist_bytes + scratch_bytes) + " bytes, got " + std::to_string(ws_bytes));
      SDMI_CHECK(workspace != nullptr, "workspace is NULL");
      f.persist.base = (char*)workspace; f.persist.cap = (size_t)persist_bytes;
      f.scratch.base = (char*)workspace + persist_bytes; f.scratch.cap = (size_t)scratch_bytes;
      if (ensure_ctx_cache(B, Lctx, ctx_only)) return -1;
    }
    const int mc = cfg_.model_channels;
    if (f.begin_pass((int64_t)12 << 20)) return -1;
    f16* ctx16 = f.P<f16>((size_t)B * Lctx * cfg_.context_dim);
    f16* ctx16_lo = precise_kv_ ? f.P<f16>((size_t)B * Lctx * cfg_.context_dim) : nullptr;
    const bool have_ctx = has_ctx() && ((ctx != nullptr) || d);
    if (!has_ctx()) {
      f.ctx16 = nullptr; f.ctx16_lo = nullptr;
    } else if (have_ctx) {
      if (!d) {
        TapeCaller tc(Tape::R_CTX, ctx);
        int r = launch_cast_f16(ctx, ctx16, ctx16_lo, (int64_t)B * Lctx * cfg_.context_dim, stream);
        if (r) return r;
      }
      f.ctx16 = ctx16; f.ctx16_lo = ctx16_lo;
    } else {
      SDMI_CHECK(ctx_valid_, "ctx == NULL but no cached context for this (B, Lctx); call sdmi_unet_cache_context first");
      f.ctx16 = nullptr; f.ctx16_lo = nullptr;
    }
    if (ctx_only) {
      auto each = [&](Layer& L) { if (L.kind == L_ATTN) for (int dd = 0; dd < (int)L.tb.size(); ++dd) f.context_kv(L, dd); };
      for (auto& blk : input_blocks_) for (auto& L : blk) each(L);
      for (auto& L : middle_) each(L);
      for (auto& blk : output_blocks_) for (auto& L : blk) each(L);
    } else {
      float* temb = f.P<float>((size_t)B * mc);
      float* e1 = f.P<float>((size_t)B * te_);
      float* emb = f.P<float>((size_t)B * te_);
      f.emb_all = f.P<float>((size_t)B * emb_total_);
      f.emb_ld = emb_total_;
      if (!d && t_i64 != nullptr && hint_row >= 0 && hint_row < (int)emb_tab_t_.size()) {
        f.emb_all = emb_tab_ + (size_t)hint_row * emb_total_;
        f.emb_ld = 0;
        f.emb_caller = true;
      } else if (!d) {
        int r;
        {
          TapeCaller tc(Tape::R_T, t_i64 ? (const void*)t_i64 : t_f32);
          r = launch_timestep_embedding(t_i64, t_f32, temb, B, mc, stream);
        }
        if (!r) r = launch_small_linear(temb, mc, te_w0_, te_b0_, e1, te_, B, te_, mc, 0, stream);
        if (!r) r = launch_small_linear(e1, te_, te_w2_, te_b2_, emb, te_, B, te_, te_, 1, stream);
        if (!r) r = launch_small_linear(emb, te_, emb_w_, emb_b_, f.emb_all, emb_total_, B, emb_total_, te_, 1, stream);
        if (r) return r;
      }
      std::vector<Act> hs;
      Act h;
      {
        Layer& L = input_blocks_[0][0];
        const char* e_cis = getenv("SDMI_CONV_IN_STATS");
        h = f.make_act(f.P<float>((size_t)B * H * W * mc), mc, H, W, (H * W) % 16 == 0 && !(e_cis && atoi(e_cis) == 0));
        IGemmParams st = IGemmParams();
        f.attach_gn_targets(st, h);
        if (!d) {
          TapeCaller tc(Tape::R_X, x);
          int r = launch_conv_in(x, L.w32[0], L.f32[0], h.p, B, cfg_.in_channels, H, W, mc, stream, st.gn_n, st.gn_acc, st.gn_cpg, st.gn_cbase);
          if (r) return r;
        }
        hs.push_back(h);
      }
      for (size_t bi = 1; bi < input_blocks_.size(); ++bi) {
        for (auto& L : input_blocks_[bi]) h = f.run_layer(L, h, nullptr);
        hs.push_back(h);
      }
      for (auto& L : middle_) h = f.run_layer(L, h, nullptr);
      for (auto& blk : output_blocks_) {
        Act skip = hs.back(); hs.pop_back();
        SDMI_CHECK(skip.H == h.H && skip.W == h.W, "skip/h spatial mismatch");
        bool first = true;
        for (auto& L : blk) { h = f.run_layer(L, h, first ? &skip : nullptr); first = false; }
      }
      float* hn = f.S<float>((size_t)B * H * W * mc);
      f.groupnorm(h, nullptr, out_gamma_, out_beta_, 1e-5f, 1, nullptr, hn, nullptr);
      if (!d && !f.rc) {
        TapeCaller tc(Tape::R_OUT, eps_out);
        int r = launch_conv_out(hn, out_w_, out_b_, eps_out, B, H, W, mc, cfg_.out_channels, stream);
        if (r) return r;
      }
    }
    if (f.rc) return f.rc;
    if (d) { persist_bytes = (int64_t)f.persist.peak + 256; scratch_bytes = (int64_t)f.scratch.peak + 256; }
    else {
      SDMI_CHECK(!f.persist.overflow && !f.scratch.overflow, "internal: arena overflow");
      if (have_ctx) ctx_valid_ = true;
    }
  }
  if (bytes_needed) *bytes_needed = persist_bytes + scratch_bytes;
  if (fresh) {
    if (fresh->broken && !verify_against) {
      static bool noted = false;
      if (!noted) fprintf(stderr, "sdmi: internal: a declared caller pointer (TapeCaller) is in no launch argument; such calls run untaped\n");
      noted = true;
      return 0;
    }
    fresh->bytes_needed = persist_bytes + scratch_bytes;
    fresh->sets_ctx_valid = ctx != nullptr;
    if (verify_against) {
      const Tape& a = *verify_against; const Tape& b = *fresh;
      auto eq3 = [](const dim3& u, const dim3& v) { return u.x == v.x && u.y == v.y && u.z == v.z; };
      bool same = !b.broken && a.ops.size() == b.ops.size() && a.blob == b.blob && a.arg_off == b.arg_off && a.arg_size == b.arg_size &&
                  a.relocs.size() == b.relocs.size();
      for (size_t i = 0; same && i < a.relocs.size(); ++i)
        same = a.relocs[i].off == b.relocs[i].off && a.relocs[i].which == b.relocs[i].which && a.relocs[i].delta == b.relocs[i].delta;
      for (size_t i = 0; same && i < a.ops.size(); ++i) {
        const Tape::Op &p = a.ops[i], &q = b.ops[i];
        same = p.kind == q.kind && p.fn == q.fn && eq3(p.grid, q.grid) && eq3(p.block, q.block) && p.shmem == q.shmem &&
               p.first_arg == q.first_arg && p.nargs == q.nargs && p.ptr == q.ptr && p.value == q.value && p.bytes == q.bytes;
      }
      SDMI_CHECK(same, "SDMI_REPLAY_VERIFY: the retargeted launch tape differs from what the executor launches for this call");
      ++tape_hits_;
    } else {
      ++tape_records_;
    }
    if (tapes_.size() >= kMaxTapes) tapes_.erase(tapes_.begin());
    tapes_.emplace_back(tkey, std::move(fresh));
  }
  return 0;
}

}
```

### stable-diffusion_amd/csrc/unet.h

```cpp
#pragma once
#include <stdlib.h>

#include <map>
#include <memory>
#include <string>
#include <utility>
#include <vector>

#include "../../include/sdmi.h"
#include "common.h"

namespace sdmi {

struct Arena {
  char* base = nullptr; size_t cap = 0, off = 0, peak = 0; bool dry = false; bool overflow = false;
  void* alloc(size_t bytes) {
    const size_t a = (off + 255) & ~(size_t)255;
    off = a + bytes;
    peak = std::max(peak, off);
    if (dry) return (void*)(uintptr_t)(a + 4096);
    if (off > cap) { overflow = true; return base; }
    return base + a;
  }
};
// ... 28 lines not shown
    if (plan && dry && (int)plan->targets.size() < n_acts) plan->targets.resize(n_acts);
    if (plan && dry && (int)plan->want_f16.size() < n_acts) plan->want_f16.resize(n_acts, 0);
    return a;
  }
  std::vector<f16*> f16_of;
  void attach_f16_copy(IGemmParams& p, Act& a) {
    a.can_f16 = plan != nullptr && p.out_f16 == nullptr && p.mode == EPI_PLAIN;
    if (dry || !a.can_f16 || a.id < 0 || a.id >= (int)plan->want_f16.size() || !plan->want_f16[a.id]) return;
    f16* c = P<f16>((size_t)B * a.H * a.W * a.C);
    if ((int)f16_of.size() <= a.id) f16_of.resize(a.id + 1, nullptr);
    f16_of[a.id] = c;
    p.out_f16 = c;
  }
  bool want_f16_copy(const Act& a) {
    if (!dry || !plan || !a.can_f16 || a.id < 0 || a.id >= (int)plan->want_f16.size()) return false;
    if (const char* e = getenv("SDMI_F16_COPY")) { if (atoi(e) == 0) return false; }
    plan->want_f16[a.id] = 1;
    (void)P<f16>((size_t)B * a.H * a.W * a.C);
    return true;
  }
  const f16* f16_copy(const Act& a) const {
    return (!dry && a.id >= 0 && a.id < (int)f16_of.size()) ? f16_of[a.id] : nullptr;
  }
  void attach_gn_targets(IGemmParams& p, const Act& a) {
    p.gn_n = 0;
    if (dry || !plan || !a.stats || a.id < 0 || a.id >= (int)plan->targets.size()) return;
    for (const GnTarget& t : plan->targets[a.id]) {
      if (p.gn_n >= 2) { ok(fail("internal: more than two GroupNorm consumers of one activation")); return; }
      p.gn_acc[p.gn_n] = gn_acc + (size_t)t.gn_idx * gn_acc_words(B);
      p.gn_cpg[p.gn_n] = t.cpg; p.gn_cbase[p.gn_n] = t.cbase;
      ++p.gn_n;
    }
  }

  template <class T> T* P(size_t n) { return (T*)persist.alloc(n * sizeof(T)); }
  template <class T> T* S(size_t n) { return (T*)scratch.alloc(n * sizeof(T)); }
  void ok(int r) { if (r && !rc) rc = r; }
  long long* next_gn_acc() {
    if (gn_calls >= GN_MAX_CALLS) { ok(fail("more GroupNorm calls than accumulator regions")); return gn_acc; }
    return gn_acc + (size_t)(gn_calls++) * gn_acc_words(B);
  }
  long long* last_gn_acc() const { return gn_acc + (size_t)(gn_calls - 1) * gn_acc_words(B); }
  int begin_pass(int64_t splitk_floats, bool with_gn = true) {
    gn_calls = 0;
    gn_acc = nullptr;
    const size_t acc_words = with_gn ? (size_t)GN_MAX_CALLS * gn_acc_words(B) : 0;
    long long* blk = P<long long>(acc_words + SPLITK_CNT_INTS / 2);
    gn_acc = with_gn ? blk : nullptr;
    splitk_cnt = (int*)(blk + acc_words);
    if (!dry) SDMI_HIP_OK(memset_async(blk, 0, (acc_words + SPLITK_CNT_INTS / 2) * sizeof(long long), s));
    splitk_ws_floats = splitk_floats;
    splitk_ws = P<float>((size_t)splitk_floats);
    (void)P<float>((size_t)(splitk_floats / 2));
    return 0;
  }

  void gemm(IGemmParams& p) {
    p.zero_page = zero;
    p.splitk_ws = splitk_ws; p.splitk_ws_floats = splitk_ws_floats;
    p.splitk_cnt = splitk_cnt; p.splitk_cnt_ints = SPLITK_CNT_INTS;
    if (!dry && !rc) ok(launch_igemm(p, IGemmTune(), s));
  }
  IGemmParams dense(const f16* a, int M, int K, const f16* w, int N, int rows_per_batch) {
    IGemmParams p = IGemmParams();
    p.a0 = a; p.c0 = K; p.lda0 = K;
    p.B = M / rows_per_batch; p.Hin = p.Hout = rows_per_batch; p.Win = p.Wout = 1;
    p.ksize = 1; p.w = w; p.M = M; p.N = N; p.K = K; p.splitk = 0;
    return p;
  }
  IGemmParams conv3(const f16* a, int C, int Hin, int Win, int Hout, int Wout, int stride, int up, const f16* w, int N) {
    IGemmParams p = IGemmParams();
    p.a0 = a; p.c0 = C; p.lda0 = C;
    p.B = B; p.Hin = Hin; p.Win = Win; p.Hout = Hout; p.Wout = Wout;
    p.ksize = 3; p.stride = stride; p.up = up; p.w = w; p.M = B * Hout * Wout; p.N = N; p.K = 9 * C; p.splitk = 0;
    return p;
  }
  IGemmParams dense1x1(const f16* hi, const f16* lo, int M, int K, const f16* w, int N, int rows_per_batch, bool precise) {
    IGemmParams p = dense(hi, M, K, w, N, rows_per_batch);
    if (precise) {
      static const bool family = !(getenv("SDMI_SPLIT16_KERNEL") && atoi(getenv("SDMI_SPLIT16_KERNEL")) == 0);
      if (family && K % 32 == 0) {
        p.a1 = lo; p.lda1 = K; p.split16 = 1; p.ldw = 3 * K;
      } else {
        p.a1 = lo; p.c1 = K; p.lda1 = K; p.a2 = hi; p.c2 = K; p.lda2 = K; p.K = 3 * K; p.k_alg = K;
      }
    }
    return p;
  }
  long long* groupnorm(const Act& x0, const Act* x1, const float* gamma, const float* beta, float eps, int silu, f16* o16,
                       float* o32, f16* raw, f16* o16_lo = nullptr, f16* raw_lo = nullptr, bool stats_only = false,
                       bool already_applied = false, const float* film = nullptr, int film_ld = 0) {
    GroupNormParams g = GroupNormParams();
    g.film = film; g.film_ld = film_ld;
    g.x0 = x0.p; g.c0 = x0.C;
    if (x1) { g.x1 = x1->p; g.c1 = x1->C; }
    g.B = B; g.HW = x0.H * x0.W; g.gamma = gamma; g.beta = beta; g.eps = eps; g.silu = silu;
    g.out_f16 = o16; g.out_f32 = o32; g.raw_f16 = raw; g.out_lo = o16_lo; g.raw_lo = raw_lo;
    g.stats_only = stats_only ? 1 : 0;
    const int idx = gn_calls;
    g.acc = next_gn_acc();
    if (plan) {
      const int cpg = (g.c0 + g.c1) / 32;
      if (dry) {
        const bool f = x0.stats && (!x1 || x1->stats) && x0.id >= 0 && (!x1 || x1->id >= 0);
        if ((int)plan->fused.size() <= idx) plan->fused.resize(idx + 1, 0);
        plan->fused[idx] = f ? 1 : 0;
        if (f) {
          plan->targets[x0.id].push_back({idx, 0, cpg});
          if (x1) plan->targets[x1->id].push_back({idx, g.c0, cpg});
        }
      } else {
        g.skip_stats = (idx < (int)plan->fused.size() && plan->fused[idx]) ? 1 : 0;
      }
    }
    if (!dry && !rc && !(stats_only && g.skip_stats) && !already_applied) ok(launch_groupnorm(g, s));
    return g.acc;
  }
};

struct DevStage {
  const float* dptr = nullptr; float* staged = nullptr;
  int acquire(const float* ptr, int64_t numel, hipStream_t stream);
  int release(hipStream_t stream);
};

enum LayerKind { L_CONV_IN, L_RES, L_ATTN, L_DOWN, L_UP, L_ATTN_LEGACY };
enum WKind { W_F32, W_F32_ROWS, W_CONV, W_CONV_OUT, W_ROWS16, W_GEGLU_W, W_GEGLU_B, W_SPLIT3, W_SPLIT3_ROWS, W_CONV_SPLIT3, W_QKV_LEGACY,
             W_QKV_LEGACY_B };

struct TBlock {
  f16* wqkv = nullptr;
  f16* wo1 = nullptr; float* bo1 = nullptr;
  f16* wq2 = nullptr;
  f16* wkv2 = nullptr;
  f16* wo2 = nullptr; float* bo2 = nullptr;
  f16* wgg = nullptr; float* bgg = nullptr;
  f16* wff2 = nullptr; float* bff2 = nullptr;
  float* ln[6] = {nullptr, nullptr, nullptr, nullptr, nullptr, nullptr};
  f16* ck = nullptr; f16* cvt = nullptr;
  f16* ck_lo = nullptr; f16* cvt_lo = nullptr;
  float* lnf[6] = {nullptr, nullptr, nullptr, nullptr, nullptr, nullptr};
  float* lnf_csd = nullptr;
};

struct Layer {
  LayerKind kind = L_RES;
  std::string prefix;
  int cin = 0, cout = 0, heads = 0, dh = 0, emb_off = 0, attn_index = -1;
  int updown = 0;
  bool p1x1 = true, precise3 = false;
  f16* w16[3] = {nullptr, nullptr, nullptr};
  float* w32[1] = {nullptr};
  float* f32[7] = {nullptr, nullptr, nullptr, nullptr, nullptr, nullptr, nullptr};
  std::vector<TBlock> tb;
};

struct WeightSlot {
  std::string key;
  std::vector<int64_t> shape;
  WKind kind = W_F32;
  void** dst = nullptr; int row0 = 0, ld = 0; void** dst2 = nullptr;
  bool set = false;
};

class UNet {
 public:
  UNet() = default;
  ~UNet();
  UNet(const UNet&) = delete;
  UNet& operator=(const UNet&) = delete;

  int build(const sdmi_unet_cfg& cfg, int precision = SDMI_PRECISION_MIXED, const sdmi_unet_ext* ext = nullptr, unsigned flags = 0);
  int set_weight(const char* key, const float* ptr, const int64_t* shape, int ndim, hipStream_t stream);
  int finalize();
  int packed_layout(std::vector<std::pair<void**, size_t>>* bufs, int64_t* total) const;
  int export_packed(void* host_buf, int64_t bytes, hipStream_t stream);
  int import_packed(const void* host_buf, int64_t bytes, hipStream_t stream);
  int run(const float* x, const int64_t* t_i64, const float* t_f32, const float* ctx, float* eps_out, int B, int H, int W,
          int Lctx, void* workspace, int64_t ws_bytes, hipStream_t stream, bool dry, bool ctx_only, int64_t* bytes_needed);

  int cache_timesteps(const int64_t* t_host, int n, hipStream_t stream);
  int reserve_ctx_cache(int B, int Lctx);
  int hint_timestep(int64_t t);

  const std::vector<WeightSlot>& slots() const { return slots_; }

  sdmi_unet_cfg cfg_{};
  sdmi_unet_ext ext_{};
  bool has_ctx() const { return ext_.attention_block == 0; }
  bool scale_shift_ = false;
  int num_head_channels_ = 0;
  int precision_ = SDMI_PRECISION_MIXED;
  bool full() const { return precision_ == SDMI_PRECISION_FULL; }
  int te_ = 0, emb_total_ = 0, n_attn_ = 0;
  f16* zero_ = nullptr;
  bool precise_1x1_ = true;
  bool precise_last_res_ = true;
  int precise_1x1_max_ds_ = 4;
  bool precise_kv_ = true;

 private:
  friend struct Fwd;
  void expect(const std::string& key, std::vector<int64_t> shape, WKind kind, void** dst, int row0 = 0, int ld = 0,
              void** dst2 = nullptr);
  int dev_alloc(void** dst, size_t bytes);
  size_t slot_bytes(const WeightSlot& s) const;
  int ensure_ctx_cache(int B, int Lctx, bool may_grow);
  GnPlan gn_plan_;
  bool fuse_gn_stats_ = true;
  bool ln_fold_ = true; int ln_fold_min_rows_ = 512;
  bool ff_tail_ = true;
  bool st_head_ = true;

  struct TapeKey {
    int B = 0, H = 0, W = 0, Lctx = 0, mode = 0;
    const void* ws = nullptr; int64_t ws_bytes = 0; bool have_ctx = false;
    uint64_t env = 0, weights_gen = 0, ctx_gen = 0;
    unsigned align = 0;
    bool operator==(const TapeKey& o) const {
      return B == o.B && H == o.H && W == o.W && Lctx == o.Lctx && mode == o.mode && ws == o.ws && ws_bytes == o.ws_bytes &&
             have_ctx == o.have_ctx && env == o.env && weights_gen == o.weights_gen && ctx_gen == o.ctx_gen && align == o.align;
    }
  };
  std::vector<std::pair<TapeKey, std::unique_ptr<Tape>>> tapes_;
  static constexpr size_t kMaxTapes = 12;
  uint64_t weights_gen_ = 0, ctx_gen_ = 0;
  int gn2_applied_ = 0;
 public:
  uint64_t tape_hits_ = 0, tape_records_ = 0;
 private:

  std::vector<std::vector<Layer>> input_blocks_, output_blocks_;
  std::vector<Layer> middle_;
  std::vector<WeightSlot> slots_;
  std::map<std::string, int> slot_index_;
  std::vector<void*> owned_;
  float *te_w0_ = nullptr, *te_b0_ = nullptr, *te_w2_ = nullptr, *te_b2_ = nullptr;
  float *emb_w_ = nullptr, *emb_b_ = nullptr;
  float *out_gamma_ = nullptr, *out_beta_ = nullptr, *out_w_ = nullptr, *out_b_ = nullptr;
  bool finalized_ = false;
  int ctx_B_ = 0, ctx_L_ = 0; bool ctx_valid_ = false;
  int64_t ctx_cap_ = 0;
  float* emb_tab_ = nullptr; size_t emb_tab_floats_ = 0;
  int64_t* emb_tab_tdev_ = nullptr; size_t emb_tab_tcap_ = 0;
  std::vector<int64_t> emb_tab_t_;
  std::vector<int64_t> emb_tab_src_;
  int emb_hint_row_ = -1;
  void drop_timestep_table() { emb_tab_t_.clear(); emb_hint_row_ = -1; }
};

}
```

Baseline: 3.794.

## Fold ResBlock 1x1 skip projection into the 3x3 conv as a K-tail

Adds a pointwise K-tail to the halo-staged 3x3 conv kernel. After the 3x3 reduction, the same accumulators take a 1x1 GEMM over the block's input (the skip projection), and the two biases are pre-summed. This removes a separate 1x1 GEMM launch plus the f32 write and re-read of its residual in ResBlocks with channel change. In exchange the conv takes a longer K loop with new split-K boundary logic, is restricted to halo tiles, and loses freedom in tile and split choice.

New measurement: 3.827 (median of 6 runs). No clear change (+0.9%).

```diff
diff --git a/include/sdmi.h b/include/sdmi.h
--- a/include/sdmi.h
+++ b/include/sdmi.h
@@ -178,6 +178,11 @@
   void* out_lo;
 } sdmi_igemm_desc;
 int sdmi_k_igemm(const sdmi_igemm_desc* d, void* stream);
+typedef struct sdmi_igemm_tail {
+  const void* a[3]; int32_t c[3]; int32_t ld;
+  const void* w;
+} sdmi_igemm_tail;
+int sdmi_k_igemm_tail(const sdmi_igemm_desc* d, const sdmi_igemm_tail* t, void* stream);
 int sdmi_k_ff_tail(const sdmi_igemm_desc* proj_out, const void* ln_f16, const float* lnp, float ln_eps, const float* csd,
                    const void* wgg_f16, const void* wff2_f16, const float* bff2, const float* t, void* stream);
 int sdmi_k_st_tail(const sdmi_igemm_desc* proj_out, const void* a_f16, const void* wo_f16, const float* bo, float* t, const float* ln_gamma,
diff --git a/stable-diffusion_amd/_lib.py b/stable-diffusion_amd/_lib.py
--- a/stable-diffusion_amd/_lib.py
+++ b/stable-diffusion_amd/_lib.py
@@ -60,6 +60,10 @@
                 ('pgn_gamma', c_ptr), ('pgn_beta', c_ptr), ('pgn_eps', C.c_float), ('pgn_silu', C.c_int32),
                 ('pgn_out', c_ptr), ('pgn_keep_f32', C.c_int32), ('pgn_applied', C.POINTER(C.c_int32)),
                 ('out_lo', c_ptr)]
+
+
+class IGemmTail(C.Structure):
+    _fields_ = [('a', c_ptr * 3), ('c', C.c_int32 * 3), ('ld', C.c_int32), ('w', c_ptr)]
 
 
 _SIGS = {
@@ -126,6 +130,7 @@
     'sdmi_bert_forward': (C.c_int, [c_ptr, c_ptr, c_ptr, C.c_int, C.c_int, c_ptr, C.c_int64, c_ptr]),
     'sdmi_has_experiments': (C.c_int, []),
     'sdmi_k_igemm': (C.c_int, [C.POINTER(IGemmDesc), c_ptr]),
+    'sdmi_k_igemm_tail': (C.c_int, [C.POINTER(IGemmDesc), C.POINTER(IGemmTail), c_ptr]),
     'sdmi_k_ff_tail': (C.c_int, [C.POINTER(IGemmDesc), c_ptr, c_ptr, C.c_float, c_ptr, c_ptr, c_ptr, c_ptr, c_ptr, c_ptr]),
     'sdmi_k_gn_conv3': (C.c_int, [C.POINTER(IGemmDesc), c_ptr, c_ptr, C.c_int, C.c_int, c_ptr, C.c_int64, c_ptr, c_ptr, C.c_float, c_ptr]),
     'sdmi_k_st_mid_ctx': (C.c_int, [c_ptr, c_ptr, c_ptr, c_ptr, c_ptr, C.c_float, c_ptr, c_ptr, c_ptr, c_ptr, c_ptr, C.c_int, C.c_int, C.c_float, c_ptr,
diff --git a/stable-diffusion_amd/csrc/api.cpp b/stable-diffusion_amd/csrc/api.cpp
--- a/stable-diffusion_amd/csrc/api.cpp
+++ b/stable-diffusion_amd/csrc/api.cpp
@@ -364,6 +364,16 @@
   IGemmTune t; t.tile = d->tile; t.dma = d->dma;
   return launch_igemm(p, t, (hipStream_t)stream);
 }
+int sdmi_k_igemm_tail(const sdmi_igemm_desc* d, const sdmi_igemm_tail* t, void* stream) {
+  SDMI_CHECK(d && t, "null descriptor");
+  IGemmParams p = IGemmParams();
+  if (igemm_params_of(d, p)) return -1;
+  for (int i = 0; i < 3; ++i) { p.pw_a[i] = (const f16*)t->a[i]; p.pw_c[i] = t->c[i]; }
+  p.pw_ld = t->ld; p.pw_w = (const f16*)t->w;
+  SDMI_CHECK(p.pw_a[0] != nullptr, "pointwise tail: first source missing");
+  IGemmTune tn; tn.tile = d->tile; tn.dma = d->dma;
+  return launch_igemm(p, tn, (hipStream_t)stream);
+}
 int sdmi_k_ff_tail(const sdmi_igemm_desc* proj_out, const void* ln_f16, const float* lnp, float ln_eps, const float* csd,
                    const void* wgg_f16, const void* wff2_f16, const float* bff2, const float* t, void* stream) {
   SDMI_CHECK(proj_out, "null descriptor");
diff --git a/stable-diffusion_amd/csrc/common.h b/stable-diffusion_amd/csrc/common.h
--- a/stable-diffusion_amd/csrc/common.h
+++ b/stable-diffusion_amd/csrc/common.h
@@ -173,7 +173,14 @@
   unsigned long long magic_cpg_in = 0;
   int halo_thi = 0, halo_ipt = 1, log2_tpi = 30;
   unsigned long long magic_hpi = 0;
-};
+  const f16* pw_a[3] = {nullptr, nullptr, nullptr};
+  int pw_c[3] = {0, 0, 0};
+  int pw_ld = 0;
+  const f16* pw_w = nullptr;
+  int pw_k_alg = 0;
+  int pw_bnd[17] = {0};
+};
+static inline int igemm_tail_k(const IGemmParams& p) { return p.pw_a[0] ? p.pw_c[0] + p.pw_c[1] + p.pw_c[2] : 0; }
 
 constexpr int SDMI_NUM_TILES = 22;
 struct IGemmTune {
@@ -182,6 +189,7 @@
 };
 
 int launch_igemm(const IGemmParams& p, const IGemmTune& tune, hipStream_t stream);
+bool igemm_tail_ready(const IGemmParams& p);
 bool range_check_enabled();
 uint64_t tune_generation();
 bool tune_collecting();
diff --git a/stable-diffusion_amd/csrc/conv3halo.hip b/stable-diffusion_amd/csrc/conv3halo.hip
--- a/stable-diffusion_amd/csrc/conv3halo.hip
+++ b/stable-diffusion_amd/csrc/conv3halo.hip
@@ -3,7 +3,7 @@
 namespace sdmi {
 namespace {
 
-template <int BM, int BN, int WARPS_M, int WARPS_N, int NS>
+template <int BM, int BN, int WARPS_M, int WARPS_N, int NS, bool TAIL = false>
 __global__ void __launch_bounds__(WARPS_M* WARPS_N * 64) conv3halo_kernel(const IGemmParams p, const int tiles_m,
                                                                            const int tiles_n, const int chunks_per_split) {
 #if defined(__HIP_DEVICE_COMPILE__)
@@ -40,9 +40,17 @@
   else { tile_n = tmn / tiles_m; tile_m = tmn - tile_n * tiles_m; }
   const int m0 = tile_m * BM, n0 = tile_n * BN;
   const int nch = (p.c0 + p.c1 + p.c2) / BK;
-  const int c_begin = split * chunks_per_split;
-  const int c_end = min(nch, c_begin + chunks_per_split);
-  if (c_begin >= c_end) return;
+  int c_begin, c_end, t_begin = 0, t_end = 0;
+  if constexpr (TAIL) {
+    const int kb = p.pw_bnd[split], ke = p.pw_bnd[split + 1], seam = nch * 9;
+    c_begin = min(kb, seam) / 9; c_end = min(ke, seam) / 9;
+    t_begin = max(kb, seam) - seam; t_end = max(ke, seam) - seam;
+    if (c_begin >= c_end && t_begin >= t_end) return;
+  } else {
+    c_begin = split * chunks_per_split;
+    c_end = min(nch, c_begin + chunks_per_split);
+    if (c_begin >= c_end) return;
+  }
 
   const int tid = threadIdx.x;
   SDMI_STAMP(dbg_t0);
@@ -145,6 +153,11 @@
     return n;
   };
 
+  f16x8 fa[2][G][TM], fb[2][G][TN];
+#ifdef SDMI_IGEMM_TIMING
+  long long dbg_t1 = 0;
+#endif
+  if (!TAIL || c_begin < c_end) {
   const int kt_first = c_begin * 9, kt_last = c_end * 9 - 1;
   {
     const ChunkSrc cs = chunk_src(c_begin);
@@ -161,8 +174,9 @@
   }
   wait_vmcnt_n(in_flight_ok(8));
   asm volatile("s_waitcnt lgkmcnt(0)\n\ts_barrier" ::: "memory");
-  SDMI_STAMP(dbg_t1);
-  f16x8 fa[2][G][TM], fb[2][G][TN];
+#ifdef SDMI_IGEMM_TIMING
+  dbg_t1 = p.dbg_times ? (long long)__builtin_readcyclecounter() : 0;
+#endif
   int ab[TM];
 #pragma unroll
   for (int i = 0; i < TM; ++i) ab[i] = a_base(i, 0, 0, 0);
@@ -219,6 +233,101 @@
     }
   }
   wait_vmcnt<0>();
+  }
+  if constexpr (TAIL) {
+    if (t_begin < t_end) {
+      constexpr int APASS = BM / RPP;
+      constexpr int ASTAGE = BM * 128;
+      constexpr int TS_FIT = 2 * HALO_BYTES / ASTAGE;
+      constexpr int TS = NS < TS_FIT ? NS : TS_FIT;
+      constexpr int LPT = APASS + PB;
+      constexpr int PPU = (LPT + U - 2) / (U - 1);
+      static_assert(TS >= 2 && APASS >= 1 && BM % RPP == 0 && LPT * (TS - 2) <= 48, "tail ring");
+      asm volatile("s_waitcnt vmcnt(0) lgkmcnt(0)\n\ts_barrier" ::: "memory");
+      int ta_off[APASS], tb_off[PB];
+#pragma unroll
+      for (int q = 0; q < APASS; ++q) ta_off[q] = ((m0 + q * RPP + lrow) * p.pw_ld + gch * 8) * 2;
+      const int pq0 = p.pw_c[0], pq01 = p.pw_c[0] + p.pw_c[1], pwK = pq01 + p.pw_c[2];
+#pragma unroll
+      for (int i = 0; i < PB; ++i) tb_off[i] = (min(n0 + i * RPP + lrow, p.N - 1) * pwK + gch * 8) * 2;
+      const char* const tA0 = (const char*)p.pw_a[0]; const char* const tA1 = (const char*)p.pw_a[1];
+      const char* const tA2 = (const char*)p.pw_a[2];
+      const __amdgpu_buffer_rsrc_t rsrc_pw = __builtin_amdgcn_make_buffer_rsrc((void*)p.pw_w, 0, OOB, 0x00020000);
+      int ld_t = t_begin;
+      struct TailCursor { __amdgpu_buffer_rsrc_t rsrc_a; int a_soff, b_soff, stage; };
+      auto tail_next = [&](int stage) {
+        TailCursor c;
+        const int cin0 = ld_t * BK;
+        const char* src; int coff;
+        if (cin0 < pq0) { src = tA0; coff = cin0; }
+        else if (cin0 < pq01) { src = tA1; coff = cin0 - pq0; }
+        else { src = tA2; coff = cin0 - pq01; }
+        c.rsrc_a = __builtin_amdgcn_make_buffer_rsrc((void*)src, 0, OOB, 0x00020000);
+        c.a_soff = coff * 2; c.b_soff = ld_t * (BK * 2); c.stage = stage;
+        if (ld_t + 1 < t_end) ++ld_t;
+        return c;
+      };
+      auto tail_piece = [&](const TailCursor& c, int q) {
+        if (q < APASS) {
+          auto dst = (__attribute__((address_space(3))) void*)(smem + c.stage * ASTAGE + (q * RPP + wave_u * 8) * 128);
+          __builtin_amdgcn_raw_ptr_buffer_load_lds(c.rsrc_a, dst, 16, ta_off[q], c.a_soff, 0, 0);
+        } else {
+          auto dst = (__attribute__((address_space(3))) void*)(smem + 2 * HALO_BYTES + c.stage * BSTAGE + ((q - APASS) * RPP + wave_u * 8) * 128);
+          __builtin_amdgcn_raw_ptr_buffer_load_lds(rsrc_pw, dst, 16, tb_off[q - APASS], c.b_soff, 0, SDMI_W_AUX);
+        }
+      };
+      const int ta_lds = (wm * WTM + l31) * 128;
+      auto tail_frags = [&](int stage, int ks, f16x8 (&a)[TM], f16x8 (&b)[TN]) {
+        const int sw = ((ks * 2 + lg) ^ rsw) << 4;
+        const unsigned char* sa = smem + stage * ASTAGE + ta_lds + sw;
+#pragma unroll
+        for (int i = 0; i < TM; ++i) a[i] = *(const f16x8*)(sa + i * 32 * 128);
+        const unsigned char* sb = smem + stage * BSTAGE + b_lds + sw;
+#pragma unroll
+        for (int j = 0; j < TN; ++j) b[j] = *(const f16x8*)(sb + j * 32 * 128);
+      };
+#pragma unroll
+      for (int s2 = 0; s2 < TS - 1; ++s2) {
+        const TailCursor c = tail_next(s2);
+#pragma unroll
+        for (int q = 0; q < LPT; ++q) tail_piece(c, q);
+      }
+      wait_vmcnt<LPT*(TS - 2)>();
+      asm volatile("s_waitcnt lgkmcnt(0)\n\ts_barrier" ::: "memory");
+#pragma unroll
+      for (int g = 0; g < G; ++g) tail_frags(0, g, fa[0][g], fb[0][g]);
+      int cur = 0, nxt = TS - 1;
+      for (int t = t_begin; t < t_end; ++t) {
+        const TailCursor c = tail_next(nxt);
+        const int cur1 = (cur + 1 == TS) ? 0 : cur + 1;
+#pragma unroll
+        for (int u = 0; u < U; ++u) {
+          if (u + 1 < U) {
+#pragma unroll
+            for (int g = 0; g < G; ++g) tail_frags(cur, (u + 1) * G + g, fa[(u + 1) & 1][g], fb[(u + 1) & 1][g]);
+#pragma unroll
+            for (int q = u * PPU; q < (u + 1) * PPU && q < LPT; ++q) tail_piece(c, q);
+          } else {
+            wait_vmcnt<LPT*(TS - 2)>();
+            asm volatile("s_waitcnt lgkmcnt(0)\n\ts_barrier" ::: "memory");
+#pragma unroll
+            for (int g = 0; g < G; ++g) tail_frags(cur1, g, fa[0][g], fb[0][g]);
+          }
+#pragma unroll
+          for (int g = 0; g < G; ++g) mfma_step(fa[u & 1][g], fb[u & 1][g]);
+          __builtin_amdgcn_sched_group_barrier(0x100, G * (TM + TN), 0);
+#pragma unroll
+          for (int e = 0; e < MPU; ++e) {
+            __builtin_amdgcn_sched_group_barrier(0x008, 1, 0);
+            if (u + 1 < U && e < PPU && u * PPU + e < LPT) __builtin_amdgcn_sched_group_barrier(0x010, 1, 0);
+          }
+        }
+        cur = cur1;
+        nxt = (nxt + 1 == TS) ? 0 : nxt + 1;
+      }
+      wait_vmcnt<0>();
+    }
+  }
   SDMI_STAMP(dbg_t2);
   igemm_epilogue<BM, BN, WARPS_M, WARPS_N, LDS_BYTES>(p, acc, m0, n0, split, tile_m, tile_n, smem);
 #ifdef SDMI_IGEMM_TIMING
@@ -248,9 +357,23 @@
   SDMI_CHECK(halo_supported(p, BM), "halo-staged conv tile requested for an unsupported shape");
   const int tiles_m = cdiv(p.M, BM), tiles_n = cdiv(p.N, BN);
   const int nch = (p.c0 + p.c1 + p.c2) / BK;
-  const int chunks_per_split = cdiv(nch, splitk);
-  const int nsplit = cdiv(nch, chunks_per_split);
+  const bool tail = p.pw_a[0] != nullptr;
+  int chunks_per_split = cdiv(nch, splitk);
+  int nsplit = cdiv(nch, chunks_per_split);
   IGemmParams q = p;
+  if (tail) {
+    const int seam = 9 * nch, T = seam + igemm_tail_k(p) / BK;
+    const int kps = cdiv(T, std::max(1, std::min(splitk, 16)));
+    nsplit = 0;
+    q.pw_bnd[0] = 0;
+    for (int x = kps; ; x += kps) {
+      const int b = x >= T ? T : (x >= seam ? x : (x + 4) / 9 * 9);
+      if (b > q.pw_bnd[nsplit]) q.pw_bnd[++nsplit] = b;
+      if (x >= T) break;
+    }
+    for (int i = nsplit + 1; i < 17; ++i) q.pw_bnd[i] = T;
+    chunks_per_split = 0;
+  }
   q.splitk = nsplit;
   q.tile_n_fastest = tile_order_n_fastest(p);
   q.splitk_fused = 0;
@@ -279,13 +402,16 @@
   std::string pname = std::string("conv3halo_") + std::to_string(BM) + "x" + std::to_string(BN) + "w" +
                       std::to_string(WARPS_M * WARPS_N) + "s" + std::to_string(NS);
   if (by_shape && prof_enabled())
-    pname += "_M" + std::to_string(p.M) + "_N" + std::to_string(p.N) + "_K" + std::to_string(p.K) + "_s" + std::to_string(nsplit);
+    pname += "_M" + std::to_string(p.M) + "_N" + std::to_string(p.N) + "_K" + std::to_string(p.K) + "_s" + std::to_string(nsplit) +
+             (tail ? "_pw" + std::to_string(igemm_tail_k(p)) : std::string());
   const double src_pix = (double)p.B * p.Hin * p.Win;
-  ProfScope ps(pname.c_str(), 2.0 * p.M * (double)p.N * p.K,
+  const double k_tail = tail ? (double)(p.pw_k_alg > 0 ? p.pw_k_alg : igemm_tail_k(p)) : 0.0;
+  ProfScope ps(pname.c_str(), 2.0 * p.M * (double)p.N * (p.K + k_tail),
                src_pix * (p.c0 + p.c1) * 2.0 + (double)p.N * p.K * 2.0 + (double)p.M * p.N * ((p.out_f32 ? 4.0 : 0.0) + (p.out_f16 ? 2.0 : 0.0)) +
-                   (p.residual ? (double)p.M * p.N * 4.0 : 0.0),
+                   (p.residual ? (double)p.M * p.N * 4.0 : 0.0) + ((double)p.M + p.N) * k_tail * 2.0,
                stream);
-  SDMI_LAUNCH((conv3halo_kernel<BM, BN, WARPS_M, WARPS_N, NS>), grid, block, 0, stream, q, tiles_m, tiles_n, chunks_per_split);
+  if (tail) SDMI_LAUNCH((conv3halo_kernel<BM, BN, WARPS_M, WARPS_N, NS, true>), grid, block, 0, stream, q, tiles_m, tiles_n, chunks_per_split);
+  else SDMI_LAUNCH((conv3halo_kernel<BM, BN, WARPS_M, WARPS_N, NS>), grid, block, 0, stream, q, tiles_m, tiles_n, chunks_per_split);
   SDMI_HIP_OK(hipGetLastError());
   ps.end();
   if (nsplit > 1) return launch_splitk_reduce(q, nsplit, stream);
diff --git a/stable-diffusion_amd/csrc/igemm.hip b/stable-diffusion_amd/csrc/igemm.hip
--- a/stable-diffusion_amd/csrc/igemm.hip
+++ b/stable-diffusion_amd/csrc/igemm.hip
@@ -485,6 +485,7 @@
   for (int t = 0; t < SDMI_NUM_TILES; ++t) {
     const TileCfg& c = kTiles[t];
     if (tile_is_halo(t) && !halo_supported(p, c.bm)) continue;
+    if (p.pw_a[0] && !tile_is_halo(t)) continue;
     if (p.split16 && !split16_tile_supported(t)) continue;
     if (!p.split16 && ((c.ns == 2 && t != 11 && !tile_is_halo(t)) || t == 12 || t == 13)) continue;
     if (p.mode == EPI_GEGLU && !tile_tn_even(t)) continue;
@@ -584,6 +585,22 @@
     }
   }
   return 0;
+}
+
+bool igemm_tail_ready(const IGemmParams& p) {
+  if (p.ksize != 3 || p.stride != 1 || p.up || p.pad != 1 || p.split16 || igemm_has_half(p)) return false;
+  static const int env_tile = env_int("SDMI_IGEMM_TILE", -1);
+  if (env_tile >= 0) return env_tile < SDMI_NUM_TILES && tile_is_halo(env_tile) && halo_supported(p, kTiles[env_tile].bm);
+  std::lock_guard<std::mutex> lk(g_tuner.mu);
+  g_tuner.ensure_loaded();
+  if (g_tuner.collecting) return false;
+  static const int env_split = env_int("SDMI_SPLITK", -1);
+  const TuneKey tkey{p.M, p.N, igemm_nkt(p) * BK, 3, 1, 0, p.mode, (env_split >= 0 && p.splitk == 0) ? env_split : p.splitk};
+  const auto it = g_tuner.table.find(tkey);
+  if (it != g_tuner.table.end()) return tile_is_halo(it->second.tile) && halo_supported(p, kTiles[it->second.tile].bm);
+  for (int t = 14; t <= 17; ++t)
+    if (halo_supported(p, kTiles[t].bm)) return true;
+  return false;
 }
 
 int launch_igemm(const IGemmParams& p, const IGemmTune& tune, hipStream_t stream) {
@@ -620,6 +637,21 @@
       SDMI_CHECK(p.gn_acc[t] && p.gn_cpg[t] >= 2 && (p.gn_cbase[t] + p.N + p.gn_cpg[t] - 1) / p.gn_cpg[t] <= 32, "bad GroupNorm statistics target");
   }
   if (p.mode == EPI_HEADS) SDMI_CHECK(p.segC > 0 && p.dh > 0 && p.N % p.segC == 0 && p.N / p.segC <= 3, "bad head scatter");
+  const bool tail = p.pw_a[0] != nullptr;
+  if (tail) {
+    SDMI_CHECK(p.ksize == 3 && p.stride == 1 && !p.up && p.pad == 1 && p.Hin == p.Hout && p.Win == p.Wout && !p.split16,
+               "pointwise tail: needs a 3x3 convolution with stride 1, pad 1 and no upsampling");
+    SDMI_CHECK(p.mode == EPI_PLAIN && !p.lnf_part && !p.lnp_out && !p.f16_scale && !p.ln_out,
+               "pointwise tail: plain epilogue only (no GEGLU, no head scatter, no LayerNorm fold)");
+    SDMI_CHECK((tune.dma >= 0 ? tune.dma : env_int("SDMI_IGEMM_DMA", 1)) != 0, "pointwise tail: LDS-DMA path only (no register staging)");
+    SDMI_CHECK(p.pw_w != nullptr && p.pw_c[0] > 0 && p.pw_c[0] % BK == 0 && p.pw_c[1] % BK == 0 && p.pw_c[2] % BK == 0 && p.pw_c[1] >= 0 &&
+                   p.pw_c[2] >= 0 && !igemm_has_half(p),
+               "pointwise tail: weights missing or a width off the 64-channel grid");
+    SDMI_CHECK((p.pw_c[1] == 0 || p.pw_a[1]) && (p.pw_c[2] == 0 || (p.pw_a[2] && p.pw_c[1] > 0)), "pointwise tail: source missing");
+    SDMI_CHECK(p.pw_ld % 8 == 0 && p.pw_ld >= std::max(p.pw_c[0], std::max(p.pw_c[1], p.pw_c[2])), "pointwise tail: bad row pitch");
+    SDMI_CHECK((int64_t)p.M * p.pw_ld * 2 < ((int64_t)1 << 31) - 65536 && (int64_t)p.N * igemm_tail_k(p) * 2 < ((int64_t)1 << 31) - 65536,
+               "pointwise tail: tensor too large for 31-bit byte offsets");
+  }
 
   SDMI_CHECK((int64_t)p.B * p.Hin * p.Win * p.lda0 * 2 + (int64_t)(p.Win + 1) * p.lda0 * 2 < ((int64_t)1 << 31) - 65536 &&
                  (int64_t)p.N * p.K * 2 < ((int64_t)1 << 31) - 65536,
@@ -669,6 +701,19 @@
       }
     }
   }
+  if (tail) {
+    if (tune.tile >= 0 || env_tile >= 0) SDMI_CHECK(tile_is_halo(tile), "pointwise tail: needs a halo-staged tile (14 .. 17)");
+    if (tile < 0 || !tile_is_halo(tile)) {
+      static const int order[2][4] = {{16, 17, 14, 15}, {14, 15, 16, 17}};
+      tile = -1;
+      for (int t : order[p.M >= 2048 ? 1 : 0])
+        if (halo_supported(p, kTiles[t].bm)) { tile = t; break; }
+      SDMI_CHECK(tile >= 0, "pointwise tail: no halo-staged tile fits this shape");
+      splitk = p.splitk;
+      if (env_split >= 0 && splitk == 0) splitk = env_split;
+    }
+    SDMI_CHECK(halo_supported(p, kTiles[tile].bm), "pointwise tail: the halo-staged tile does not fit this shape");
+  }
   if (p.mode == EPI_GEGLU && tile >= 0 && !tile_tn_even(tile)) tile = 0;
   if (p.split16) {
     if (tile >= 0) SDMI_CHECK(split16_tile_supported(tile), "split-fp16 GEMM: tile id without an instantiation");
diff --git a/stable-diffusion_amd/csrc/unet.cpp b/stable-diffusion_amd/csrc/unet.cpp
--- a/stable-diffusion_amd/csrc/unet.cpp
+++ b/stable-diffusion_amd/csrc/unet.cpp
@@ -462,9 +462,20 @@
       }
       return 0;
     };
-    for (auto& blk : input_blocks_) for (auto& L : blk) if (each(L)) return -1;
-    for (auto& L : middle_) if (each(L)) return -1;
-    for (auto& blk : output_blocks_) for (auto& L : blk) if (each(L)) return -1;
+    std::vector<float> hb2, hbs;
+    auto each_res = [&](Layer& L) -> int {
+      if (L.kind != L_RES || L.updown || L.cin == L.cout || !L.f32[5] || !L.f32[6]) return 0;
+      hb2.resize((size_t)L.cout); hbs.resize((size_t)L.cout);
+      SDMI_HIP_OK(hipMemcpy(hb2.data(), L.f32[5], hb2.size() * sizeof(float), hipMemcpyDeviceToHost));
+      SDMI_HIP_OK(hipMemcpy(hbs.data(), L.f32[6], hbs.size() * sizeof(float), hipMemcpyDeviceToHost));
+      for (size_t i = 0; i < hb2.size(); ++i) hb2[i] += hbs[i];
+      if (dev_alloc((void**)&L.bias2s, hb2.size() * sizeof(float))) return -1;
+      SDMI_HIP_OK(hipMemcpy(L.bias2s, hb2.data(), hb2.size() * sizeof(float), hipMemcpyHostToDevice));
+      return 0;
+    };
+    for (auto& blk : input_blocks_) for (auto& L : blk) if (each(L) || each_res(L)) return -1;
+    for (auto& L : middle_) if (each(L) || each_res(L)) return -1;
+    for (auto& blk : output_blocks_) for (auto& L : blk) if (each(L) || each_res(L)) return -1;
     SDMI_HIP_OK(hipDeviceSynchronize());
   }
   ++weights_gen_;
@@ -567,6 +578,8 @@
   bool st_tail_on = false;
   bool st_mid_ctx_on = false;
   bool ctx1_on = false;
+  int skip_fold_on = 0;
+  int skip_fold_min_hw = 0;
   bool gn_conv_on = false;
   float* emb_all = nullptr;
   int emb_ld = 0;
@@ -628,8 +641,14 @@
       TapeCaller tc(Tape::R_EMB, emb_caller ? p.rowvec : nullptr);
       gemm(p);
     }
+    bool fold = false;
+    if (skip_fold_on && (!p1 || skip_fold_on >= 2) && Cin != Cout && !u->full() && !p3 && !ss && !gc2 && Cin % 64 == 0 && Cout % 64 == 0 && H * W >= skip_fold_min_hw &&
+        L.bias2s) {
+      const IGemmParams probe = conv3(nullptr, Cout, H, W, H, W, 1, 0, L.w16[1], Cout);
+      fold = igemm_tail_ready(probe);
+    }
     const float* residual = x0.p;
-    if (Cin != Cout) {
+    if (Cin != Cout && !fold) {
       IGemmParams p = dense1x1(raw, raw_lo, M, Cin, L.w16[2], Cout, H * W, p1);
       p.bias = L.f32[6]; p.out_f32 = out.p; p.ldo = Cout;
       gemm(p);
@@ -652,6 +671,11 @@
       IGemmParams p = conv3(a2, Cout, H, W, H, W, 1, 0, L.w16[1], Cout);
       if (p3) split3(p, a2, a2_lo, Cout);
       p.bias = L.f32[5]; p.residual = residual; p.ldr = Cout; p.out_f32 = out.p; p.ldo = Cout;
+      if (fold) {
+        p.bias = L.bias2s; p.residual = nullptr; p.ldr = 0;
+        p.pw_a[0] = raw; p.pw_c[0] = Cin; p.pw_ld = Cin; p.pw_w = L.w16[2]; p.pw_k_alg = Cin;
+        if (p1) { p.pw_a[1] = raw_lo; p.pw_c[1] = Cin; p.pw_a[2] = raw; p.pw_c[2] = Cin; }
+      }
       attach_gn_targets(p, out);
       attach_f16_copy(p, out);
       gemm(p);
@@ -1214,6 +1238,9 @@
     f.ctx1_on = !(e_c1 && atoi(e_c1) == 0);
     const char* e_gc = getenv("SDMI_GN_CONV");
     f.gn_conv_on = e_gc ? atoi(e_gc) != 0 : false;
+    const char* e_sf = getenv("SDMI_SKIP_FOLD"); const char* e_sfm = getenv("SDMI_SKIP_FOLD_MIN_HW");
+    f.skip_fold_on = tune_collecting() ? 0 : (e_sf ? atoi(e_sf) : 1);
+    f.skip_fold_min_hw = e_sfm ? atoi(e_sfm) : 0;
     if (full()) {
       f.ln_fold_on = f.ff_tail_on = f.st_head_on = f.st_mid_on = f.st_tail_on = f.st_mid_ctx_on = f.gn_conv_on = false;
     }
diff --git a/stable-diffusion_amd/csrc/unet.h b/stable-diffusion_amd/csrc/unet.h
--- a/stable-diffusion_amd/csrc/unet.h
+++ b/stable-diffusion_amd/csrc/unet.h
@@ -204,6 +204,7 @@
   f16* w16[3] = {nullptr, nullptr, nullptr};
   float* w32[1] = {nullptr};
   float* f32[7] = {nullptr, nullptr, nullptr, nullptr, nullptr, nullptr, nullptr};
+  float* bias2s = nullptr;
   std::vector<TBlock> tb;
 };
 
```
